# sec-bit/ckb-zkp

Measured on AMD Instinct MI355X. Metric: Groth16 proofs/sec (2^20 constraints, BN256), higher is better.
Workload: dtype u32 limbs (256-bit Montgomery integers); 1 GPU; Groth16 prove, MiMC-chain R1CS, 1048570 constraints (domain 2^20), 1258284 aux, bn254, G1 x4 + G2 x1 MSM + 4 NTT (7 in the reference: evaluation-form key); curve=bn254, log_domain=20, parallelism=independent proofs x1

## Files before the change

ckb_zkp_amd/_lib.py:

```python
from __future__ import annotations

import ctypes as C
import os
from pathlib import Path

LIB_PATH = Path(os.environ.get("ZKP_ACCEL_LIB") or Path(__file__).resolve().parent / "lib" / "libzkp_accel.so")

u64p = C.POINTER(C.c_uint64)
u32p = C.POINTER(C.c_uint32)
u8p = C.POINTER(C.c_uint8)
vp = C.c_void_p


class ZkpError(RuntimeError):
    def __init__(self, status: int, where: str, text: str):
        super().__init__(f"{where}: status {status} ({text})")
        self.status = status


class Csr(C.Structure):
    _fields_ = [("row_ptr", vp), ("col", vp), ("coeff", vp)]


class Groth16PkDesc(C.Structure):
# ... 35 lines not shown

class CtxConfig(C.Structure):
    _fields_ = [("struct_size", C.c_uint32), ("lanes", C.c_int32), ("msm_batch_lanes", C.c_int32),
                ("msm_window_bits", C.c_int32), ("msm_window_bits_g2", C.c_int32), ("msm_chunk_points", C.c_int64),
                ("table_budget_gb", C.c_double), ("h_evaluation_form", C.c_int32), ("c_fold", C.c_int32),
                ("host_affine", C.c_int32), ("c_fold_heavy_cost", C.c_int64), ("multi_exchange", C.c_int32),
                ("multi_exchange_timeout_ms", C.c_int32), ("multi_witness_split", C.c_int32)]


ZKP_ON, ZKP_OFF = 1, 2
ZKP_EXCHANGE_AUTO, ZKP_EXCHANGE_RCCL, ZKP_EXCHANGE_PEER = 0, 1, 2


def make_config(config) -> "CtxConfig | None":
    if config is None:
        return None
    if isinstance(config, CtxConfig):
        cfg = config
    else:
        cfg = CtxConfig()
        names = {f[0] for f in CtxConfig._fields_} - {"struct_size"}
        for k, v in dict(config).items():
            if k not in names:
                raise KeyError(f"zkp_ctx_config has no field {k!r} (fields: {sorted(names)})")
            if isinstance(v, bool):
                v = ZKP_ON if v else ZKP_OFF
            if k == "multi_exchange" and isinstance(v, str):
                v = {"auto": ZKP_EXCHANGE_AUTO, "rccl": ZKP_EXCHANGE_RCCL, "peer": ZKP_EXCHANGE_PEER}[v]
            setattr(cfg, k, v)
    cfg.struct_size = C.sizeof(CtxConfig)
    return cfg


MARLIN_NUM_EVALS = 21


class MarlinProof(C.Structure):
    _fields_ = [("comm", C.c_uint64 * (9 * 12)), ("comm_inf", C.c_uint8 * 9),
                ("shifted", C.c_uint64 * (2 * 12)), ("shifted_inf", C.c_uint8 * 2),
                ("evaluations", C.c_uint64 * (MARLIN_NUM_EVALS * 4)), ("num_opening_proofs", C.c_uint32),
                ("opening_w", C.c_uint64 * (2 * 12)), ("opening_w_inf", C.c_uint8 * 2), ("opening_has_rand", C.c_uint8 * 2),
                ("opening_rand_v", C.c_uint64 * (2 * 4)), ("challenges", C.c_uint64 * (7 * 4))]


SIGNATURES = {
    "zkp_status_string": (C.c_char_p, [C.c_int32]),
    "zkp_version": (C.c_char_p, []),
    "zkp_ctx_create": (C.c_int32, [C.POINTER(vp), C.c_int]),
    "zkp_ctx_create_ex": (C.c_int32, [C.POINTER(vp), C.c_int, C.POINTER(CtxConfig)]),
    "zkp_ctx_get_config": (C.c_int32, [vp, C.POINTER(CtxConfig)]),
    "zkp_ctx_destroy": (C.c_int32, [vp]),
    "zkp_ctx_create_multi": (C.c_int32, [C.POINTER(vp), C.POINTER(C.c_int), C.c_int]),
    "zkp_ctx_create_multi_ex": (C.c_int32, [C.POINTER(vp), C.POINTER(C.c_int), C.c_int, C.POINTER(CtxConfig)]),
    "zkp_ctx_num_devices": (C.c_int32, [vp, C.POINTER(C.c_int32)]),
    "zkp_ctx_device": (C.c_int32, [vp, C.c_int32, C.POINTER(vp)]),
    "zkp_groth16_pk_upload_multi": (C.c_int32, [vp, C.POINTER(Groth16PkDesc), C.c_int32, C.POINTER(vp)]),
    "zkp_groth16_pk_multi_free": (C.c_int32, [vp, vp]),
    "zkp_groth16_multi_info": (C.c_int32, [vp, vp, u64p]),
    "zkp_groth16_prove_multi": (C.c_int32, [vp, vp, vp, C.c_int32, vp, vp, vp, vp]),
    "zkp_groth16_prove_batch_multi": (C.c_int32, [vp, vp, C.c_size_t, vp, C.c_int32, vp, vp, vp, vp]),
    "zkp_ctx_set_stream": (C.c_int32, [vp, vp]),
    "zkp_ctx_sync": (C.c_int32, [vp]),
    "zkp_dev_alloc": (C.c_int32, [vp, C.c_size_t, C.POINTER(vp)]),
    "zkp_dev_free": (C.c_int32, [vp, vp]),
    "zkp_h2d": (C.c_int32, [vp, vp, vp, C.c_size_t]),
    "zkp_d2h": (C.c_int32, [vp, vp, vp, C.c_size_t]),
    "zkp_timer_start": (C.c_int32, [vp]),
    "zkp_timer_stop_ms": (C.c_int32, [vp, C.POINTER(C.c_float)]),
    "zkp_ntt": (C.c_int32, [vp, C.c_int, vp, C.c_uint32, C.c_int32]),
    "zkp_ntt_dev": (C.c_int32, [vp, C.c_int, vp, C.c_uint32, C.c_int32]),
    "zkp_bases_upload_g1": (C.c_int32, [vp, C.c_int, vp, vp, C.c_size_t, C.POINTER(C.c_uint64)]),
    "zkp_bases_upload_g2": (C.c_int32, [vp, C.c_int, vp, vp, C.c_size_t, C.POINTER(C.c_uint64)]),
    "zkp_bases_share": (C.c_int32, [vp, vp, C.c_uint64, u64p]),
    "zkp_bases_free": (C.c_int32, [vp, C.c_uint64]),
    "zkp_bases_len": (C.c_int32, [vp, C.c_uint64, C.POINTER(C.c_size_t)]),
    "zkp_msm_g1": (C.c_int32, [vp, C.c_uint64, C.c_size_t, vp, C.c_size_t, vp]),
    "zkp_msm_g2": (C.c_int32, [vp, C.c_uint64, C.c_size_t, vp, C.c_size_t, vp]),
    "zkp_msm_g1_dev": (C.c_int32, [vp, C.c_uint64, C.c_size_t, vp, C.c_size_t, vp]),
    "zkp_msm_g2_dev": (C.c_int32, [vp, C.c_uint64, C.c_size_t, vp, C.c_size_t, vp]),
    "zkp_vartime_multiscalar_mul_g1": (C.c_int32, [vp, C.c_uint64, vp, C.c_size_t, vp]),
    "zkp_vartime_multiscalar_mul_g2": (C.c_int32, [vp, C.c_uint64, vp, C.c_size_t, vp]),
    "zkp_msm_g1_var": (C.c_int32, [vp, C.c_int, vp, vp, vp, C.c_size_t, C.c_int32, vp]),
    "zkp_msm_g2_var": (C.c_int32, [vp, C.c_int, vp, vp, vp, C.c_size_t, C.c_int32, vp]),
    "zkp_msm_g1_var_batch_dev": (C.c_int32, [vp, C.c_int, C.c_size_t, vp, vp, vp, vp, C.c_int32, vp]),
    "zkp_msm_g2_var_batch_dev": (C.c_int32, [vp, C.c_int, C.c_size_t, vp, vp, vp, vp, C.c_int32, vp]),
    "zkp_g1_ipa_fold_dev": (C.c_int32, [vp, C.c_int, vp, vp, vp, vp, C.c_size_t, vp, vp, vp, vp]),
    "zkp_fr_dot_batch_dev": (C.c_int32, [vp, C.c_int, C.c_size_t, vp, vp, vp, vp]),
    "zkp_fr_sumcheck_round_dev": (C.c_int32, [vp, C.c_int, C.c_int32, C.c_size_t, vp, C.c_size_t, vp, vp]),
    "zkp_fr_eq_evals_dev": (C.c_int32, [vp, C.c_int, vp, C.c_size_t, vp]),
    "zkp_fr_product_circuit_dev": (C.c_int32, [vp, C.c_int, C.c_size_t, vp, C.c_size_t, vp]),
    "zkp_fr_memcheck_circuits_dev": (C.c_int32, [vp, C.c_int, C.c_size_t, vp, vp, vp, vp, vp, C.c_size_t, vp, vp, vp]),
    "zkp_msm_g1_mont_dev": (C.c_int32, [vp, C.c_uint64, C.c_size_t, vp, C.c_size_t, vp]),
    "zkp_msm_g2_mont_dev": (C.c_int32, [vp, C.c_uint64, C.c_size_t, vp, C.c_size_t, vp]),
    "zkp_msm_g1_mont_batch_dev": (C.c_int32, [vp, C.c_uint64, C.c_size_t, vp, vp, vp, vp]),
    "zkp_msm_mont_multi_dev": (C.c_int32, [vp, C.c_size_t, vp, vp, vp, vp, vp, C.c_size_t]),
    "zkp_fr_vec_op_dev": (C.c_int32, [vp, C.c_int, C.c_int32, vp, vp, vp, vp, C.c_size_t]),
    "zkp_fr_spmv_dev": (C.c_int32, [vp, C.c_int, vp, vp, vp, C.c_size_t, vp, vp]),
    "zkp_fr_gather_dev": (C.c_int32, [vp, vp, vp, C.c_size_t, vp]),
    "zkp_poly_divide_by_vanishing_dev": (C.c_int32, [vp, C.c_int, vp, C.c_size_t, C.c_size_t, vp, vp]),
    "zkp_d2d": (C.c_int32, [vp, vp, vp, C.c_size_t]),
    "zkp_dev_zero": (C.c_int32, [vp, vp, C.c_size_t]),
    "zkp_fr_batch_inverse_dev": (C.c_int32, [vp, C.c_int, vp, C.c_size_t]),
    "zkp_poly_evaluate_dev": (C.c_int32, [vp, C.c_int, vp, C.c_size_t, vp, vp]),
    "zkp_poly_div_linear_dev": (C.c_int32, [vp, C.c_int, vp, C.c_size_t, vp, vp, vp]),
    "zkp_g1_fold": (C.c_int32, [vp, C.c_int, vp, C.c_size_t, vp]),
    "zkp_g2_fold": (C.c_int32, [vp, C.c_int, vp, C.c_size_t, vp]),
    "zkp_g1_into_affine": (C.c_int32, [vp, C.c_int, vp, vp, vp]),
    "zkp_g1_decompress": (C.c_int32, [vp, C.c_int, vp, C.c_size_t, vp, vp, C.POINTER(C.c_size_t)]),
    "zkp_g2_decompress": (C.c_int32, [vp, C.c_int, vp, C.c_size_t, vp, vp, C.POINTER(C.c_size_t)]),
    "zkp_g1_compress": (C.c_int32, [vp, C.c_int, vp, vp, C.c_size_t, vp]),
    "zkp_g2_compress": (C.c_int32, [vp, C.c_int, vp, vp, C.c_size_t, vp]),
    "zkp_g1_subgroup_check": (C.c_int32, [vp, C.c_int, vp, vp, C.c_size_t, C.POINTER(C.c_size_t)]),
    "zkp_g2_subgroup_check": (C.c_int32, [vp, C.c_int, vp, vp, C.c_size_t, C.POINTER(C.c_size_t)]),
    "zkp_g2_into_affine": (C.c_int32, [vp, C.c_int, vp, vp, vp]),
    "zkp_groth16_points_into_affine": (C.c_int32, [C.c_int, vp, vp, vp, vp, vp]),
    "zkp_fixed_base_mul_g1": (C.c_int32, [vp, C.c_int, vp, vp, C.c_size_t, vp, vp]),
    "zkp_fixed_base_mul_g2": (C.c_int32, [vp, C.c_int, vp, vp, C.c_size_t, vp, vp]),
    "zkp_groth16_pk_upload": (C.c_int32, [vp, C.POINTER(Groth16PkDesc), C.POINTER(vp)]),
    "zkp_groth16_pk_upload_ex": (C.c_int32, [vp, C.POINTER(Groth16PkDesc), C.c_uint32, C.POINTER(vp)]),
    "zkp_groth16_pk_upload_shard": (C.c_int32, [vp, C.POINTER(Groth16PkDesc), C.c_int32, C.c_int32, C.POINTER(vp)]),
    "zkp_groth16_partials_bytes": (C.c_int32, [C.c_int, C.POINTER(C.c_size_t)]),
    "zkp_groth16_prove_partials_dev": (C.c_int32, [vp, vp, vp, vp, vp, vp]),
    "zkp_groth16_fold_assemble_dev": (C.c_int32, [vp, C.c_int, vp, C.c_int32, vp, vp, vp, vp]),
    "zkp_groth16_pk_free": (C.c_int32, [vp, vp]),
    "zkp_groth16_witness_map": (C.c_int32, [vp, vp, vp, vp]),
    "zkp_groth16_witness_map_dev": (C.c_int32, [vp, vp, vp, vp]),
    "zkp_groth16_domain_size": (C.c_int32, [vp, C.POINTER(C.c_uint64)]),
    "zkp_groth16_pk_info": (C.c_int32, [vp, vp, C.POINTER(C.c_uint64)]),
    "zkp_groth16_prove": (C.c_int32, [vp, vp, vp, vp, vp, vp, vp]),
    "zkp_groth16_prove_dev": (C.c_int32, [vp, vp, vp, vp, vp, vp, vp]),
    "zkp_groth16_prove_batch_dev": (C.c_int32, [vp, vp, C.c_size_t, vp, vp, vp, vp, vp]),
    "zkp_groth16_prove_batch": (C.c_int32, [vp, vp, C.c_size_t, vp, vp, vp, vp, vp]),
    "zkp_groth16_assemble": (C.c_int32, [vp, C.c_int, vp, vp, vp, vp, vp]),
    "zkp_groth16_last_timing": (C.c_int32, [vp, C.POINTER(Groth16Timing)]),
    "zkp_marlin_last_timing": (C.c_int32, [vp, C.POINTER(MarlinTiming)]),
    "zkp_set_profiling": (C.c_int32, [vp, C.c_int32]),
    "zkp_marlin_index_upload": (C.c_int32, [vp, C.POINTER(MarlinIndexDesc), C.POINTER(vp)]),
    "zkp_marlin_index_free": (C.c_int32, [vp, vp]),
    "zkp_marlin_index_info": (C.c_int32, [vp, u64p]),
    "zkp_marlin_index_commit": (C.c_int32, [vp, vp, C.c_uint64, vp, vp]),
    "zkp_marlin_prove": (C.c_int32, [vp, vp, C.c_uint64, C.c_uint64, vp, C.c_size_t, vp, vp, C.c_size_t,
                                     C.POINTER(MarlinRand), vp, C.POINTER(MarlinProof)]),
    "zkp_fs_rng_new": (C.c_int32, [vp, C.c_size_t, C.POINTER(vp)]),
    "zkp_fs_rng_free": (C.c_int32, [vp]),
    "zkp_fs_rng_absorb": (C.c_int32, [vp, vp, C.c_size_t]),
    "zkp_fs_rng_seed": (C.c_int32, [vp, vp]),
    "zkp_fs_rng_next_u64": (C.c_int32, [vp, u64p]),
    "zkp_fs_rng_rand_u128": (C.c_int32, [vp, vp]),
    "zkp_fs_rng_rand_fr": (C.c_int32, [vp, C.c_int, vp]),
    "zkp_fs_rng_sample_outside_domain": (C.c_int32, [vp, C.c_int, C.c_uint32, vp]),
    "zkp_merlin_oneshot": (C.c_int32, [vp, C.c_size_t, vp, C.c_size_t, vp, C.c_size_t, vp, C.c_size_t, vp, C.c_size_t]),
    "zkp_bench_mulmod": (C.c_int32, [vp, C.c_int, C.c_int32, C.c_int32, C.POINTER(C.c_double)]),
    "zkp_bench_hbm_copy": (C.c_int32, [vp, C.c_size_t, C.POINTER(C.c_double)]),
}

_lib = None


def load(path: os.PathLike | None = None) -> C.CDLL:
    global _lib
    if _lib is not None and path is None:
        return _lib
    p = Path(path) if path else LIB_PATH
    if not p.exists():
        raise ImportError(f"{p} not found — build it with `python -m ckb_zkp_amd.build` "
                          "(hipcc --offload-arch=gfx950); there is no CPU fallback")
    lib = C.CDLL(str(p))
    for name, (res, args) in SIGNATURES.items():
        fn = getattr(lib, name)
        fn.restype, fn.argtypes = res, args
    if path is None:
        _lib = lib
    return lib


ZKP_ERR_INVALID_POINT = -7


def check(status: int, where: str) -> None:
    if status != 0:
        raise ZkpError(status, where, load().zkp_status_string(status).decode())
```

ckb_zkp_amd/csrc/capi.hip:

```cpp
#include <cstdint>
#include <cstdlib>
#include <cstring>

#include "ctx.hpp"
#include "host_field.hpp"
#include "internal.hpp"
#include "ipa.hpp"
#include "spark.hpp"
#include "sumcheck.hpp"

using namespace zkp;

namespace {

template <class Fn>
int32_t guarded(zkp_ctx* ctx, Fn&& fn) {
  if (!ctx) return ZKP_ERR_BAD_ARG;
  std::lock_guard<std::recursive_mutex> lk(ctx->mu);
  try {
    ZKP_HIP(hipSetDevice(ctx->device));
    fn();
    return ZKP_OK;
  } catch (const StatusError& e) {
    return e.status;
// ... 572 lines not shown
  return subgroup_any(ctx, curve, 1, xy, inf, n, bad);
}
int32_t zkp_g2_subgroup_check(zkp_ctx* ctx, zkp_curve_t curve, const uint64_t* xy, const uint8_t* inf, size_t n, size_t* bad) {
  return subgroup_any(ctx, curve, 2, xy, inf, n, bad);
}
int32_t zkp_fixed_base_mul_g1(zkp_ctx* ctx, zkp_curve_t curve, const uint64_t* base, const uint64_t* scalars, size_t n,
                              uint64_t* out_xy, uint8_t* out_inf) {
  if (!base || (n && (!scalars || !out_xy || !out_inf))) return ZKP_ERR_BAD_ARG;
  return guarded(ctx, [&] { fixed_base_mul(ctx, curve, 1, base, scalars, n, out_xy, out_inf); });
}
int32_t zkp_fixed_base_mul_g2(zkp_ctx* ctx, zkp_curve_t curve, const uint64_t* base, const uint64_t* scalars, size_t n,
                              uint64_t* out_xy, uint8_t* out_inf) {
  if (!base || (n && (!scalars || !out_xy || !out_inf))) return ZKP_ERR_BAD_ARG;
  return guarded(ctx, [&] { fixed_base_mul(ctx, curve, 2, base, scalars, n, out_xy, out_inf); });
}

int32_t zkp_groth16_pk_upload(zkp_ctx* ctx, const zkp_groth16_pk_desc* desc, zkp_groth16_pk** out) {
  if (!desc || !out) return ZKP_ERR_BAD_ARG;
  return guarded(ctx, [&] { *out = groth16_pk_upload(ctx, desc); });
}
int32_t zkp_groth16_pk_upload_ex(zkp_ctx* ctx, const zkp_groth16_pk_desc* desc, uint32_t flags, zkp_groth16_pk** out) {
  if (!desc || !out || (flags & ~(uint32_t)ZKP_PK_KEEP_FORM)) return ZKP_ERR_BAD_ARG;
  return guarded(ctx, [&] { *out = groth16_pk_upload(ctx, desc, 0, 0, (int)flags); });
}
int32_t zkp_groth16_pk_upload_shard(zkp_ctx* ctx, const zkp_groth16_pk_desc* desc, int32_t rank, int32_t world,
                                    zkp_groth16_pk** out) {
  if (!desc || !out || world < 1 || rank < 0 || rank >= world) return ZKP_ERR_BAD_ARG;
  return guarded(ctx, [&] { *out = groth16_pk_upload(ctx, desc, rank, world); });
}
int32_t zkp_groth16_partials_bytes(zkp_curve_t curve, size_t* bytes) {
  if (!bytes || (curve != ZKP_BN254 && curve != ZKP_BLS12_381)) return ZKP_ERR_BAD_ARG;
  *bytes = groth16_partials_bytes(curve);
  return ZKP_OK;
}
int32_t zkp_groth16_prove_partials_dev(zkp_ctx* ctx, zkp_groth16_pk* pk, const uint64_t* z_dev, const uint64_t* r,
                                       const uint64_t* s, void* partials_dev) {
  if (!pk || !z_dev || !r || !s || !partials_dev) return ZKP_ERR_BAD_ARG;
  return guarded(ctx, [&] { groth16_prove_partials(ctx, pk, z_dev, r, s, partials_dev); });
}
int32_t zkp_groth16_fold_assemble_dev(zkp_ctx* ctx, zkp_curve_t curve, const void* gathered_dev, int32_t world,
                                      const uint64_t* r, const uint64_t* s, uint64_t* proof, uint8_t* inf) {
  if (!gathered_dev || world < 1 || !r || !s || !proof || !inf) return ZKP_ERR_BAD_ARG;
  return guarded(ctx, [&] { groth16_fold_assemble(ctx, curve, gathered_dev, world, r, s, proof, inf); });
}
int32_t zkp_groth16_pk_upload_multi(zkp_ctx* ctx, const zkp_groth16_pk_desc* desc, int32_t mode, zkp_groth16_pk_multi** out) {
  if (!ctx || !desc || !out || ctx->devs.empty() || (mode != ZKP_MULTI_SHARD && mode != ZKP_MULTI_REPLICATE)) return ZKP_ERR_BAD_ARG;
  return guarded_multi(ctx, [&] { *out = groth16_pk_upload_multi(ctx, desc, mode); });
}
int32_t zkp_groth16_pk_multi_free(zkp_ctx* ctx, zkp_groth16_pk_multi* pk) {
  if (!ctx || !pk || ctx->devs.empty()) return ZKP_ERR_BAD_ARG;
  return guarded_multi(ctx, [&] { groth16_pk_multi_free(ctx, pk); });
}
int32_t zkp_groth16_multi_info(zkp_ctx* ctx, zkp_groth16_pk_multi* pk, uint64_t info[6]) {
  if (!ctx || !pk || !info || ctx->devs.empty()) return ZKP_ERR_BAD_ARG;
  return guarded(ctx, [&] { groth16_multi_info(ctx, pk, info); });
}
int32_t zkp_groth16_prove_multi(zkp_ctx* ctx, zkp_groth16_pk_multi* pk, const uint64_t* const* z, int32_t z_on_device,
                                const uint64_t* r, const uint64_t* s, uint64_t* proof, uint8_t* inf) {
  if (!ctx || !pk || !z || !z[0] || !r || !s || !proof || !inf || ctx->devs.empty()) return ZKP_ERR_BAD_ARG;
  if (z_on_device)
    for (size_t k = 0; k < ctx->devs.size(); k++)
      if (!z[k]) return ZKP_ERR_BAD_ARG;
  return guarded_multi(ctx, [&] { groth16_prove_multi(ctx, pk, z, z_on_device != 0, r, s, proof, inf); });
}
int32_t zkp_groth16_prove_batch_multi(zkp_ctx* ctx, zkp_groth16_pk_multi* pk, size_t count, const uint64_t* const* z,
                                      int32_t z_on_device, const uint64_t* r, const uint64_t* s, uint64_t* proofs,
                                      uint8_t* inf) {
  if (!ctx || !pk || ctx->devs.empty() || (count && (!z || !r || !s || !proofs || !inf))) return ZKP_ERR_BAD_ARG;
  return guarded_multi(ctx, [&] { groth16_prove_batch_multi(ctx, pk, count, z, z_on_device != 0, r, s, proofs, inf); });
}
int32_t zkp_groth16_pk_free(zkp_ctx* ctx, zkp_groth16_pk* pk) {
  if (!pk) return ZKP_ERR_BAD_ARG;
  return guarded(ctx, [&] { groth16_pk_free(ctx, pk); });
}
int32_t zkp_groth16_pk_info(zkp_ctx* ctx, zkp_groth16_pk* pk, uint64_t info[8]) {
  if (!ctx || !pk || !info) return ZKP_ERR_BAD_ARG;
  return guarded(ctx, [&] { groth16_pk_info(ctx, pk, info); });
}
int32_t zkp_groth16_domain_size(zkp_groth16_pk* pk, uint64_t* n) {
  if (!pk || !n) return ZKP_ERR_BAD_ARG;
  *n = groth16_domain_size(pk);
  return ZKP_OK;
}
int32_t zkp_groth16_witness_map(zkp_ctx* ctx, zkp_groth16_pk* pk, const uint64_t* z, uint64_t* h) {
  if (!pk || !z || !h) return ZKP_ERR_BAD_ARG;
  return guarded(ctx, [&] { groth16_witness_map(ctx, pk, z, h, false); });
}
int32_t zkp_groth16_witness_map_dev(zkp_ctx* ctx, zkp_groth16_pk* pk, const uint64_t* z, uint64_t* h) {
  if (!pk || !z || !h) return ZKP_ERR_BAD_ARG;
  return guarded(ctx, [&] { groth16_witness_map(ctx, pk, z, h, true); });
}
int32_t zkp_groth16_prove(zkp_ctx* ctx, zkp_groth16_pk* pk, const uint64_t* z, const uint64_t* r, const uint64_t* s,
                          uint64_t* proof, uint8_t* inf) {
  if (!pk || !z || !r || !s || !proof || !inf) return ZKP_ERR_BAD_ARG;
  return guarded(ctx, [&] { groth16_prove(ctx, pk, z, false, r, s, proof, inf); });
}
int32_t zkp_groth16_prove_dev(zkp_ctx* ctx, zkp_groth16_pk* pk, const uint64_t* z, const uint64_t* r,
                              const uint64_t* s, uint64_t* proof, uint8_t* inf) {
  if (!pk || !z || !r || !s || !proof || !inf) return ZKP_ERR_BAD_ARG;
  return guarded(ctx, [&] { groth16_prove(ctx, pk, z, true, r, s, proof, inf); });
}
int32_t zkp_groth16_prove_batch_dev(zkp_ctx* ctx, zkp_groth16_pk* pk, size_t n, const uint64_t* const* z_dev,
                                    const uint64_t* r, const uint64_t* s, uint64_t* proofs, uint8_t* inf) {
  if (!pk || (n && (!z_dev || !r || !s || !proofs || !inf))) return ZKP_ERR_BAD_ARG;
  return guarded(ctx, [&] { groth16_prove_batch(ctx, pk, n, z_dev, r, s, proofs, inf); });
}
int32_t zkp_groth16_prove_batch(zkp_ctx* ctx, zkp_groth16_pk* pk, size_t n, const uint64_t* const* z_host,
                                const uint64_t* r, const uint64_t* s, uint64_t* proofs, uint8_t* inf) {
  if (!pk || (n && (!z_host || !r || !s || !proofs || !inf))) return ZKP_ERR_BAD_ARG;
  return guarded(ctx, [&] { groth16_prove_batch(ctx, pk, n, z_host, r, s, proofs, inf, false); });
}
int32_t zkp_groth16_assemble(zkp_ctx* ctx, zkp_curve_t curve, const uint64_t* sums, const uint64_t* r,
                             const uint64_t* s, uint64_t* proof, uint8_t* inf) {
  if (!sums || !r || !s || !proof || !inf) return ZKP_ERR_BAD_ARG;
  return guarded(ctx, [&] { groth16_assemble(ctx, curve, sums, r, s, proof, inf); });
}
int32_t zkp_marlin_index_upload(zkp_ctx* ctx, const zkp_marlin_index_desc* desc, zkp_marlin_index** out) {
  if (!desc || !out) return ZKP_ERR_BAD_ARG;
  return guarded(ctx, [&] { *out = marlin_index_upload(ctx, desc); });
}
int32_t zkp_marlin_index_free(zkp_ctx* ctx, zkp_marlin_index* index) {
  if (!index) return ZKP_ERR_BAD_ARG;
  return guarded(ctx, [&] { marlin_index_free(ctx, index); });
}
int32_t zkp_marlin_index_info(const zkp_marlin_index* index, uint64_t info[6]) {
  if (!index || !info) return ZKP_ERR_BAD_ARG;
  marlin_index_info(index, info);
  return ZKP_OK;
}
int32_t zkp_marlin_index_commit(zkp_ctx* ctx, zkp_marlin_index* index, uint64_t powers_of_g, uint64_t* comms_xy,
                                uint8_t* inf) {
  if (!index || !comms_xy || !inf) return ZKP_ERR_BAD_ARG;
  return guarded(ctx, [&] { marlin_index_commit(ctx, index, powers_of_g, comms_xy, inf); });
}
int32_t zkp_marlin_prove(zkp_ctx* ctx, zkp_marlin_index* index, uint64_t powers_of_g, uint64_t powers_of_gamma_g,
                         const uint8_t* ivk_bytes, size_t ivk_len, const uint64_t* x, const uint64_t* w, size_t n_w,
                         const zkp_marlin_rand* rnd, const uint64_t* fixed_challenges, zkp_marlin_proof* out) {
  if (!index || !x || (n_w && !w) || !rnd || !out || (!fixed_challenges && !ivk_bytes)) return ZKP_ERR_BAD_ARG;
  if (!rnd->w || !rnd->z_a || !rnd->z_b || !rnd->mask || !rnd->blind_w || !rnd->blind_z_a || !rnd->blind_z_b ||
      !rnd->blind_g_1 || !rnd->blind_shifted_g_1)
    return ZKP_ERR_BAD_ARG;
  return guarded(ctx, [&] {
    marlin_prove(ctx, index, powers_of_g, powers_of_gamma_g, ivk_bytes, ivk_len, x, w, n_w, rnd, fixed_challenges, out);
  });
}
int32_t zkp_bench_mulmod(zkp_ctx* ctx, zkp_curve_t curve, int32_t field, int32_t unsaturated, double* out) {
  if (!out || (curve != ZKP_BN254 && curve != ZKP_BLS12_381) || field < 0 || field > 1) return ZKP_ERR_BAD_ARG;
  return guarded(ctx, [&] { *out = bench_mulmod(ctx, curve, field, unsaturated != 0); });
}
int32_t zkp_bench_hbm_copy(zkp_ctx* ctx, size_t bytes, double* out) {
  if (!out) return ZKP_ERR_BAD_ARG;
  return guarded(ctx, [&] { *out = bench_hbm_copy(ctx, bytes); });
}
int32_t zkp_marlin_last_timing(zkp_ctx* ctx, zkp_marlin_timing* out) {
  if (!ctx || !out) return ZKP_ERR_BAD_ARG;
  return guarded(ctx, [&] { *out = ctx->last_marlin_timing; });
}
int32_t zkp_groth16_last_timing(zkp_ctx* ctx, zkp_groth16_timing* out) {
  if (!ctx || !out) return ZKP_ERR_BAD_ARG;
  return guarded(ctx, [&] { *out = ctx->last_timing; });
}

}
```

ckb_zkp_amd/csrc/internal.hpp:

```cpp
#pragma once
#include "ctx.hpp"

namespace zkp {

void ntt_run(zkp_ctx* ctx, int curve, uint32_t* data_dev, int log_n, int op);
void ntt_run_batch(zkp_ctx* ctx, int curve, uint32_t* const* data_dev, int count, int log_n, int op);
bool ntt_ifft_coset_fft(zkp_ctx* ctx, int curve, uint32_t* data, int log_n);
uint32_t* ntt_qap_coset_ifft(zkp_ctx* ctx, int curve, uint32_t* a, uint32_t* b, uint32_t* c, const uint32_t* zinv, int log_n);
void ntt_free_tables(zkp_ctx* ctx);

void fr_vec_op(zkp_ctx* ctx, int curve, int op, const uint64_t* a, const uint64_t* b, const uint64_t* k_host,
               uint64_t* out, size_t n);
void fr_batch_inverse(zkp_ctx* ctx, int curve, uint64_t* v, size_t n);
void fr_dot_batch(zkp_ctx* ctx, int curve, size_t count, const uint64_t* const* a, const uint64_t* const* b, const size_t* ns,
                  uint64_t* out_host);
void fr_spmv(zkp_ctx* ctx, int curve, const uint32_t* row_ptr, const uint32_t* col, const uint64_t* coeff, size_t nrows,
             const uint64_t* x, uint64_t* out);
void fr_gather(zkp_ctx* ctx, const uint64_t* in, const int32_t* idx, size_t n, uint64_t* out);
void poly_vanishing_fold(zkp_ctx* ctx, int curve, const uint64_t* p, size_t len, size_t n, uint64_t* q, uint64_t* rem);
void poly_div_linear(zkp_ctx* ctx, int curve, const uint64_t* p, size_t n, const uint64_t* z_host, uint64_t* q,
                     uint64_t* eval_out_host);
void marlin_round2_prod(zkp_ctx* ctx, int curve, const uint64_t* ra, const uint64_t* za, const uint64_t* zb, const uint64_t* t,
                        const uint64_t* z, const uint64_t* k_host, uint64_t* out, size_t n);
void marlin_t3_evals(zkp_ctx* ctx, int curve, const uint64_t* const* on_k, const uint64_t* k_host, uint64_t* out, size_t n);
void marlin_h2_numerator(zkp_ctx* ctx, int curve, const uint64_t* const* on_b, const uint64_t* t, const uint64_t* k_host, uint64_t* out,
                         size_t n);
void poly_evaluate_batch(zkp_ctx* ctx, int curve, size_t count, const uint64_t* const* p, const size_t* n, const uint64_t* z_host,
                         uint64_t* out_host);

uint64_t bases_upload(zkp_ctx* ctx, int curve, int group, const uint64_t* xy_host, const uint8_t* inf_host, size_t n,
                      int c_hint = 0, int cap_hint = 0, int lgk_hint = -1);
size_t bases_table_bytes(zkp_ctx* ctx, int curve, int group, size_t n, int lgk);
int bases_plan_lgk(zkp_ctx* ctx, int curve, const int* groups, const size_t* ns, int count);
void bases_free(zkp_ctx* ctx, uint64_t handle);
uint64_t bases_share(zkp_ctx* dst, zkp_ctx* src, uint64_t handle);
size_t bases_len(zkp_ctx* ctx, uint64_t handle);
int bases_group(zkp_ctx* ctx, uint64_t handle);
void msm_run(zkp_ctx* ctx, uint64_t handle, size_t offset, const uint64_t* scalars_dev, size_t n, bool montgomery,
             uint64_t* out_xyz_host, void* out_dev_xyzz = nullptr, float* ms_accumulate = nullptr,
             uint64_t* n_entries = nullptr, int ws = 0, int sort_src = -1, float* ms_scan = nullptr, int l1_src = -1);
double bench_mulmod(zkp_ctx* ctx, int curve, int field, bool unsaturated);
double bench_hbm_copy(zkp_ctx* ctx, size_t bytes);
bool bases_same_shape(zkp_ctx* ctx, uint64_t h1, uint64_t h2);
void bases_set_sort_flags(zkp_ctx* ctx, uint64_t handle, const uint8_t* flags_host, size_t n);
void bases_set_group(zkp_ctx* ctx, uint64_t owner, const uint8_t* member_flags_host, size_t n);
void bases_set_filter_bit(zkp_ctx* ctx, uint64_t handle, int bit);
void msm_run_batch(zkp_ctx* ctx, uint64_t handle, size_t count, const size_t* offsets, const uint64_t* const* scalars_dev,
                   const size_t* ns, bool montgomery, uint64_t* out_xyz_host);
void msm_run_multi(zkp_ctx* ctx, size_t count, const uint64_t* handles, const size_t* offsets,
                   const uint64_t* const* scalars_dev, const size_t* ns, bool montgomery, uint64_t* out_xyz_host,
                   size_t slot_words);
void msm_var_run(zkp_ctx* ctx, int curve, int group, const uint64_t* xy_host, const uint8_t* inf_host,
                 const uint64_t* scalars_host, size_t n, bool montgomery, uint64_t* out_xyz_host);
void msm_var_batch_run(zkp_ctx* ctx, int curve, int group, size_t count, const uint64_t* const* xy_dev,
                       const uint8_t* const* inf_dev, const uint64_t* const* scalars_dev, const size_t* ns, bool montgomery,
                       uint64_t* out_xyz_host);
void msm_free_all(zkp_ctx* ctx);
void bases_drop(zkp_ctx* ctx, uint64_t handle);
void point_fold(zkp_ctx* ctx, int curve, int group, const uint64_t* xyz_host, size_t k, uint64_t* out_xyz_host);
void point_into_affine(zkp_ctx* ctx, int curve, int group, const uint64_t* xyz_host, uint64_t* xy_out, uint8_t* inf_out);
size_t points_decompress(zkp_ctx* ctx, int curve, int group, const uint8_t* bytes, size_t n, uint64_t* xy_out, uint8_t* inf_out);
void points_compress(zkp_ctx* ctx, int curve, int group, const uint64_t* xy, const uint8_t* inf, size_t n, uint8_t* bytes_out);
size_t points_subgroup_check(zkp_ctx* ctx, int curve, int group, const uint64_t* xy, const uint8_t* inf, size_t n);
void points_fold_into_affine(zkp_ctx* ctx, int curve, int group, const uint64_t* a_xyz_host, const uint64_t* b_xyz_host,
                             const uint8_t* has_b, size_t k, uint64_t* xy_out, uint8_t* inf_out);
void fixed_base_mul(zkp_ctx* ctx, int curve, int group, const uint64_t* base_xy, const uint64_t* scalars_host, size_t n,
                    uint64_t* out_xy, uint8_t* out_inf);

zkp_groth16_pk* groth16_pk_upload(zkp_ctx* ctx, const zkp_groth16_pk_desc* d, int rank = 0, int world = 0, int flags = 0);
size_t groth16_partials_bytes(int curve);
void groth16_prove_partials(zkp_ctx* ctx, zkp_groth16_pk* pk, const uint64_t* z_dev, const uint64_t* r, const uint64_t* s,
                            void* out_dev);
void groth16_fold_assemble(zkp_ctx* ctx, int curve, const void* gathered_dev, int world, const uint64_t* r,
                           const uint64_t* s, uint64_t* proof_out, uint8_t* inf_out);
void groth16_pk_free(zkp_ctx* ctx, zkp_groth16_pk* pk);
uint64_t groth16_domain_size(zkp_groth16_pk* pk);
void groth16_pk_info(zkp_ctx* ctx, zkp_groth16_pk* pk, uint64_t info[8]);
void bases_info(zkp_ctx* ctx, uint64_t handle, uint64_t info[5]);
void groth16_witness_map(zkp_ctx* ctx, zkp_groth16_pk* pk, const uint64_t* z, uint64_t* h, bool on_device);
void groth16_prove(zkp_ctx* ctx, zkp_groth16_pk* pk, const uint64_t* z, bool z_on_device, const uint64_t* r,
                   const uint64_t* s, uint64_t* proof_out, uint8_t* inf_out);

void groth16_prove_batch(zkp_ctx* ctx, zkp_groth16_pk* pk, size_t n, const uint64_t* const* z_dev, const uint64_t* r,
                         const uint64_t* s, uint64_t* proofs_out, uint8_t* inf_out, bool z_on_device = true);
void groth16_assemble(zkp_ctx* ctx, int curve, const uint64_t* sums_xyz, const uint64_t* r, const uint64_t* s,
                      uint64_t* proof_out, uint8_t* inf_out);

zkp_groth16_pk_multi* groth16_pk_upload_multi(zkp_ctx* root, const zkp_groth16_pk_desc* d, int mode);
void groth16_pk_multi_free(zkp_ctx* root, zkp_groth16_pk_multi* pk);
void groth16_multi_info(zkp_ctx* root, zkp_groth16_pk_multi* pk, uint64_t info[6]);
void groth16_prove_multi(zkp_ctx* root, zkp_groth16_pk_multi* pk, const uint64_t* const* z, bool z_on_device, const uint64_t* r,
                         const uint64_t* s, uint64_t* proof_out, uint8_t* inf_out);
void groth16_prove_batch_multi(zkp_ctx* root, zkp_groth16_pk_multi* pk, size_t n, const uint64_t* const* z, bool z_on_device,
                               const uint64_t* r, const uint64_t* s, uint64_t* proofs_out, uint8_t* inf_out);

zkp_marlin_index* marlin_index_upload(zkp_ctx* ctx, const zkp_marlin_index_desc* d);
void marlin_index_free(zkp_ctx* ctx, zkp_marlin_index* ix);
void marlin_index_commit(zkp_ctx* ctx, zkp_marlin_index* ix, uint64_t powers_g, uint64_t* comms_xy, uint8_t* inf);
void marlin_index_info(const zkp_marlin_index* ix, uint64_t info[6]);
void marlin_prove(zkp_ctx* ctx, zkp_marlin_index* ix, uint64_t powers_g, uint64_t powers_gamma_g, const uint8_t* ivk_bytes,
                  size_t ivk_len, const uint64_t* x_mont, const uint64_t* w_mont, size_t n_w, const zkp_marlin_rand* rnd,
                  const uint64_t* fixed_challenges, zkp_marlin_proof* out);

}
```

ckb_zkp_amd/csrc/msm.hip:

```cpp
#include <algorithm>
#include <cstdlib>
#include <cstring>
#include <map>
#include <type_traits>
#include <memory>
#include <mutex>
#include <vector>

#include "field_dev.hpp"
#include "internal.hpp"
#include "msm_digits.hpp"
#include "msm_small.hpp"
#include "msm_vtbl.hpp"

namespace zkp {

#if defined(ZKP_NO_SORT_PRIO)
#define ZKP_SORT_PRIO() do { } while (0)
#else
#define ZKP_SORT_PRIO() __builtin_amdgcn_s_setprio(3)
#endif

const MsmVtbl* msm_vtbl_c01();
const MsmVtbl* msm_vtbl_c02();
// ... 65 lines not shown
  if ((1 << lgk) >= p.W) {
    p.lgk = 0;
    while ((1 << p.lgk) < p.W) p.lgk++;
  }
  p.J = (p.W + (1 << p.lgk) - 1) >> p.lgk;
  return p;
}
size_t bases_table_bytes(zkp_ctx* ctx, int curve, int group, size_t n, int lgk) {
  const MsmVtbl* vt = msm_vtbl(curve, group);
  return std::max<size_t>(1, n) * (size_t)window_plan(ctx->cfg, vt->scalar_bits, n, group, 0, lgk).J * vt->aff_bytes;
}
static double table_budget_left(zkp_ctx* ctx) {
  size_t free_b = 0, total_b = 0;
  if (hipMemGetInfo(&free_b, &total_b) != hipSuccess) return 1e30;
  double left = (double)free_b - 0.25 * (double)total_b;
  if (ctx->cfg.table_budget_gb > 0.0) {
    const double b = ctx->cfg.table_budget_gb * 1073741824.0 - (double)ctx->table_bytes;
    left = std::min(left + 0.25 * (double)total_b - 1073741824.0, b);
  }
  return left;
}
int bases_plan_lgk(zkp_ctx* ctx, int curve, const int* groups, const size_t* ns, int count) {
  if (const char* e = getenv("ZKP_TABLE_K")) {
    int k = atoi(e), lg = 0;
    while ((1 << lg) < k) lg++;
    return std::min(lg, 6);
  }
  const double left = table_budget_left(ctx);
  for (int lgk = 0; lgk <= 6; lgk++) {
    double need = 0;
    for (int q = 0; q < count; q++) need += (double)bases_table_bytes(ctx, curve, groups[q], ns[q], lgk);
    if (need <= left) return lgk;
  }
  return 6;
}

uint64_t bases_upload(zkp_ctx* ctx, int curve, int group, const uint64_t* xy, const uint8_t* inf, size_t n, int c_hint,
                      int cap_hint, int lgk_hint) {
  auto e = std::make_shared<BasesEntry>();
  e->curve = curve;
  e->group = group;
  e->vt = msm_vtbl(curve, group);
  e->n = n;
  int lgk = lgk_hint;
  if (lgk < 0) lgk = c_hint > 0 ? 0 : bases_plan_lgk(ctx, curve, &group, &n, 1);
  const WindowPlan wp = window_plan(ctx->cfg, e->vt->scalar_bits, n, group, c_hint, lgk);
  e->c = wp.c;
  e->W = wp.W;
  e->wide = wp.wide;
  e->lgk = wp.lgk;
  e->var = wp.lgk > 0;
  {
    const char* env = group == 2 ? getenv("ZKP_TASK_CAP_G2") : nullptr;
    if (!env) env = getenv("ZKP_TASK_CAP");
    if (cap_hint >= 4) e->cap = std::min<uint32_t>(MSM_TASK_CAP, (uint32_t)cap_hint);
    if (env && atoi(env) >= 4) e->cap = std::min<uint32_t>(MSM_TASK_CAP, (uint32_t)atoi(env));
  }
  ZKP_REQUIRE((double)n * e->W < 2147483000.0, ZKP_ERR_BAD_ARG);
  const size_t ab = e->vt->aff_bytes;
  size_t bytes = std::max<size_t>(1, n) * wp.J * ab;
  if (hipMalloc(&e->table, bytes) != hipSuccess) throw StatusError{ZKP_ERR_OOM};
  e->table_bytes = bytes;
  ctx->table_bytes += bytes;
  if (n) {
    ZKP_HIP(hipMemcpyAsync(e->table, xy, n * ab, hipMemcpyHostToDevice, ctx->cur->stream));
    if (inf) {
      if (hipMalloc(&e->inf, n) != hipSuccess) throw StatusError{ZKP_ERR_OOM};
      ZKP_HIP(hipMemcpyAsync(e->inf, inf, n, hipMemcpyHostToDevice, ctx->cur->stream));
      e->vt->ingest(ctx->cur->stream, e->table, e->inf, n);
    }
    if (wp.lgk > 0) e->vt->precompute(ctx->cur->stream, e->table, n, e->c << wp.lgk, wp.J, wp.J);
    else e->vt->precompute(ctx->cur->stream, e->table, n, e->c, e->W, e->wide);
    ZKP_HIP(hipGetLastError());
    ZKP_HIP(hipStreamSynchronize(ctx->cur->stream));
  }
  if (getenv("ZKP_DEBUG_MSM"))
    fprintf(stderr, "[msm] bases group=%d n=%zu: c=%d W=%d wide=%d k=%d copies=%d (%.2f GiB)\n", group, n, e->c, e->W, e->wide,
            1 << e->lgk, wp.J, (double)bytes / 1073741824.0);
  uint64_t h = ctx->next_handle++;
  ctx->bases[h] = e;
  return h;
}

static std::shared_ptr<BasesEntry> get_bases(zkp_ctx* ctx, uint64_t handle) {
  auto it = ctx->bases.find(handle);
  if (it == ctx->bases.end()) throw StatusError{ZKP_ERR_BAD_HANDLE};
  return it->second;
}
void bases_free(zkp_ctx* ctx, uint64_t handle) {
  ZKP_HIP(hipStreamSynchronize(ctx->cur->stream));
  auto it = ctx->bases.find(handle);
  if (it == ctx->bases.end()) throw StatusError{ZKP_ERR_BAD_HANDLE};
  if (it->second.use_count() == 1) ctx->table_bytes -= std::min(ctx->table_bytes, it->second->table_bytes);
  ctx->bases.erase(it);
}
size_t bases_len(zkp_ctx* ctx, uint64_t handle) { return get_bases(ctx, handle)->n; }
int bases_group(zkp_ctx* ctx, uint64_t handle) { return get_bases(ctx, handle)->group; }
void bases_info(zkp_ctx* ctx, uint64_t handle, uint64_t info[5]) {
  auto e = get_bases(ctx, handle);
  info[0] = (uint64_t)e->c;
  info[1] = (uint64_t)e->W;
  info[2] = (uint64_t)1 << e->lgk;
  info[3] = e->lgk ? (uint64_t)((e->W + (1 << e->lgk) - 1) >> e->lgk) : (uint64_t)e->W;
  info[4] = e->table_bytes;
}
void bases_drop(zkp_ctx* ctx, uint64_t handle) {
  auto it = ctx->bases.find(handle);
  if (it == ctx->bases.end()) return;
  if (it->second.use_count() == 1) ctx->table_bytes -= std::min(ctx->table_bytes, it->second->table_bytes);
  ctx->bases.erase(it);
}
void msm_free_all(zkp_ctx* ctx) {
  ctx->bases.clear();
  ctx->table_bytes = 0;
  ctx->var_plans.clear();
}
uint64_t bases_share(zkp_ctx* dst, zkp_ctx* src, uint64_t handle) {
  auto e = get_bases(src, handle);
  ZKP_REQUIRE(dst->device == src->device, ZKP_ERR_BAD_ARG);
  uint64_t h = dst->next_handle++;
  dst->bases[h] = e;
  return h;
}
void bases_set_sort_flags(zkp_ctx* ctx, uint64_t handle, const uint8_t* flags_host, size_t n) {
  auto e = get_bases(ctx, handle);
  ZKP_REQUIRE(n == e->n, ZKP_ERR_BAD_ARG);
  if (e->sort_inf) (void)hipFree(e->sort_inf);
  e->sort_inf = nullptr;
  if (!flags_host || n == 0) return;
  if (hipMalloc(&e->sort_inf, n) != hipSuccess) throw StatusError{ZKP_ERR_OOM};
  ZKP_HIP(hipMemcpyAsync(e->sort_inf, flags_host, n, hipMemcpyHostToDevice, ctx->cur->stream));
  ZKP_HIP(hipStreamSynchronize(ctx->cur->stream));
}
void bases_set_group(zkp_ctx* ctx, uint64_t owner, const uint8_t* member_flags_host, size_t n) {
  auto e = get_bases(ctx, owner);
  ZKP_REQUIRE(n == e->n, ZKP_ERR_BAD_ARG);
  if (e->group_flags) (void)hipFree(e->group_flags);
  e->group_flags = nullptr;
  if (!member_flags_host || n == 0) return;
  if (hipMalloc(&e->group_flags, n) != hipSuccess) throw StatusError{ZKP_ERR_OOM};
  ZKP_HIP(hipMemcpyAsync(e->group_flags, member_flags_host, n, hipMemcpyHostToDevice, ctx->cur->stream));
  ZKP_HIP(hipStreamSynchronize(ctx->cur->stream));
}
void bases_set_filter_bit(zkp_ctx* ctx, uint64_t handle, int bit) {
  ZKP_REQUIRE(bit >= -1 && bit < 3, ZKP_ERR_BAD_ARG);
  get_bases(ctx, handle)->filter_bit = bit;
}
bool bases_same_shape(zkp_ctx* ctx, uint64_t h1, uint64_t h2) {
  auto a = get_bases(ctx, h1), b = get_bases(ctx, h2);
  return a->curve == b->curve && a->n == b->n && a->c == b->c && a->W == b->W && a->wide == b->wide && a->cap == b->cap && a->lgk == b->lgk;
}


constexpr int SCAN_CHUNK = 2048;
__global__ __launch_bounds__(256) void scan_reduce_kernel(const uint32_t* __restrict__ in, size_t n,
                                                          uint32_t* __restrict__ sums) {
  ZKP_SORT_PRIO();
  __shared__ uint32_t red[256];
  size_t base = (size_t)blockIdx.x * SCAN_CHUNK;
  uint32_t acc = 0;
  for (int k = 0; k < SCAN_CHUNK / 256; k++) {
    size_t i = base + (size_t)k * 256 + threadIdx.x;
    if (i < n) acc += in[i];
  }
  red[threadIdx.x] = acc;
  __syncthreads();
  for (int s = 128; s > 0; s >>= 1) {
    if ((int)threadIdx.x < s) red[threadIdx.x] += red[threadIdx.x + s];
    __syncthreads();
  }
  if (threadIdx.x == 0) sums[blockIdx.x] = red[0];
}
__global__ __launch_bounds__(1024) void scan_sums_kernel(uint32_t* __restrict__ sums, size_t m) {
  ZKP_SORT_PRIO();
  __shared__ uint32_t buf[1024];
  uint32_t carry = 0;
  for (size_t t0 = 0; t0 < m; t0 += 1024) {
    size_t i = t0 + threadIdx.x;
    uint32_t v = i < m ? sums[i] : 0;
    buf[threadIdx.x] = v;
    __syncthreads();
    for (int d = 1; d < 1024; d <<= 1) {
      uint32_t add = (int)threadIdx.x >= d ? buf[threadIdx.x - d] : 0;
      __syncthreads();
      buf[threadIdx.x] += add;
      __syncthreads();
    }
    if (i < m) sums[i] = carry + buf[threadIdx.x] - v;
    uint32_t total = buf[1023];
    __syncthreads();
    carry += total;
  }
}
__global__ __launch_bounds__(256) void scan_apply_kernel(const uint32_t* __restrict__ in, size_t n,
                                                         const uint32_t* __restrict__ sums,
                                                         uint32_t* __restrict__ out) {
  ZKP_SORT_PRIO();
  __shared__ uint32_t part[256];
  size_t base = (size_t)blockIdx.x * SCAN_CHUNK;
  constexpr int PER = SCAN_CHUNK / 256;
  uint32_t v[PER];
  uint32_t acc = 0;
  for (int k = 0; k < PER; k++) {
    size_t i = base + (size_t)threadIdx.x * PER + k;
    v[k] = i < n ? in[i] : 0;
    acc += v[k];
  }
  part[threadIdx.x] = acc;
  __syncthreads();
  for (int d = 1; d < 256; d <<= 1) {
    uint32_t add = (int)threadIdx.x >= d ? part[threadIdx.x - d] : 0;
    __syncthreads();
    part[threadIdx.x] += add;
    __syncthreads();
  }
  uint32_t run = sums[blockIdx.x] + part[threadIdx.x] - acc;
  for (int k = 0; k < PER; k++) {
    size_t i = base + (size_t)threadIdx.x * PER + k;
    if (i < n) out[i] = run;
    run += v[k];
  }
}
static void exclusive_scan_u32(hipStream_t st, const uint32_t* in, uint32_t* out, size_t n, DevBuf& tmp) {
  if (n == 0) return;
  size_t chunks = (n + SCAN_CHUNK - 1) / SCAN_CHUNK;
  uint32_t* sums = tmp.as<uint32_t>(chunks + 1);
  hipLaunchKernelGGL(scan_reduce_kernel, dim3(chunks), dim3(256), 0, st, in, n, sums);
  hipLaunchKernelGGL(scan_sums_kernel, dim3(1), dim3(1024), 0, st, sums, chunks);
  hipLaunchKernelGGL(scan_apply_kernel, dim3(chunks), dim3(256), 0, st, in, n, sums, out);
}

constexpr int SORT_H1_MAX = 13;
constexpr uint32_t SORT_BIN_TARGET = 16384;
constexpr int SORT_L_MAX = 13;
constexpr int SORT_SCALARS = 2048;
constexpr int SORT_SCALARS_UNUSED_ = 0;
template <class FrP, int NT>
__global__ __launch_bounds__(NT) void sort_hist_kernel(const uint32_t* __restrict__ scalars, size_t n, size_t offset,
                                                        const uint8_t* __restrict__ inf, int montgomery, int c, int W, int wide,
                                                        uint32_t nb, int L, uint32_t nbins1,
                                                        uint32_t* __restrict__ hist, uint32_t nblocks, uint32_t tile,
                                                        int lgk) {
  ZKP_SORT_PRIO();
  const uint32_t gmask = (1u << lgk) - 1;
  __shared__ uint32_t cnt[(1 << SORT_H1_MAX) + 1];
  for (uint32_t i = threadIdx.x; i <= nbins1; i += NT) cnt[i] = 0;
  __syncthreads();
  for (uint32_t j = threadIdx.x; j < tile; j += NT) {
    size_t i = (size_t)blockIdx.x * tile + j;
    if (i < n && !(inf && inf[offset + i])) {
      DigitIter it = load_scalar<FrP>(scalars, i, montgomery);
      for (int w = 0; w < W; w++) {
        uint32_t key, neg;
        it.next(w, c, wide, nb, key, neg);
        if (key < nb) atomicAdd(&cnt[((((uint32_t)w & gmask) << (c - 1)) | key) >> L], 1u);
      }
    }
  }
  __syncthreads();
  for (uint32_t i = threadIdx.x; i < nbins1; i += NT) hist[(size_t)i * nblocks + blockIdx.x] = cnt[i];
}
template <class FrP>
__global__ __launch_bounds__(256) void sort_scatter_kernel(const uint32_t* __restrict__ scalars, size_t n,
                                                           size_t offset, const uint8_t* __restrict__ inf,
                                                           int montgomery, size_t ntab, int c, int W, int wide, uint32_t nb,
                                                           int L, uint32_t nbins1, const uint32_t* __restrict__ offs,
                                                           uint32_t nblocks, uint32_t tile,
                                                           uint64_t* __restrict__ kv, int lgk,
                                                           const uint8_t* __restrict__ group_flags) {
  ZKP_SORT_PRIO();
  const uint32_t gmask = (1u << lgk) - 1;
  __shared__ uint32_t cur[(1 << SORT_H1_MAX) + 1];
  for (uint32_t i = threadIdx.x; i < nbins1; i += 256) cur[i] = offs[(size_t)i * nblocks + blockIdx.x];
  __syncthreads();
  const uint32_t lmask = (1u << L) - 1;
  for (uint32_t rep = 0; rep < tile / 256; rep++) {
    size_t i = (size_t)blockIdx.x * tile + rep * 256 + threadIdx.x;
    if (i < n && !(inf && inf[offset + i])) {
      DigitIter it = load_scalar<FrP>(scalars, i, montgomery);
      const uint64_t gbits = group_flags ? (uint64_t)(group_flags[offset + i] & 7u) << 61 : 0;
      for (int w = 0; w < W; w++) {
        uint32_t key, neg;
        it.next(w, c, wide, nb, key, neg);
        if (key < nb) {
          const uint32_t fk = (((uint32_t)w & gmask) << (c - 1)) | key;
          uint32_t pos = atomicAdd(&cur[fk >> L], 1u);
          uint32_t val = (uint32_t)((size_t)(w >> lgk) * ntab + offset + i) | (neg << 31);
          kv[pos] = gbits | ((uint64_t)(fk & lmask) << 32) | val;
        }
      }
    }
  }
}
template <int NT>
__device__ __forceinline__ uint32_t block_excl_scan(uint32_t v, uint32_t* tmp, uint32_t* total) {
  const uint32_t t = threadIdx.x, lane = t & 63u, wave = t >> 6;
  uint32_t incl = v;
#pragma unroll
  for (int d = 1; d < 64; d <<= 1) {
    const uint32_t up = (uint32_t)__shfl_up((int)incl, d, 64);
    if (lane >= (uint32_t)d) incl += up;
  }
  if (lane == 63u) tmp[wave] = incl;
  __syncthreads();
  if (t == 0) {
    uint32_t run = 0;
    for (int w = 0; w < NT / 64; w++) {
      const uint32_t x = tmp[w];
      tmp[w] = run;
      run += x;
    }
    tmp[NT / 64] = run;
  }
  __syncthreads();
  const uint32_t res = tmp[wave] + incl - v;
  *total = tmp[NT / 64];
  __syncthreads();
  return res;
}

__device__ __forceinline__ uint32_t wave_agg_inc(uint32_t* cnt, uint32_t idx, bool active) {
  const uint64_t act = __ballot(active);
  uint32_t res = 0;
  if (act == 0) return 0;
  const int leader = __ffsll((unsigned long long)act) - 1;
  const uint32_t lidx = (uint32_t)__builtin_amdgcn_readlane((int)idx, leader);
  const bool same = active && idx == lidx;
  const uint64_t m = __ballot(same);
  const uint32_t pc = (uint32_t)__popcll(m);
  if (pc >= 8) {
    const uint32_t lane = __builtin_amdgcn_mbcnt_hi(~0u, __builtin_amdgcn_mbcnt_lo(~0u, 0u));
    uint32_t base = 0;
    if ((int)lane == leader) base = atomicAdd(&cnt[lidx], pc);
    base = (uint32_t)__builtin_amdgcn_readlane((int)base, leader);
    if (same) res = base + __builtin_amdgcn_mbcnt_hi((uint32_t)(m >> 32), __builtin_amdgcn_mbcnt_lo((uint32_t)m, 0u));
    else if (active) res = atomicAdd(&cnt[idx], 1u);
  } else if (active) {
    res = atomicAdd(&cnt[idx], 1u);
  }
  return res;
}

#ifndef ZKP_SORT_STAGE_BYTES
#define ZKP_SORT_STAGE_BYTES (56 * 1024)
#endif
constexpr uint32_t SORT_STAGE_BYTES = ZKP_SORT_STAGE_BYTES;
template <class FrP, int NT>
__global__ __launch_bounds__(NT) void sort_scatter_staged_kernel(const uint32_t* __restrict__ scalars, size_t n,
                                                                  size_t offset, const uint8_t* __restrict__ inf,
                                                                  int montgomery, size_t ntab, int c, int W, int wide, uint32_t nb,
                                                                  int L, uint32_t nbins1, const uint32_t* __restrict__ offs,
                                                                  uint32_t nblocks, uint32_t tile, uint64_t* __restrict__ kv,
                                                                  int lgk, const uint8_t* __restrict__ group_flags, uint32_t sub) {
  ZKP_SORT_PRIO();
  const uint32_t gmask = (1u << lgk) - 1;
  extern __shared__ __attribute__((aligned(16))) uint32_t sm[];
  __shared__ uint32_t pre[NT];
  uint32_t* cur = sm;
  uint32_t* cnt = cur + nbins1;
  uint64_t* stage = reinterpret_cast<uint64_t*>(cnt + ((nbins1 + 3) & ~3u));
  const uint32_t tid = threadIdx.x;
  for (uint32_t i = tid; i < nbins1; i += NT) cur[i] = offs[(size_t)i * nblocks + blockIdx.x];
  const uint32_t lmask = (1u << L) - 1;
  const uint32_t per = (nbins1 + NT - 1) / NT;
  for (uint32_t s0 = 0; s0 < tile; s0 += sub) {
    for (uint32_t i = tid; i < nbins1; i += NT) cnt[i] = 0;
    __syncthreads();
    for (uint32_t rep = 0; rep * NT < sub; rep++) {
      const uint32_t j = rep * NT + tid;
      const size_t i = (size_t)blockIdx.x * tile + s0 + j;
      const bool live = j < sub && s0 + j < tile && i < n && !(inf && inf[offset + i]);
      DigitIter it = load_scalar<FrP>(scalars, live ? i : 0, montgomery);
      for (int w = 0; w < W; w++) {
        uint32_t key, neg;
        it.next(w, c, wide, nb, key, neg);
        const uint32_t fk = (((uint32_t)w & gmask) << (c - 1)) | key;
        (void)wave_agg_inc(cnt, fk >> L, live && key < nb);
      }
    }
    __syncthreads();
    uint32_t total;
    {
      uint32_t acc = 0;
      for (uint32_t k = 0; k < per; k++) {
        const uint32_t idx = tid * per + k;
        if (idx < nbins1) acc += cnt[idx];
      }
      uint32_t run = block_excl_scan<NT>(acc, pre, &total);
      for (uint32_t k = 0; k < per; k++) {
        const uint32_t idx = tid * per + k;
        if (idx < nbins1) {
          const uint32_t v = cnt[idx];
          cnt[idx] = run;
          run += v;
        }
      }
    }
    __syncthreads();
    for (uint32_t rep = 0; rep * NT < sub; rep++) {
      const uint32_t j = rep * NT + tid;
      const size_t i = (size_t)blockIdx.x * tile + s0 + j;
      const bool live = j < sub && s0 + j < tile && i < n && !(inf && inf[offset + i]);
      DigitIter it = load_scalar<FrP>(scalars, live ? i : 0, montgomery);
      const uint64_t gbits = live && group_flags ? (uint64_t)(group_flags[offset + i] & 7u) << 61 : 0;
      for (int w = 0; w < W; w++) {
        uint32_t key, neg;
        it.next(w, c, wide, nb, key, neg);
        const uint32_t fk = (((uint32_t)w & gmask) << (c - 1)) | key;
        const bool act = live && key < nb;
        const uint32_t pos = wave_agg_inc(cnt, fk >> L, act);
        if (act) {
          const uint32_t val = (uint32_t)((size_t)(w >> lgk) * ntab + offset + i) | (neg << 31);
          stage[pos] = gbits | ((uint64_t)(fk >> L) << 45) | ((uint64_t)(fk & lmask) << 32) | val;
        }
      }
    }
    __syncthreads();
    for (uint32_t j = tid; j < total; j += NT) {
      const uint64_t e = stage[j];
      const uint32_t b = (uint32_t)(e >> 45) & 0x1fffu;
      const uint32_t lo = b ? cnt[b - 1] : 0;
      kv[cur[b] + (j - lo)] = e;
    }
    __syncthreads();
    for (uint32_t b = tid; b < nbins1; b += NT) cur[b] += cnt[b] - (b ? cnt[b - 1] : 0);
    __syncthreads();
  }
}
constexpr uint32_t SORT_BIN_THREADS = 1024;
#ifndef ZKP_SORT_BIN_STAGE
#define ZKP_SORT_BIN_STAGE 20480
#endif
constexpr uint32_t SORT_BIN_STAGE = ZKP_SORT_BIN_STAGE;
__global__ __launch_bounds__(SORT_BIN_THREADS) void sort_bin_kernel(const uint64_t* __restrict__ kv,
                                                                    const uint32_t* __restrict__ offs,
                                                                    uint32_t nblocks, int L,
                                                                    uint32_t* __restrict__ vout,
                                                                    uint32_t* __restrict__ start,
                                                                    uint32_t* __restrict__ end, int drop_bit) {
  ZKP_SORT_PRIO();
  extern __shared__ uint32_t sm[];
  __shared__ uint32_t pre[SORT_BIN_THREADS];
  const uint32_t nk = 1u << L;
  uint32_t* cnt = sm;
  uint32_t* stage = sm + nk;
  const uint32_t b = blockIdx.x, T = SORT_BIN_THREADS, t = threadIdx.x;
  const uint32_t lo = offs[(size_t)b * nblocks], hi = offs[(size_t)(b + 1) * nblocks];
  const bool staged = hi - lo <= SORT_BIN_STAGE;
  for (uint32_t i = t; i < nk; i += T) cnt[i] = 0;
  __syncthreads();
  const uint64_t dmask = drop_bit >= 0 ? (uint64_t)1 << (61 + drop_bit) : 0;
  const uint32_t kmask = nk - 1;
  for (uint32_t i = lo + t; i < hi; i += T) {
    const uint64_t x = kv[i];
    if (!(x & dmask)) atomicAdd(&cnt[(uint32_t)(x >> 32) & kmask], 1u);
  }
  __syncthreads();
  {
    const uint32_t per = (nk + T - 1) / T;
    uint32_t acc = 0;
    for (uint32_t k = 0; k < per; k++) {
      uint32_t idx = t * per + k;
      if (idx < nk) acc += cnt[idx];
    }
    uint32_t total_unused;
    uint32_t run = block_excl_scan<(int)SORT_BIN_THREADS>(acc, pre, &total_unused);
    for (uint32_t k = 0; k < per; k++) {
      uint32_t idx = t * per + k;
      if (idx < nk) {
        uint32_t v = cnt[idx];
        start[((size_t)b << L) + idx] = lo + run;
        end[((size_t)b << L) + idx] = lo + run + v;
        cnt[idx] = run;
        run += v;
      }
    }
  }
  __syncthreads();
  for (uint32_t i = lo + t; i < hi; i += T) {
    const uint64_t x = kv[i];
    if (x & dmask) continue;
    uint32_t pos = atomicAdd(&cnt[(uint32_t)(x >> 32) & kmask], 1u);
    if (staged) stage[pos] = (uint32_t)x;
    else vout[lo + pos] = (uint32_t)x;
  }
  if (staged) {
    __syncthreads();
    for (uint32_t i = t; i < hi - lo; i += T) vout[lo + i] = stage[i];
  }
}

constexpr int TM_NLONG = 0, TM_HIST = 1, TM_CUR = 256, TM_WORDS = 512;

__global__ void task_count_kernel(const uint32_t* __restrict__ start, const uint32_t* __restrict__ end, uint32_t nb,
                                  uint32_t* __restrict__ tcount, uint32_t cap) {
  ZKP_SORT_PRIO();
  uint32_t b = blockIdx.x * blockDim.x + threadIdx.x;
  if (b > nb) return;
  tcount[b] = b < nb ? (end[b] - start[b] + cap - 1) / cap : 0;
}

__global__ __launch_bounds__(256) void zero_empty_buckets_kernel(const uint32_t* __restrict__ start,
                                                                 const uint32_t* __restrict__ end, uint32_t nb,
                                                                 char* __restrict__ buckets, uint32_t xb) {
  ZKP_SORT_PRIO();
  const uint32_t b = blockIdx.x * blockDim.x + threadIdx.x;
  if (b >= nb || end[b] != start[b]) return;
  uint4* p = reinterpret_cast<uint4*>(buckets + (size_t)b * xb);
  for (uint32_t k = 0; k < xb / 16; k++) p[k] = make_uint4(0, 0, 0, 0);
}

__global__ __launch_bounds__(1024) void task_fill_kernel(const uint32_t* __restrict__ start,
                                                        const uint32_t* __restrict__ end,
                                                        const uint32_t* __restrict__ toff, uint32_t nb,
                                                        uint32_t* __restrict__ task_start,
                                                        uint32_t* __restrict__ task_len,
                                                        uint32_t* __restrict__ task_dst,
                                                        uint32_t* __restrict__ long_list,
                                                        uint32_t* __restrict__ tmeta, uint32_t cap) {
  ZKP_SORT_PRIO();
  __shared__ uint32_t hist[MSM_TASK_CAP + 1];
  for (int i = threadIdx.x; i <= (int)MSM_TASK_CAP; i += blockDim.x) hist[i] = 0;
  __syncthreads();
  uint32_t b = blockIdx.x * blockDim.x + threadIdx.x;
  if (b < nb) {
    const uint32_t s = start[b], len = end[b] - s;
    const uint32_t t0 = toff[b], nt = toff[b + 1] - t0;
    if (nt > 1) long_list[atomicAdd(&tmeta[TM_NLONG], 1u)] = b;
    for (uint32_t j = 0; j < nt; j++) {
      uint32_t l = min(cap, len - j * cap);
      task_start[t0 + j] = s + j * cap;
      task_len[t0 + j] = l;
      task_dst[t0 + j] = nt == 1 ? b : (0x80000000u | (t0 + j));
      atomicAdd(&hist[l], 1u);
    }
  }
  __syncthreads();
  for (int i = threadIdx.x; i <= (int)MSM_TASK_CAP; i += blockDim.x)
    if (hist[i]) atomicAdd(&tmeta[TM_HIST + i], hist[i]);
}

__global__ void task_cursor_kernel(uint32_t* tmeta) {
  ZKP_SORT_PRIO();
  if (threadIdx.x || blockIdx.x) return;
  uint32_t acc = 0;
  for (int l = MSM_TASK_CAP; l >= 0; l--) {
    tmeta[TM_CUR + l] = acc;
    acc += tmeta[TM_HIST + l];
  }
}

__global__ __launch_bounds__(1024) void task_order_kernel(const uint32_t* __restrict__ task_start,
                                                         const uint32_t* __restrict__ task_len,
                                                         const uint32_t* __restrict__ task_dst,
                                                         const uint32_t* __restrict__ n_tasks_dev,
                                                         uint32_t* __restrict__ tmeta, uint4* __restrict__ desc) {
  ZKP_SORT_PRIO();
  __shared__ uint32_t cnt[MSM_TASK_CAP + 1];
  __shared__ uint32_t base[MSM_TASK_CAP + 1];
  for (int i = threadIdx.x; i <= (int)MSM_TASK_CAP; i += blockDim.x) cnt[i] = 0;
  __syncthreads();
  uint32_t t = blockIdx.x * blockDim.x + threadIdx.x;
  const bool live = t < *n_tasks_dev;
  uint32_t l = 0, rank = 0;
  if (live) {
    l = task_len[t];
    rank = atomicAdd(&cnt[l], 1u);
  }
  __syncthreads();
  for (int i = threadIdx.x; i <= (int)MSM_TASK_CAP; i += blockDim.x)
    if (cnt[i]) base[i] = atomicAdd(&tmeta[TM_CUR + i], cnt[i]);
  __syncthreads();
  if (live) desc[base[l] + rank] = make_uint4(task_start[t], l, task_dst[t], t);
}

__global__ void sched_check_kernel(const uint32_t* toff, const uint32_t* long_list, const uint32_t* tmeta, uint32_t nb,
                                   uint32_t max_tasks, uint32_t* rep) {
  const uint32_t n_long = tmeta[TM_NLONG], n_tasks = toff[nb];
  for (uint32_t b = blockIdx.x * blockDim.x + threadIdx.x; b < nb; b += gridDim.x * blockDim.x) {
    if (toff[b + 1] < toff[b]) atomicAdd(&rep[0], 1u);
    atomicMax(&rep[1], toff[b + 1] - toff[b]);
  }
  for (uint32_t w = blockIdx.x * blockDim.x + threadIdx.x; w < n_long; w += gridDim.x * blockDim.x)
    if (long_list[w] >= nb) atomicAdd(&rep[2], 1u);
  if (blockIdx.x == 0 && threadIdx.x == 0) {
    rep[3] = n_long;
    rep[4] = n_tasks;
    rep[5] = n_tasks > max_tasks;
  }
}

static void msm_run_entry(zkp_ctx* ctx, const BasesEntry* be, size_t offset, const uint64_t* scalars_dev, size_t n,
                          bool montgomery, uint64_t* out_xyz_host, void* out_dev_xyzz, float* ms_accumulate,
                          uint64_t* n_entries, int ws_idx, int sort_src, float* ms_scan, int l1_src = -1);
void msm_run(zkp_ctx* ctx, uint64_t handle, size_t offset, const uint64_t* scalars_dev, size_t n, bool montgomery,
             uint64_t* out_xyz_host, void* out_dev_xyzz, float* ms_accumulate, uint64_t* n_entries, int ws_idx,
             int sort_src, float* ms_scan, int l1_src) {
  struct ChainReset {
    zkp_ctx* c;
    ~ChainReset() {
      c->msm_defer_reduce = false;
      c->msm_acc_into = -1;
    }
  } chain_reset{ctx};
  auto be = get_bases(ctx, handle);
  const size_t chunk_pts = (size_t)std::max<long long>(0, ctx->cfg.msm_chunk);
  const bool chunkable = chunk_pts >= 1024 && n >= 2 * chunk_pts && be->group == 1 && !be->var && sort_src < 0 && l1_src < 0 &&
                         !be->group_flags && !ctx->profiling && !ms_accumulate && !ms_scan && !n_entries &&
                         !ctx->msm_defer_reduce && ctx->msm_acc_into < 0 && ctx->msm_bucket_ws < 0 && !ctx->batch_mode;
  if (!chunkable) {
    msm_run_entry(ctx, be.get(), offset, scalars_dev, n, montgomery, out_xyz_host, out_dev_xyzz, ms_accumulate, n_entries,
                  ws_idx, sort_src, ms_scan, l1_src);
    return;
  }
  const size_t nch0 = (n + chunk_pts - 1) / chunk_pts, per = ((n + nch0 - 1) / nch0 + 255) & ~(size_t)255;
  static const size_t first_div = [] { const char* e = getenv("ZKP_MSM_CHUNK_FIRST"); long v = e ? atol(e) : 2; return (size_t)(v < 1 ? 1 : v); }();
  const size_t first = first_div > 1 ? std::max<size_t>(((per / first_div) + 255) & ~(size_t)255, 1024) : 0;
  const size_t rest = first && first < n ? n - first : n;
  const size_t nrest = (rest + per - 1) / per, per_rest = ((rest + nrest - 1) / nrest + 255) & ~(size_t)255;
  const size_t nch = (first && first < n ? 1 : 0) + (rest + per_rest - 1) / per_rest;
  const int wa = ws_idx, wb = ws_idx ^ 2;
  hipStream_t sa = wa == 0 ? ctx->cur->stream : ctx->cur->ws[wa].stream, sb = wb == 0 ? ctx->cur->stream : ctx->cur->ws[wb].stream;
  ZKP_HIP(hipEventRecord(ctx->cur->ws[wa].l1_done, sa));
  ZKP_HIP(hipStreamWaitEvent(sb, ctx->cur->ws[wa].l1_done, 0));
  size_t done = 0;
  for (size_t k = 0; k < nch; k++) {
    const size_t len = std::min((k == 0 && first && first < n) ? first : per_rest, n - done);
    const bool last = k + 1 == nch;
    const int w = ((nch - 1 - k) & 1) ? wb : wa;
    ctx->msm_defer_reduce = !last;
    ctx->msm_acc_into = k > 0 ? wa : -1;
    ctx->msm_bucket_ws = wa;
    msm_run_entry(ctx, be.get(), offset + done, scalars_dev + 4 * done, len, montgomery, last ? out_xyz_host : nullptr,
                  last ? out_dev_xyzz : nullptr, nullptr, nullptr, w, -1, nullptr, -1);
    done += len;
  }
}

struct VarPlan {
  DevBuf d1, d2;
  uint32_t n1 = 0, n2 = 0;
};
static VarPlan& var_plan(zkp_ctx* ctx, int c, int W, hipStream_t st) {
  auto key = std::make_pair(c, W);
  auto it = ctx->var_plans.find(key);
  if (it != ctx->var_plans.end()) return *static_cast<VarPlan*>(it->second.get());
  const uint32_t nb_w = 1u << (c - 1);
  std::vector<SegDesc> s1, s2(256);
  uint32_t lvl_off = 0, cnt = (uint32_t)W * nb_w;
  for (auto& d : s2) d = SegDesc{0, 1, 0, 0};
  for (int l = 0; l < c - 1; l++) {
    const uint32_t pw = nb_w >> (l + 1);
    const uint32_t ch = std::min<uint32_t>((uint32_t)SEG_CHUNK, pw);
    for (int w = 0; w < W; w++) {
      const uint32_t first = (uint32_t)s1.size();
      for (uint32_t j = 0; j < pw / ch; j++)
        s1.push_back(SegDesc{lvl_off + (uint32_t)w * (nb_w >> l) + 1 + 2 * j * ch, 2, ch, (uint32_t)s1.size()});
      const int t = c * w + l;
      if (t < 256) s2[t] = SegDesc{first, 1, (uint32_t)s1.size() - first, (uint32_t)t};
    }
    lvl_off += cnt;
    cnt >>= 1;
  }
  for (int t = 0; t < 256; t++) s2[t].out = (uint32_t)t;
  auto vp = std::make_shared<VarPlan>();
  vp->n1 = (uint32_t)s1.size();
  vp->n2 = 256;
  ZKP_HIP(hipMemcpyAsync(vp->d1.as<SegDesc>(s1.size()), s1.data(), s1.size() * sizeof(SegDesc), hipMemcpyHostToDevice, st));
  ZKP_HIP(hipMemcpyAsync(vp->d2.as<SegDesc>(256), s2.data(), 256 * sizeof(SegDesc), hipMemcpyHostToDevice, st));
  ZKP_HIP(hipStreamSynchronize(st));
  ctx->var_plans[key] = vp;
  return *vp;
}

static void msm_run_entry(zkp_ctx* ctx, const BasesEntry* be, size_t offset, const uint64_t* scalars_dev, size_t n,
                          bool montgomery, uint64_t* out_xyz_host, void* out_dev_xyzz, float* ms_accumulate,
                          uint64_t* n_entries, int ws_idx, int sort_src, float* ms_scan, int l1_src) {
  const MsmVtbl* vt = be->vt;
  MsmWorkspace& ws = ctx->cur->ws[ws_idx];
  const bool defer = ctx->msm_defer_reduce;
  const int into = ctx->msm_acc_into;
  const int bucket_ws = into >= 0 ? into : ctx->msm_bucket_ws;
  ctx->msm_defer_reduce = false;
  ctx->msm_acc_into = -1;
  ctx->msm_bucket_ws = -1;
  ZKP_REQUIRE(!(defer || into >= 0) || (n > 0 && !be->var && be->group == 1), ZKP_ERR_BAD_ARG);
  const bool reuse = sort_src >= 0;
  MsmWorkspace& sw = reuse ? ctx->cur->ws[sort_src] : ws;
  hipStream_t st = ws_idx == 0 ? ctx->cur->stream : ws.stream;
  const size_t XB = vt->bucket_bytes;
  const size_t jac_words = 3 * (size_t)vt->fN;
  uint32_t* out_jac = ws.out.as<uint32_t>(64 * 4);
  if (ms_accumulate) *ms_accumulate = 0.f;
  if (ms_scan) *ms_scan = 0.f;
  if (n_entries) *n_entries = 0;
  if (n == 0) {
    vt->write_identity(st, (char*)out_dev_xyzz, out_jac);
  } else {
    const int c = be->c, W = be->W, wide = be->wide;
    const int var = be->var ? 1 : 0;
    const int lgk = be->lgk, K = 1 << lgk;
    ZKP_REQUIRE(var == (lgk > 0), ZKP_ERR_BAD_ARG);
    const uint32_t nb_w = 1u << (c - 1);
    const int kbits = (c - 1) + lgk;
    const uint32_t nb = 1u << kbits;
    const size_t E = n * (size_t)W;
    ZKP_REQUIRE(E < 2147483000ull, ZKP_ERR_BAD_ARG);
    const bool l1_reuse = !reuse && l1_src >= 0;
    MsmWorkspace& lw = l1_reuse ? ctx->cur->ws[l1_src] : sw;
    uint32_t* vals = sw.vals.as<uint32_t>(E + 8);
    uint64_t* kv = lw.keys2.as<uint64_t>(E);
    const uint32_t* sc = reinterpret_cast<const uint32_t*>(scalars_dev);
    const int mont = montgomery ? 1 : 0;
    static const int h1_env = [] { const char* e = getenv("ZKP_SORT_H1"); return e ? atoi(e) : 0; }();
    int H1 = 10;
    while (H1 < SORT_H1_MAX && (E >> H1) > SORT_BIN_TARGET) H1++;
    if (h1_env > 0) H1 = std::min(SORT_H1_MAX, h1_env);
    H1 = std::min(H1, kbits);
    if (kbits - H1 > SORT_L_MAX) H1 = kbits - SORT_L_MAX;
    const int LB = kbits - H1;
    const uint32_t nbins1 = 1u << H1;
    uint32_t tile = SORT_SCALARS;
    while ((n + tile - 1) / tile > 1536) tile += 256;
    const uint32_t nblocks = (uint32_t)((n + tile - 1) / tile);
    const size_t hist_n = (size_t)nbins1 * nblocks + 1;
    uint32_t* hist = lw.sort_tmp.as<uint32_t>(2 * hist_n);
    uint32_t* offs = hist + hist_n;
    uint32_t* start = sw.offsets.as<uint32_t>(2 * (size_t)nb);
    uint32_t* end = start + nb;
    const uint8_t* scan_inf = be->sort_inf && !ctx->profiling ? be->sort_inf : be->inf;
    if (reuse) {
      if (sort_src != ws_idx) ZKP_HIP(hipStreamWaitEvent(st, sw.sorted, 0));
    } else if (l1_reuse) {
      if (l1_src != ws_idx) ZKP_HIP(hipStreamWaitEvent(st, lw.l1_done, 0));
    } else {
      ZKP_HIP(hipMemsetAsync(hist + hist_n - 1, 0, 4, st));
    }
    const uint8_t* grp = scan_inf == be->sort_inf ? be->group_flags : nullptr;
    static const bool staged_on = !(getenv("ZKP_SORT_STAGED") && atoi(getenv("ZKP_SORT_STAGED")) == 0);
    uint32_t staged_sub = 0;
    size_t staged_lds = 0;
    if (staged_on && nbins1 <= 2048 && (size_t)256 * W * 8 <= SORT_STAGE_BYTES) {
      staged_sub = (uint32_t)(SORT_STAGE_BYTES / ((size_t)W * 8)) / 256 * 256;
      staged_sub = std::min<uint32_t>(staged_sub, tile);
      staged_lds = ((size_t)nbins1 + ((nbins1 + 3) & ~3u)) * 4 + (size_t)staged_sub * W * 8;
    }
    const bool timed_scan = ms_scan && ctx->profiling && !reuse && !l1_reuse;
    if (timed_scan) ZKP_HIP(hipEventRecord(ctx->ev2, st));
    if (reuse || l1_reuse) {
    } else {
      static const int nt_hist = [] { const char* e = getenv("ZKP_SORT_NT_HIST"); return e ? atoi(e) : 1024; }();
      static const int nt_scat = [] { const char* e = getenv("ZKP_SORT_NT_SCATTER"); return e ? atoi(e) : 512; }();
      auto level1 = [&](auto tag) {
        using FrP = decltype(tag);
        auto hist_l = [&](auto nt) {
          constexpr int NT = decltype(nt)::value;
          hipLaunchKernelGGL((sort_hist_kernel<FrP, NT>), dim3(nblocks), dim3(NT), 0, st, sc, n, offset, scan_inf, mont, c, W, wide, nb_w,
                             LB, nbins1, hist, nblocks, tile, lgk);
        };
        if (nt_hist >= 1024) hist_l(std::integral_constant<int, 1024>{});
        else if (nt_hist >= 512) hist_l(std::integral_constant<int, 512>{});
        else hist_l(std::integral_constant<int, 256>{});
        exclusive_scan_u32(st, hist, offs, hist_n, ws.scan_tmp);
        if (staged_sub) {
          auto scat_l = [&](auto nt) {
            constexpr int NT = decltype(nt)::value;
            hipLaunchKernelGGL((sort_scatter_staged_kernel<FrP, NT>), dim3(nblocks), dim3(NT), staged_lds, st, sc, n, offset,
                               scan_inf, mont, be->n, c, W, wide, nb_w, LB, nbins1, offs, nblocks, tile, kv, lgk, grp, staged_sub);
          };
          if (nt_scat >= 1024) scat_l(std::integral_constant<int, 1024>{});
          else if (nt_scat >= 512) scat_l(std::integral_constant<int, 512>{});
          else scat_l(std::integral_constant<int, 256>{});
        } else {
          hipLaunchKernelGGL(sort_scatter_kernel<FrP>, dim3(nblocks), dim3(256), 0, st, sc, n, offset, scan_inf, mont, be->n, c, W, wide,
                             nb_w, LB, nbins1, offs, nblocks, tile, kv, lgk, grp);
        }
      };
      if (be->curve == ZKP_BN254) level1(Bn254Fr{});
      else level1(Bls381Fr{});
    }
    if (timed_scan) {
      ZKP_HIP(hipEventRecord(ctx->ev3, st));
      ZKP_HIP(hipEventSynchronize(ctx->ev3));
      ZKP_HIP(hipEventElapsedTime(ms_scan, ctx->ev2, ctx->ev3));
    }
    if (!reuse && !l1_reuse) ZKP_HIP(hipEventRecord(ws.l1_done, st));
    if (!reuse && !l1_reuse) ctx->mark(st, ":l1");
    if (!reuse)
      hipLaunchKernelGGL(sort_bin_kernel, dim3(nbins1), dim3(SORT_BIN_THREADS), ((size_t)4 << LB) + 4 * (size_t)SORT_BIN_STAGE, st,
                         kv, offs, nblocks, LB, vals, start, end, (l1_reuse || grp) ? be->filter_bit : -1);
    uint32_t* const sorted_vals = vals;
    const uint32_t max_tasks = nb + (uint32_t)(E / be->cap) + 1;
    uint32_t* sched = sw.sched.as<uint32_t>((size_t)2 * (nb + 2) + (size_t)8 * max_tasks + TM_WORDS + 8);
    uint32_t* tcount = sched;
    uint32_t* toff = tcount + (nb + 2);
    uint32_t* task_start = toff + (nb + 2);
    uint32_t* task_len = task_start + max_tasks;
    uint32_t* task_dst = task_len + max_tasks;
    uint32_t* long_list = task_dst + max_tasks;
    uint32_t* tmeta = long_list + max_tasks;
    uint4* desc = reinterpret_cast<uint4*>((reinterpret_cast<uintptr_t>(tmeta + TM_WORDS) + 15) & ~(uintptr_t)15);
    if (!reuse) {
      ZKP_HIP(hipMemsetAsync(tmeta, 0, TM_WORDS * 4, st));
      hipLaunchKernelGGL(task_count_kernel, dim3((nb + 256) / 256), dim3(256), 0, st, start, end, nb, tcount, be->cap);
      exclusive_scan_u32(st, tcount, toff, (size_t)nb + 1, ws.scan_tmp2);
      static const uint32_t tnt = [] { const char* e = getenv("ZKP_TASK_NT"); const int v = e ? atoi(e) : 1024; return (uint32_t)(v >= 1024 ? 1024 : v >= 512 ? 512 : 256); }();
      hipLaunchKernelGGL(task_fill_kernel, dim3((nb + tnt - 1) / tnt), dim3(tnt), 0, st, start, end, toff, nb, task_start,
                         task_len, task_dst, long_list, tmeta, be->cap);
      hipLaunchKernelGGL(task_cursor_kernel, dim3(1), dim3(64), 0, st, tmeta);
      hipLaunchKernelGGL(task_order_kernel, dim3((max_tasks + tnt - 1) / tnt), dim3(tnt), 0, st, task_start, task_len, task_dst,
                         toff + nb, tmeta, desc);
      ZKP_HIP(hipEventRecord(ws.sorted, st));
      ctx->mark(st, ":sorted");
    }
    MsmWorkspace& bws = bucket_ws >= 0 ? ctx->cur->ws[bucket_ws] : ws;
    char* buckets = reinterpret_cast<char*>(bws.buckets.get((size_t)2 * nb * XB + XB));
    char* task_partial = reinterpret_cast<char*>(ws.partial.get((size_t)max_tasks * XB));
    static const bool zero_all = getenv("ZKP_MEMSET_BUCKETS") && atoi(getenv("ZKP_MEMSET_BUCKETS")) != 0;
    const uint32_t init = into >= 0 ? 1u : 0u;
    if (init) {
      ZKP_REQUIRE(bws.chain_nb == nb && bws.chain_xb == XB, ZKP_ERR_BAD_ARG);
      ZKP_HIP(hipStreamWaitEvent(st, bws.acc_done, 0));
    } else if (zero_all) ZKP_HIP(hipMemsetAsync(buckets, 0, (size_t)nb * XB, st));
    else hipLaunchKernelGGL(zero_empty_buckets_kernel, dim3((nb + 255) / 256), dim3(256), 0, st, start, end, nb, buckets, (uint32_t)XB);
    bws.chain_nb = 0;
    const bool timed = ms_accumulate && ctx->profiling;
    if (timed) ZKP_HIP(hipEventRecord(ctx->ev2, st));
    static const uint32_t force_redo = getenv("ZKP_DEBUG_FORCE_REDO") && atoi(getenv("ZKP_DEBUG_FORCE_REDO")) != 0 ? 2u : 0u;
    ctx->mark(st, ":acc0");
    vt->accumulate(st, be->table, sorted_vals, desc, toff + nb, max_tasks, buckets, task_partial,
                   ws.redo.as<uint32_t>((size_t)max_tasks + 1), init | force_redo);
    ctx->mark(st, ":acc1");
    if (timed) {
      ZKP_HIP(hipEventRecord(ctx->ev3, st));
      ZKP_HIP(hipEventSynchronize(ctx->ev3));
      ZKP_HIP(hipEventElapsedTime(ms_accumulate, ctx->ev2, ctx->ev3));
    }
    static const int dbg = [] { const char* e = getenv("ZKP_DEBUG_MSM"); return e ? atoi(e) : 0; }();
    if (dbg) {
      uint32_t* rep = ws.redo.as<uint32_t>((size_t)max_tasks + 1);
      ZKP_HIP(hipStreamSynchronize(st));
      ZKP_HIP(hipMemsetAsync(rep, 0, 32, st));
      hipLaunchKernelGGL(sched_check_kernel, dim3(256), dim3(256), 0, st, toff, long_list, tmeta, nb, max_tasks, rep);
      uint32_t h[8];
      ZKP_HIP(hipMemcpyAsync(h, rep, 32, hipMemcpyDeviceToHost, st));
      ZKP_HIP(hipStreamSynchronize(st));
      printf("[msm] group=%d n=%zu nb=%u max_tasks=%u: toff inversions=%u max tasks/bucket=%u bad long_list=%u n_long=%u n_tasks=%u overflow=%u\n",
             be->group, n, nb, max_tasks, h[0], h[1], h[2], h[3], h[4], h[5]);
      fflush(stdout);
    }
#ifdef ZKP_ABLATION
    if (dbg != 2)
#endif
      vt->combine(st, long_list, tmeta + TM_NLONG, toff, task_partial, buckets, init);
    if (dbg) {
      hipError_t e = hipStreamSynchronize(st);
      printf("[msm] combine: %s\n", hipGetErrorString(e));
      fflush(stdout);
    }
    if (n_entries) {
      *n_entries = E;
      if (ctx->profiling) {
        uint32_t emitted = 0;
        ZKP_HIP(hipMemcpyAsync(&emitted, offs + hist_n - 1, 4, hipMemcpyDeviceToHost, st));
        ZKP_HIP(hipStreamSynchronize(st));
        *n_entries = emitted;
      }
    }
    if (var) {
      VarPlan& vp = var_plan(ctx, c, K, st);
      uint32_t lvl_off = 0, cnt = nb;
      for (int l = 0; l < c - 1; l++) {
        vt->pair(st, buckets + (size_t)lvl_off * XB, buckets + (size_t)(lvl_off + cnt) * XB, cnt / 2);
        lvl_off += cnt;
        cnt /= 2;
      }
      const char* roots = buckets + (size_t)lvl_off * XB;
      char* partial = reinterpret_cast<char*>(ws.tmp.get(((size_t)vp.n1 + 256 + 8) * XB));
      char* R = partial + (size_t)vp.n1 * XB;
      vt->segsum_desc(st, buckets, vp.d1.as<SegDesc>(vp.n1), vp.n1, partial);
      vt->segsum_desc(st, partial, vp.d2.as<SegDesc>(256), 256, R);
      vt->final_var(st, R, roots, c, K, (char*)out_dev_xyzz, out_jac);
      ZKP_HIP(hipGetLastError());
      if (out_xyz_host) {
        ZKP_HIP(hipMemcpyAsync(out_xyz_host, out_jac, jac_words * 4, hipMemcpyDeviceToHost, st));
        ZKP_HIP(hipStreamSynchronize(st));
      }
      return;
    }
    if (defer) {
      bws.chain_nb = nb;
      bws.chain_xb = XB;
      ZKP_HIP(hipEventRecord(bws.acc_done, st));
      vt->write_identity(st, (char*)out_dev_xyzz, out_jac);
      ZKP_HIP(hipGetLastError());
      ZKP_REQUIRE(!out_xyz_host, ZKP_ERR_BAD_ARG);
      return;
    }
#ifdef ZKP_ABLATION
    if (ctx->dbg_skip_k8) return;
#endif
    const int L = c - 1;
    SegPlan plan{};
    plan.L = L;
    const uint32_t chunk = ctx->batch_mode ? SEG_CHUNK_BATCH : SEG_CHUNK;
    plan.chunk = chunk;
    uint32_t lvl_off = 0, cnt = nb, blocks = 0;
    static const bool fuse_seg = !(getenv("ZKP_PAIR_TOP_FUSE_SEG") && atoi(getenv("ZKP_PAIR_TOP_FUSE_SEG")) == 0);
    int l_top = -1;
    char* top_base = nullptr;
    uint32_t top_cnt = 0;
    for (int l = 0; l < L; l++) {
      uint32_t next_off = lvl_off + cnt;
      static const bool top_fused = !(getenv("ZKP_PAIR_TOP") && atoi(getenv("ZKP_PAIR_TOP")) == 0);
      static const uint32_t top_max = [] {
        const char* e = getenv("ZKP_PAIR_TOP_MAX");
        uint32_t v = e ? (uint32_t)atoi(e) : PAIR_TOP_MAX;
        if (v < 2) v = PAIR_TOP_MAX;
        while (v & (v - 1)) v &= v - 1;
        return v;
      }();
      if (!top_fused || cnt > top_max) vt->pair(st, buckets + (size_t)lvl_off * XB, buckets + (size_t)next_off * XB, cnt / 2);
      else if (cnt == top_max || l == 0) {
        if (fuse_seg && cnt / 2 <= chunk) {
          l_top = l;
          top_base = buckets + (size_t)lvl_off * XB;
          top_cnt = cnt;
        } else {
          vt->pair_top(st, buckets + (size_t)lvl_off * XB, cnt);
        }
      }
      plan.first_block[l] = blocks;
      plan.off[l] = lvl_off + 1;
      plan.stride[l] = 2;
      plan.count[l] = cnt / 2;
      blocks += (cnt / 2 + chunk - 1) / chunk;
      lvl_off = next_off;
      cnt /= 2;
    }
    plan.first_block[L] = blocks;
    const char* root = buckets + (size_t)lvl_off * XB;
    char* partial = reinterpret_cast<char*>(ws.tmp.get(((size_t)blocks + 64) * XB));
    char* Obuf = partial + (size_t)blocks * XB;
    if (L > 0 && l_top >= 0) {
      SegPlan low = plan;
      low.L = l_top;
      const uint32_t blocks_low = plan.first_block[l_top];
      vt->pair_top_segsum(st, top_base, top_cnt, buckets, &low, partial, blocks_low);
      SegPlan p2{};
      p2.L = L;
      p2.chunk = chunk;
      for (int l = 0; l < L; l++) {
        p2.first_block[l] = l;
        if (l < l_top) {
          p2.off[l] = plan.first_block[l];
          p2.stride[l] = 1;
          p2.count[l] = plan.first_block[l + 1] - plan.first_block[l];
        } else {
          p2.off[l] = plan.off[l];
          p2.stride[l] = plan.stride[l];
          p2.count[l] = plan.count[l];
        }
        ZKP_REQUIRE(p2.count[l] <= chunk, ZKP_ERR_BAD_ARG);
      }
      p2.first_block[L] = L;
      vt->segsum(st, partial, &p2, Obuf, L, buckets, l_top);
    } else if (L > 0) {
      vt->segsum(st, buckets, &plan, partial, blocks, nullptr, 1 << 30);
      SegPlan p2{};
      p2.L = L;
      p2.chunk = chunk;
      for (int l = 0; l < L; l++) {
        p2.first_block[l] = l;
        p2.off[l] = plan.first_block[l];
        p2.stride[l] = 1;
        p2.count[l] = plan.first_block[l + 1] - plan.first_block[l];
        ZKP_REQUIRE(p2.count[l] <= chunk, ZKP_ERR_BAD_ARG);
      }
      p2.first_block[L] = L;
      vt->segsum(st, partial, &p2, Obuf, L, nullptr, 1 << 30);
    }
    vt->final(st, Obuf, L, root, (char*)out_dev_xyzz, out_jac);
    ctx->mark(st, ":reduced");
  }
  ZKP_HIP(hipGetLastError());
  if (out_xyz_host) {
    ZKP_HIP(hipMemcpyAsync(out_xyz_host, out_jac, jac_words * 4, hipMemcpyDeviceToHost, st));
    ZKP_HIP(hipStreamSynchronize(st));
  }
}

void msm_run_multi(zkp_ctx* ctx, size_t count, const uint64_t* handles, const size_t* offsets,
                   const uint64_t* const* scalars_dev, const size_t* ns, bool montgomery, uint64_t* out_xyz_host,
                   size_t slot_words) {
  if (count == 0) return;
  const size_t jw = slot_words;
  zkp_lane* L = ctx->cur;
  if (ctx->pinned_cap < count * jw * 4) {
    if (ctx->pinned) (void)hipHostFree(ctx->pinned);
    ctx->pinned = nullptr;
    ctx->pinned_cap = 0;
    ZKP_HIP(hipHostMalloc(reinterpret_cast<void**>(&ctx->pinned), count * jw * 4 + 4096));
    ctx->pinned_cap = count * jw * 4 + 4096;
  }
  constexpr int NW = zkp_lane::N_WS_MSM;
  const int NL = std::max(1, std::min(ctx->cfg.msm_batch_lanes, (int)zkp_ctx::N_LANES));
  auto stream_of = [&](int li, int w) { return w == 0 ? ctx->lanes[li].stream : ctx->lanes[li].ws[w].stream; };
  struct Restore {
    zkp_ctx* c;
    zkp_lane* cur;
    int idx;
    ~Restore() {
      c->cur = cur;
      c->cur_idx = idx;
    }
  } restore{ctx, ctx->cur, ctx->cur_idx};
  ZKP_HIP(hipEventRecord(L->ev_fork, L->stream));
  for (int li = 0; li < NL; li++)
    for (int w = 0; w < NW; w++)
      if (stream_of(li, w) != L->stream) ZKP_HIP(hipStreamWaitEvent(stream_of(li, w), L->ev_fork, 0));
  for (size_t k = 0; k < count; k++) {
    const int li = (int)((k / NW) % NL), w = (int)(k % NW);
    auto be = get_bases(ctx, handles[k]);
    const size_t words = 3 * (size_t)be->vt->fN;
    ZKP_REQUIRE(words <= jw, ZKP_ERR_BAD_ARG);
    ZKP_REQUIRE(offsets[k] <= be->n, ZKP_ERR_BAD_ARG);
    const size_t n = std::min(ns[k], be->n - offsets[k]);
    ctx->cur = &ctx->lanes[li];
    ctx->cur_idx = li;
    msm_run(ctx, handles[k], offsets[k], scalars_dev[k], n, montgomery, nullptr, nullptr, nullptr, nullptr, w);
    ZKP_HIP(hipMemcpyAsync(ctx->pinned + k * jw, ctx->lanes[li].ws[w].out.p, words * 4, hipMemcpyDeviceToHost, stream_of(li, w)));
  }
  ctx->cur = restore.cur;
  ctx->cur_idx = restore.idx;
  for (int li = 0; li < NL; li++)
    for (int w = 0; w < NW; w++) {
      if (stream_of(li, w) == L->stream) continue;
      ZKP_HIP(hipEventRecord(ctx->lanes[li].ws[w].done, stream_of(li, w)));
      ZKP_HIP(hipStreamWaitEvent(L->stream, ctx->lanes[li].ws[w].done, 0));
    }
  ZKP_HIP(hipStreamSynchronize(L->stream));
  memcpy(out_xyz_host, ctx->pinned, count * jw * 4);
}

void msm_run_batch(zkp_ctx* ctx, uint64_t handle, size_t count, const size_t* offsets, const uint64_t* const* scalars_dev,
                   const size_t* ns, bool montgomery, uint64_t* out_xyz_host) {
  if (count == 0) return;
  std::vector<uint64_t> handles(count, handle);
  msm_run_multi(ctx, count, handles.data(), offsets, scalars_dev, ns, montgomery, out_xyz_host,
                3 * (size_t)get_bases(ctx, handle)->vt->fN);
}

void msm_var_run(zkp_ctx* ctx, int curve, int group, const uint64_t* xy_host, const uint8_t* inf_host,
                 const uint64_t* scalars_host, size_t n, bool montgomery, uint64_t* out_xyz_host) {
  BasesEntry e;
  e.curve = curve;
  e.group = group;
  e.vt = msm_vtbl(curve, group);
  e.n = n;
  e.var = true;
  e.owns = false;
  e.c = n >= 4096 ? 16 : 8;
  if (const char* env = getenv("ZKP_MSM_VAR_C")) {
    int c = atoi(env);
    if (c == 4 || c == 8 || c == 16) e.c = c;
  }
  e.W = 256 / e.c;
  e.wide = e.W;
  while ((1 << e.lgk) < e.W) e.lgk++;
  ZKP_REQUIRE((double)n * e.W < 2147483000.0, ZKP_ERR_BAD_ARG);
  hipStream_t st = ctx->cur->stream;
  const size_t ab = e.vt->aff_bytes;
  uint64_t* sdev = nullptr;
  if (n) {
    char* buf = reinterpret_cast<char*>(ctx->var_bases.get(n * ab + n + 64));
    e.table = buf;
    ZKP_HIP(hipMemcpyAsync(e.table, xy_host, n * ab, hipMemcpyHostToDevice, st));
    if (inf_host) {
      e.inf = reinterpret_cast<uint8_t*>(buf + n * ab);
      ZKP_HIP(hipMemcpyAsync(e.inf, inf_host, n, hipMemcpyHostToDevice, st));
    }
    sdev = ctx->msm_scalars.as<uint64_t>(n * 4);
    ZKP_HIP(hipMemcpyAsync(sdev, scalars_host, n * 32, hipMemcpyHostToDevice, st));
  }
  msm_run_entry(ctx, &e, 0, sdev, n, montgomery, out_xyz_host, nullptr, nullptr, nullptr, 0, -1, nullptr);
}

const MsmSmallVtbl* msm_small_vtbl_c01();
const MsmSmallVtbl* msm_small_vtbl_c02();
const MsmSmallVtbl* msm_small_vtbl_c11();
const MsmSmallVtbl* msm_small_vtbl_c12();
const MsmSmallVtbl* msm_small_vtbl(int curve, int group) {
  if (curve == ZKP_BN254 && group == 1) return msm_small_vtbl_c01();
  if (curve == ZKP_BN254 && group == 2) return msm_small_vtbl_c02();
  if (curve == ZKP_BLS12_381 && group == 1) return msm_small_vtbl_c11();
  if (curve == ZKP_BLS12_381 && group == 2) return msm_small_vtbl_c12();
  throw StatusError{ZKP_ERR_UNSUPPORTED_CURVE};
}

void msm_var_batch_run(zkp_ctx* ctx, int curve, int group, size_t count, const uint64_t* const* xy_dev,
                       const uint8_t* const* inf_dev, const uint64_t* const* scalars_dev, const size_t* ns, bool montgomery,
                       uint64_t* out_xyz_host) {
  const MsmSmallVtbl* vt = msm_small_vtbl(curve, group);
  const size_t cap = group == 1 ? ZKP_MSM_SMALL_MAX_G1 : ZKP_MSM_SMALL_MAX_G2;
  for (size_t k = 0; k < count; k++) {
    ZKP_REQUIRE(ns[k] <= cap, ZKP_ERR_BAD_ARG);
    if (ns[k] == 0) continue;
    ZKP_REQUIRE(xy_dev[k] && scalars_dev[k], ZKP_ERR_BAD_ARG);
    ZKP_REQUIRE(((uintptr_t)xy_dev[k] | (uintptr_t)scalars_dev[k]) % 16 == 0, ZKP_ERR_BAD_ARG);
  }
  if (count == 0) return;
  ZKP_REQUIRE(count <= ((size_t)1 << 24), ZKP_ERR_BAD_ARG);
  const bool c9_ok = !(curve == ZKP_BLS12_381 && group == 2);
  std::vector<SmallDesc> d(count);
  int c_max = 8;
  for (size_t k = 0; k < count; k++) {
    d[k].c = (c9_ok && ns[k] >= 8192) ? 9 : 8;
    c_max = std::max(c_max, (int)d[k].c);
  }
  uint32_t slice = 4096;
  while (small_lds_bytes(vt->bk_bytes, c_max, slice) > SMALL_LDS_MAX) slice >>= 1;
  auto grid = [&](uint32_t sl) {
    uint64_t total = 0;
    for (size_t k = 0; k < count; k++)
      if (ns[k]) total += (uint64_t)((256 + d[k].c) / d[k].c) * ((ns[k] + sl - 1) / sl);
    return total;
  };
  while (slice > 256 && grid(slice) < 2048) slice >>= 1;
  const uint64_t total_wg = grid(slice);
  ZKP_REQUIRE(total_wg < ((uint64_t)1 << 31), ZKP_ERR_BAD_ARG);
  uint32_t first = 0;
  for (size_t k = 0; k < count; k++) {
    SmallDesc& e = d[k];
// ... 162 lines not shown
```

ckb_zkp_amd/csrc/msm_group.hip:

```cpp
#include "bucket_dev.hpp"
#include "coop_dev.hpp"
#include "ec_dev.hpp"
#include "glv.hpp"
#include "msm_vtbl.hpp"

#ifndef ZKP_CFG_CURVE
#error "compile with -DZKP_CFG_CURVE=0|1 -DZKP_CFG_GROUP=1|2"
#endif

namespace zkp {

#if ZKP_CFG_CURVE == 0
using CfgFq = Bn254Fq;
using CfgFr = Bn254Fr;
constexpr int CFG_BITS = 254;
#else
using CfgFq = Bls381Fq;
using CfgFr = Bls381Fr;
constexpr int CFG_BITS = 255;
#endif
#if ZKP_CFG_GROUP == 1
using CfgF = Fp<CfgFq>;
#else
using CfgF = Fp2<CfgFq>;
#endif
#define ZKP_CAT3(a, b, c) a##b##c
#define ZKP_SYM(name, cu, gr) ZKP_CAT3(name, cu, gr)
#define ZKP_CFG_SYM(name) ZKP_SYM(name##_c, ZKP_CFG_CURVE, ZKP_CFG_GROUP)

namespace ZKP_CFG_SYM(cfg) {}
using namespace ZKP_CFG_SYM(cfg);

template <class F>
__global__ void ingest_kernel(char* table, const uint8_t* inf, size_t n) {
  size_t i = (size_t)blockIdx.x * blockDim.x + threadIdx.x;
  if (i >= n) return;
  if (inf && inf[i]) Affine<F>::inf().store(table + i * Affine<F>::BYTES);
}

template <class F>
__global__ __launch_bounds__(128) void precompute_kernel(char* table, size_t n, int c, int W, int wide) {
  size_t i = (size_t)blockIdx.x * blockDim.x + threadIdx.x;
  if (i >= n) return;
  Affine<F> p = Affine<F>::load(table + i * Affine<F>::BYTES);
  XYZZ<F> acc = XYZZ<F>::from_affine(p);
  for (int w = 1; w < W; w++) {
    const int cw = w - 1 < wide ? c : c - 1;
    for (int k = 0; k < cw; k++) acc = acc.dbl();
    Affine<F> a = acc.to_affine();
    a.store(table + ((size_t)w * n + i) * Affine<F>::BYTES);
    acc = XYZZ<F>::from_affine(a);
  }
}

template <class F>
__global__ __launch_bounds__(256) void pair_kernel(const char* __restrict__ in, char* __restrict__ out,
                                                   uint32_t count) {
  __builtin_amdgcn_s_setprio(3);
  uint32_t k = blockIdx.x * blockDim.x + threadIdx.x;
  if (k >= count) return;
  BkPoint<F>::add_mem(in + (size_t)(2 * k) * BkPoint<F>::BYTES, in + (size_t)(2 * k + 1) * BkPoint<F>::BYTES,
                      out + (size_t)k * BkPoint<F>::BYTES);
}

constexpr int PAIR_TOP_THREADS = 512;
template <class F>
__device__ __forceinline__ void pair_top_body(char* __restrict__ base, uint32_t cnt) {
  char* in = base;
  for (; cnt > 1; cnt >>= 1) {
    char* out = in + (size_t)cnt * BkPoint<F>::BYTES;
    bool coop = false;
    if constexpr (QuadCoop<F>::ON) coop = cnt / 2 <= PAIR_TOP_THREADS / 4;
    if constexpr (QuadCoop<F>::ON) {
      if (coop) {
        const uint32_t k = threadIdx.x >> 2;
        if (k < cnt / 2)
          quad_add_any<F>(in + (size_t)(2 * k) * BkPoint<F>::BYTES, in + (size_t)(2 * k + 1) * BkPoint<F>::BYTES,
                          out + (size_t)k * BkPoint<F>::BYTES, threadIdx.x & 3);
      }
    }
    if (!coop)
      for (uint32_t k = threadIdx.x; k < cnt / 2; k += PAIR_TOP_THREADS)
        BkPoint<F>::add_mem(in + (size_t)(2 * k) * BkPoint<F>::BYTES, in + (size_t)(2 * k + 1) * BkPoint<F>::BYTES,
                            out + (size_t)k * BkPoint<F>::BYTES);
    __threadfence_block();
    __syncthreads();
    in = out;
  }
}
template <class F>
__global__ __launch_bounds__(PAIR_TOP_THREADS) void pair_top_kernel(char* __restrict__ base, uint32_t cnt) {
  __builtin_amdgcn_s_setprio(3);
  pair_top_body<F>(base, cnt);
}

template <class F>
__device__ __forceinline__ void segsum_body(const char* __restrict__ base, const SegPlan& plan, char* __restrict__ partial, uint32_t block,
                                            const char* __restrict__ base_hi, int l_hi) {
  extern __shared__ __attribute__((aligned(16))) char smem[];
  const uint32_t t = threadIdx.x;
  const bool act = t < 256;
  int l = 0;
  while (l + 1 < plan.L && block >= plan.first_block[l + 1]) l++;
  if (l >= l_hi) base = base_hi;
  uint32_t chunk = block - plan.first_block[l];
  uint32_t lo = chunk * plan.chunk;
  uint32_t hi = min(plan.count[l], lo + plan.chunk);
  if constexpr (BkPoint<F>::MEM_ADD) {
    char* my = smem + (act ? t : 0) * BkPoint<F>::BYTES;
    if (act) {
      BkPoint<F>::inf().store(my);
      for (uint32_t i = lo + t; i < hi; i += 256)
        BkPoint<F>::add_mem(my, base + ((size_t)plan.off[l] + (size_t)i * plan.stride[l]) * BkPoint<F>::BYTES, my);
    }
    __syncthreads();
    for (int s = 128; s > 0; s >>= 1) {
      bool coop = false;
      if constexpr (QuadCoop<F>::ON) {
        coop = s <= 64;
        if (coop && (int)(t >> 2) < s) {
          char* mine = smem + (t >> 2) * BkPoint<F>::BYTES;
          quad_add_any<F>(mine, smem + ((t >> 2) + s) * BkPoint<F>::BYTES, mine, t & 3);
        }
      }
      if (!coop && (int)t < s) BkPoint<F>::add_mem(my, smem + (t + s) * BkPoint<F>::BYTES, my);
      __syncthreads();
    }
    if (t == 0) BkPoint<F>::copy_point(partial + (size_t)block * BkPoint<F>::BYTES, my);
    return;
  }
  BkPoint<F> acc = BkPoint<F>::inf();
  if (act) {
    for (uint32_t i = lo + t; i < hi; i += 256)
      acc.add(BkPoint<F>::load(base + ((size_t)plan.off[l] + (size_t)i * plan.stride[l]) * BkPoint<F>::BYTES));
    acc.store(smem + t * BkPoint<F>::BYTES);
  }
  __syncthreads();
  for (int s = 128; s > 0; s >>= 1) {
    if ((int)t < s) {
      BkPoint<F> o = BkPoint<F>::load(smem + (t + s) * BkPoint<F>::BYTES);
      if (!o.is_inf() || !acc.is_inf()) {
        acc.add(o);
        acc.store(smem + t * BkPoint<F>::BYTES);
      }
    }
    __syncthreads();
  }
  if (t == 0) acc.store(partial + (size_t)block * BkPoint<F>::BYTES);
}
template <class F>
__global__ __launch_bounds__(256) void segsum_kernel(const char* __restrict__ base, SegPlan plan, char* __restrict__ partial,
                                                     const char* __restrict__ base_hi, int l_hi) {
  __builtin_amdgcn_s_setprio(3);
  segsum_body<F>(base, plan, partial, blockIdx.x, base_hi, l_hi);
}
template <class F>
__global__ __launch_bounds__(PAIR_TOP_THREADS) void pair_top_segsum_kernel(char* __restrict__ top_base, uint32_t top_cnt,
                                                                           const char* __restrict__ base, SegPlan plan,
                                                                           char* __restrict__ partial) {
  __builtin_amdgcn_s_setprio(3);
  if (blockIdx.x == 0) {
    pair_top_body<F>(top_base, top_cnt);
    return;
  }
  segsum_body<F>(base, plan, partial, blockIdx.x - 1, nullptr, 1 << 30);
}

constexpr uint32_t COMBINE_SMALL = 32;
template <class F>
__global__ __launch_bounds__(256) void combine_small_kernel(const uint32_t* __restrict__ long_list,
                                                            const uint32_t* __restrict__ n_long_dev,
                                                            const uint32_t* __restrict__ toff,
                                                            const char* __restrict__ partial,
                                                            char* __restrict__ buckets, uint32_t init) {
  __builtin_amdgcn_s_setprio(3);
  const uint32_t n_long = *n_long_dev;
  for (uint32_t w = blockIdx.x * blockDim.x + threadIdx.x; w < n_long; w += gridDim.x * blockDim.x) {
    const uint32_t b = long_list[w];
    const uint32_t p0 = toff[b], p1 = toff[b + 1];
    if (p1 - p0 > COMBINE_SMALL) continue;
    BkPoint<F> acc = BkPoint<F>::load(partial + (size_t)p0 * BkPoint<F>::BYTES);
    for (uint32_t i = p0 + 1; i < p1; i++) acc.add(BkPoint<F>::load(partial + (size_t)i * BkPoint<F>::BYTES));
    if (init) acc.add(BkPoint<F>::load(buckets + (size_t)b * BkPoint<F>::BYTES));
    acc.store(buckets + (size_t)b * BkPoint<F>::BYTES);
  }
}

template <class F>
__global__ __launch_bounds__(256) void combine_kernel(const uint32_t* __restrict__ long_list,
                                                      const uint32_t* __restrict__ n_long_dev,
                                                      const uint32_t* __restrict__ toff,
                                                      const char* __restrict__ partial, char* __restrict__ buckets, uint32_t init) {
  extern __shared__ __attribute__((aligned(16))) char smem[];
  const int lane = threadIdx.x & 63;
  const uint32_t wv = __builtin_amdgcn_readfirstlane(threadIdx.x >> 6), nw = blockDim.x >> 6;
  char* my = smem + (size_t)wv * 64 * BkPoint<F>::BYTES;
  const uint32_t n_long = *n_long_dev;
  for (uint32_t w = blockIdx.x * nw + wv; w < n_long; w += gridDim.x * nw) {
    const uint32_t b = __builtin_amdgcn_readfirstlane(long_list[w]);
    const uint32_t p0 = __builtin_amdgcn_readfirstlane(toff[b]), p1 = __builtin_amdgcn_readfirstlane(toff[b + 1]);
    if (p1 - p0 <= COMBINE_SMALL) continue;
    BkPoint<F> acc = BkPoint<F>::inf();
    for (uint32_t i = p0 + lane; i < p1; i += 64) acc.add(BkPoint<F>::load(partial + (size_t)i * BkPoint<F>::BYTES));
    acc.store(my + lane * BkPoint<F>::BYTES);
    __builtin_amdgcn_fence(__ATOMIC_RELEASE, "wavefront");
    for (int s = 32; s > 0; s >>= 1) {
      __builtin_amdgcn_wave_barrier();
      if (lane < s) {
        BkPoint<F> o = BkPoint<F>::load(my + (lane + s) * BkPoint<F>::BYTES);
        if (!o.is_inf()) {
          acc.add(o);
          acc.store(my + lane * BkPoint<F>::BYTES);
        }
      }
      __builtin_amdgcn_fence(__ATOMIC_ACQ_REL, "wavefront");
    }
    if (lane == 0) {
      if (init) acc.add(BkPoint<F>::load(buckets + (size_t)b * BkPoint<F>::BYTES));
      acc.store(buckets + (size_t)b * BkPoint<F>::BYTES);
    }
    __builtin_amdgcn_fence(__ATOMIC_ACQ_REL, "wavefront");
    __builtin_amdgcn_wave_barrier();
  }
}

template <class F>
__global__ __launch_bounds__(128) void final_kernel(const char* __restrict__ O, int L, const char* __restrict__ root,
                                                   char* __restrict__ out_xyzz, uint32_t* __restrict__ out_jac) {
  __builtin_amdgcn_s_setprio(3);
  extern __shared__ __attribute__((aligned(16))) char smem[];
  int t = threadIdx.x;
  if constexpr (QuadCoop<F>::ON && QuadCoop<F>::GROUP == 1) {
    const int q = t >> 2, role = t & 3;
    char* my = smem + q * BkPoint<F>::BYTES;
    if (role == 0) {
      if (q < L) BkPoint<F>::copy_point(my, O + (size_t)q * BkPoint<F>::BYTES);
      else if (q == L) BkPoint<F>::copy_point(my, root);
      else BkPoint<F>::inf().store(my);
    }
    __syncthreads();
    if (q < L)
      for (int k = 0; k < q; k++) quad_dbl_mem<typename QuadCoop<F>::P>(my, my, role);
    __syncthreads();
    for (int s = 16; s > 0; s >>= 1) {
      if (q < s) quad_add_mem<typename QuadCoop<F>::P>(my, smem + (q + s) * BkPoint<F>::BYTES, my, role);
      __syncthreads();
    }
    if (t == 0) {
      const XYZZ<F> res = BkPoint<F>::load(my).to_sat();
      if (out_xyzz) res.store(out_xyzz);
      if (out_jac) res.store_jacobian(out_jac);
    }
    return;
  }
  if constexpr (BkPoint<F>::MEM_ADD) {
    char* my = smem + t * BkPoint<F>::BYTES;
    if (t < L) BkPoint<F>::copy_point(my, O + (size_t)t * BkPoint<F>::BYTES);
    else if (t == L) BkPoint<F>::copy_point(my, root);
    else BkPoint<F>::inf().store(my);
    if (t < L && !BkPoint<F>::load(my).is_inf())
      for (int k = 0; k < t; k++) BkPoint<F>::dbl_mem(my, my);
    __syncthreads();
    for (int s = 32; s > 0; s >>= 1) {
      bool coop = false;
      if constexpr (QuadCoop<F>::ON) {
        coop = s <= 16;
        if (coop && (t >> 2) < s) {
          char* mine = smem + (t >> 2) * BkPoint<F>::BYTES;
          quad_add_any<F>(mine, smem + ((t >> 2) + s) * BkPoint<F>::BYTES, mine, t & 3);
        }
      }
      if (!coop && t < s) BkPoint<F>::add_mem(my, smem + (t + s) * BkPoint<F>::BYTES, my);
      __syncthreads();
    }
    if (t == 0) {
      const XYZZ<F> res = BkPoint<F>::load(my).to_sat();
      if (out_xyzz) res.store(out_xyzz);
      if (out_jac) res.store_jacobian(out_jac);
    }
    return;
  }
  BkPoint<F> acc = BkPoint<F>::inf();
  if (t < L) {
    acc = BkPoint<F>::load(O + (size_t)t * BkPoint<F>::BYTES);
    for (int k = 0; k < t; k++) acc = acc.dbl();
  } else if (t == L) {
    acc = BkPoint<F>::load(root);
  }
  acc.store(smem + t * BkPoint<F>::BYTES);
  __syncthreads();
  for (int s = 32; s > 0; s >>= 1) {
    if (t < s) {
      BkPoint<F> o = BkPoint<F>::load(smem + (t + s) * BkPoint<F>::BYTES);
      if (!o.is_inf() || !acc.is_inf()) {
        acc.add(o);
        acc.store(smem + t * BkPoint<F>::BYTES);
      }
    }
    __syncthreads();
  }
  if (t == 0) {
    const XYZZ<F> res = acc.to_sat();
    if (out_xyzz) res.store(out_xyzz);
    if (out_jac) res.store_jacobian(out_jac);
  }
}

template <class F>
__global__ __launch_bounds__(256) void segsum_desc_kernel(const char* __restrict__ base, const SegDesc* __restrict__ descs,
                                                          char* __restrict__ out) {
  __builtin_amdgcn_s_setprio(3);
  extern __shared__ __attribute__((aligned(16))) char smem[];
  const SegDesc d = descs[blockIdx.x];
  BkPoint<F> acc = BkPoint<F>::inf();
  for (uint32_t i = threadIdx.x; i < d.count; i += 256)
    acc.add(BkPoint<F>::load(base + ((size_t)d.off + (size_t)i * d.stride) * BkPoint<F>::BYTES));
  acc.store(smem + threadIdx.x * BkPoint<F>::BYTES);
  __syncthreads();
// ... 413 lines not shown
  }
  XYZZ<F> r = L_inf[m] ? XYZZ<F>::inf() : XYZZ<F>::from_affine(Affine<F>::load(L_xy + m * Affine<F>::BYTES));
  r.add(acc.neg());
  r.to_affine().store(out_xy + m * Affine<F>::BYTES);
  out_inf[m] = r.is_inf() ? 1 : 0;
}
#endif

namespace ZKP_CFG_SYM(cfg) {
#if ZKP_CFG_GROUP == 1
template <class F>
__device__ __forceinline__ void jac_dbl(F& X, F& Y, F& Z) {
  F A = X.sqr(), B = Y.sqr();
  F C = B.sqr();
  F D = ((X + B).sqr() - A - C).dbl();
  F E = A.dbl() + A;
  F Fq = E.sqr();
  F Z3 = (Y * Z).dbl();
  X = Fq - D.dbl();
  Y = E * (D - X) - C.dbl().dbl().dbl();
  Z = Z3;
}
__global__ __launch_bounds__(128) void assemble_g1_part1_kernel(char* __restrict__ res, size_t slot,
                                                                const uint32_t* __restrict__ rs,
                                                                uint32_t* __restrict__ out,
                                                                uint32_t* __restrict__ flags) {
  using F = CfgF;
  using G = GlvConst<CfgFq>;
  __builtin_amdgcn_s_setprio(3);
  extern __shared__ __attribute__((aligned(16))) char smem[];
  constexpr int NB = G::BITS;
  constexpr size_t JB = 3 * 4 * F::N;
  const int t = threadIdx.x, chain = t >> 6, lane = t & 63;
  char* D = smem + (size_t)chain * NB * JB;
  char* red = smem + 2 * NB * JB + (size_t)chain * 64 * XYZZ<F>::BYTES;
  Fp<CfgFr> k = Fp<CfgFr>::load(rs + (chain == 0 ? 8 : 0)).from_mont();
  uint32_t k1[5], k2[5];
  int neg1, neg2;
  glv_decompose<G>(k.v, k1, &neg1, k2, &neg2);
  if (lane == 0) {
    XYZZ<F> p = XYZZ<F>::load(res + (size_t)chain * slot);
    F X, Y, Z;
    if (out) {
      Affine<F> a = p.to_affine();
      if (chain == 0) {
        a.store(out);
        flags[0] = p.is_inf() ? 1 : 0;
      }
      X = a.x, Y = a.y, Z = p.is_inf() ? F::zero() : F::one();
    } else {
      X = p.x * p.zz.sqr();
      Y = p.y * p.zzz.sqr();
      Z = p.is_inf() ? F::zero() : p.zzz;
    }
    for (int b = 0; b < NB; b++) {
      X.store(D + (size_t)b * JB);
      Y.store(D + (size_t)b * JB + 4 * F::N);
      Z.store(D + (size_t)b * JB + 8 * F::N);
      if (b + 1 < NB) jac_dbl(X, Y, Z);
    }
  }
  __syncthreads();
  F beta;
#pragma unroll
  for (int i = 0; i < F::N; i++) beta.v[i] = G::BETA_MONT[i];
  XYZZ<F> acc = XYZZ<F>::inf();
  for (int b = lane; b < NB; b += 64) {
    const bool t1 = (k1[b >> 5] >> (b & 31)) & 1, t2 = (k2[b >> 5] >> (b & 31)) & 1;
    if (!(t1 || t2)) continue;
    const F X = F::load(D + (size_t)b * JB), Y = F::load(D + (size_t)b * JB + 4 * F::N), Z = F::load(D + (size_t)b * JB + 8 * F::N);
    if (Z.is_zero()) continue;
    const F zz = Z.sqr();
    const F zzz = zz * Z;
    if (t1) acc.add(XYZZ<F>{X, neg1 ? Y.neg() : Y, zz, zzz});
    if (t2) acc.add(XYZZ<F>{beta * X, neg2 ? Y.neg() : Y, zz, zzz});
  }
  acc.store(red + (size_t)lane * XYZZ<F>::BYTES);
  __syncthreads();
  for (int s2 = 32; s2 > 0; s2 >>= 1) {
    if (lane < s2) {
      XYZZ<F> o = XYZZ<F>::load(red + (size_t)(lane + s2) * XYZZ<F>::BYTES);
      if (!o.is_inf() || !acc.is_inf()) {
        acc.add(o);
        acc.store(red + (size_t)lane * XYZZ<F>::BYTES);
      }
    }
    __syncthreads();
  }
  if (t == 0) {
    acc.add(XYZZ<F>::load(smem + 2 * NB * JB + 64 * XYZZ<F>::BYTES));
    acc.store(res + 5 * slot);
  }
}
__global__ __launch_bounds__(64) void assemble_g1_part2_kernel(char* __restrict__ res, size_t slot,
                                                               uint32_t* __restrict__ out,
                                                               uint32_t* __restrict__ flags, int c_off_words) {
  using F = CfgF;
  if (threadIdx.x || blockIdx.x) return;
  XYZZ<F> acc = XYZZ<F>::load(res + 5 * slot);
  acc.add(XYZZ<F>::load(res + 3 * slot));
  acc.add(XYZZ<F>::load(res + 4 * slot));
  if (!out) {
    acc.store(res + 5 * slot);
    return;
  }
  Affine<F> c = acc.to_affine();
  c.store(out + c_off_words);
  flags[2] = acc.is_inf() ? 1 : 0;
}
#else
__global__ __launch_bounds__(64) void assemble_g2_kernel(const char* __restrict__ res, size_t slot,
                                                         uint32_t* __restrict__ out, uint32_t* __restrict__ flags,
                                                         int out_off_words) {
  if (threadIdx.x || blockIdx.x) return;
  XYZZ<CfgF> p = XYZZ<CfgF>::load(res + 2 * slot);
  p.to_affine().store(out + out_off_words);
  flags[1] = p.is_inf() ? 1 : 0;
}
#endif
}

void ZKP_CFG_SYM(msm_accumulate_launch)(hipStream_t, const char*, const uint32_t*, const uint4*, const uint32_t*, uint32_t,
                                        char*, char*, uint32_t*, uint32_t);

namespace {
using F = CfgF;
constexpr size_t XB = XYZZ<F>::BYTES;
constexpr size_t BB = BkPoint<F>::BYTES;
void l_ingest(hipStream_t s, char* table, const uint8_t* inf, size_t n) {
  hipLaunchKernelGGL(ingest_kernel<F>, dim3((n + 255) / 256), dim3(256), 0, s, table, inf, n);
}
void l_precompute(hipStream_t s, char* table, size_t n, int c, int W, int wide) {
  hipLaunchKernelGGL(precompute_kernel<F>, dim3((n + 127) / 128), dim3(128), 0, s, table, n, c, W, wide);
}
void l_combine(hipStream_t s, const uint32_t* long_list, const uint32_t* n_long_dev, const uint32_t* toff,
               const char* partial, char* buckets, uint32_t init) {
  hipLaunchKernelGGL(combine_small_kernel<F>, dim3(256), dim3(256), 0, s, long_list, n_long_dev, toff, partial, buckets, init);
  hipLaunchKernelGGL(combine_kernel<F>, dim3(512), dim3(256), 256 * BB, s, long_list, n_long_dev, toff, partial, buckets, init);
}
void l_pair(hipStream_t s, const char* in, char* out, uint32_t count) {
  hipLaunchKernelGGL(pair_kernel<F>, dim3((count + 255) / 256), dim3(256), 0, s, in, out, count);
}
void l_pair_top(hipStream_t s, char* base, uint32_t count) {
  hipLaunchKernelGGL(pair_top_kernel<F>, dim3(1), dim3(PAIR_TOP_THREADS), 0, s, base, count);
}
void l_segsum(hipStream_t s, const char* base, const SegPlan* plan, char* partial, uint32_t blocks, const char* base_hi, int l_hi) {
  hipLaunchKernelGGL(segsum_kernel<F>, dim3(blocks), dim3(256), 256 * BB, s, base, *plan, partial, base_hi, l_hi);
}
void l_pair_top_segsum(hipStream_t s, char* top_base, uint32_t top_cnt, const char* base, const SegPlan* plan, char* partial,
                       uint32_t blocks) {
  hipLaunchKernelGGL(pair_top_segsum_kernel<F>, dim3(1 + blocks), dim3(PAIR_TOP_THREADS), 256 * BB, s, top_base, top_cnt, base, *plan,
                     partial);
}
void l_final(hipStream_t s, const char* O, int L, const char* root, char* out_xyzz, uint32_t* out_jac) {
  constexpr int threads = (QuadCoop<F>::ON && QuadCoop<F>::GROUP == 1) ? 128 : 64;
  hipLaunchKernelGGL(final_kernel<F>, dim3(1), dim3(threads), 64 * BB, s, O, L, root, out_xyzz, out_jac);
}
void l_identity(hipStream_t s, char* out_xyzz, uint32_t* out_jac) {
  hipLaunchKernelGGL(write_identity_kernel<F>, dim3(1), dim3(64), 0, s, out_xyzz, out_jac);
}
void l_fold(hipStream_t s, const uint32_t* pts, int k, uint32_t* out_jac) {
  hipLaunchKernelGGL(fold_kernel<F>, dim3(1), dim3(64), 0, s, pts, k, out_jac);
}
void l_segsum_desc(hipStream_t s, const char* base, const SegDesc* descs, uint32_t n_desc, char* out) {
  if (n_desc) hipLaunchKernelGGL(segsum_desc_kernel<F>, dim3(n_desc), dim3(256), 256 * BB, s, base, descs, out);
}
void l_final_var(hipStream_t s, const char* R, const char* roots, int c, int W, char* out_xyzz, uint32_t* out_jac) {
  hipLaunchKernelGGL(final_var_kernel<F>, dim3(1), dim3(256), 256 * BB, s, R, roots, c, W, out_xyzz, out_jac);
}
#if ZKP_CFG_GROUP == 1
void l_gfft(hipStream_t s, const char* xy, const uint8_t* inf, size_t n_in, const uint32_t* scal, const uint32_t* tw, uint32_t log_n,
            char* X, char* out_xy, uint8_t* out_inf) {
  const size_t N = (size_t)1 << log_n;
  hipLaunchKernelGGL((gfft_scale_kernel<F, CFG_BITS>), dim3((N + 127) / 128), dim3(128), 0, s, xy, inf, n_in, scal, log_n, X);
  for (uint32_t st = 1; st <= log_n; st++)
    hipLaunchKernelGGL((gfft_stage_kernel<F, CFG_BITS>), dim3((N / 2 + 127) / 128), dim3(128), 0, s, X, tw, log_n, st);
  hipLaunchKernelGGL(gfft_affine_kernel<F>, dim3((N + 127) / 128), dim3(128), 0, s, X, N, out_xy, out_inf);
}
void l_lfold(hipStream_t s, const char* L_xy, const uint8_t* L_inf, size_t n_vars, const uint32_t* col_ptr, const uint32_t* rows,
             const uint8_t* kind, const uint32_t* coeff, const char* G_xy, const uint8_t* G_inf, char* out_xy, uint8_t* out_inf) {
  if (n_vars)
    hipLaunchKernelGGL((lfold_kernel<F, CFG_BITS>), dim3((n_vars + 127) / 128), dim3(128), 0, s, L_xy, L_inf, n_vars, col_ptr, rows,
                       kind, coeff, G_xy, G_inf, out_xy, out_inf);
}
#endif
void l_fold_slots(hipStream_t s, const char* gathered, size_t rank_stride, int world, size_t slot, uint32_t mask,
                  char* res) {
  hipLaunchKernelGGL(fold_slots_kernel<F>, dim3(1), dim3(64), 0, s, gathered, rank_stride, world, slot, mask, res);
}
void l_into_affine(hipStream_t s, const uint32_t* jac, uint32_t* xy, uint32_t* inf) {
  hipLaunchKernelGGL(into_affine_kernel<F>, dim3(1), dim3(64), 0, s, jac, xy, inf);
}
void l_fold_affine_batch(hipStream_t s, const uint32_t* ja, const uint32_t* jb, const uint32_t* has_b, int k, uint32_t* xy,
                         uint32_t* inf) {
  if (k > 0) hipLaunchKernelGGL(fold_affine_batch_kernel<F>, dim3((k + 63) / 64), dim3(64), 0, s, ja, jb, has_b, k, xy, inf);
}
void l_decompress(hipStream_t s, const uint32_t* bytes, size_t n, const uint32_t* bcoef, char* xy, uint8_t* inf, uint32_t* status) {
  hipLaunchKernelGGL(curve_b_kernel<F>, dim3(1), dim3(64), 0, s, const_cast<uint32_t*>(bcoef));
  if (n) hipLaunchKernelGGL(decompress_kernel<F>, dim3((n + 63) / 64), dim3(64), 0, s, bytes, n, bcoef, xy, inf, status);
}
void l_compress(hipStream_t s, const char* xy, const uint8_t* inf, size_t n, uint32_t* bytes) {
  if (n) hipLaunchKernelGGL(compress_kernel<F>, dim3((n + 63) / 64), dim3(64), 0, s, xy, inf, n, bytes);
}
void l_subgroup_check(hipStream_t s, const char* xy, const uint8_t* inf, size_t n, const uint32_t* bcoef, uint32_t* status) {
  hipLaunchKernelGGL(curve_b_kernel<F>, dim3(1), dim3(64), 0, s, const_cast<uint32_t*>(bcoef));
  if (n) hipLaunchKernelGGL(subgroup_check_kernel<F>, dim3((n + 63) / 64), dim3(64), 0, s, xy, inf, n, bcoef, status);
}
void l_from_jacobian(hipStream_t s, const uint32_t* jac, char* out) {
  hipLaunchKernelGGL(from_jacobian_kernel<F>, dim3(1), dim3(64), 0, s, jac, out);
}
void l_fixed_base(hipStream_t s, const uint32_t* base, const uint32_t* scalars, size_t n, char* out_xy,
                  uint8_t* out_inf) {
  hipLaunchKernelGGL((fixed_base_kernel<F, CFG_BITS>), dim3((n + 127) / 128), dim3(128), 0, s, base, scalars, n,
                     out_xy, out_inf);
}
#if ZKP_CFG_GROUP == 1
void l_assemble_g1_p1(hipStream_t s, char* res, size_t slot, const uint32_t* rs, uint32_t* out, uint32_t* flags) {
  const size_t lds = 2 * (size_t)GlvConst<CfgFq>::BITS * 3 * 4 * F::N + 2 * 64 * XB;
  hipLaunchKernelGGL(assemble_g1_part1_kernel, dim3(1), dim3(128), lds, s, res, slot, rs, out, flags);
}
void l_assemble_g1_p2(hipStream_t s, char* res, size_t slot, uint32_t* out, uint32_t* flags, int c_off_words) {
  hipLaunchKernelGGL(assemble_g1_part2_kernel, dim3(1), dim3(64), 0, s, res, slot, out, flags, c_off_words);
}
#else
void l_assemble_g2(hipStream_t s, const char* res, size_t slot, uint32_t* out, uint32_t* flags, int off) {
  hipLaunchKernelGGL(assemble_g2_kernel, dim3(1), dim3(64), 0, s, res, slot, out, flags, off);
}
#endif
}

const MsmVtbl* ZKP_CFG_SYM(msm_vtbl)() {
  static const MsmVtbl v = {
      F::N, Affine<F>::BYTES, XYZZ<F>::BYTES, BkPoint<F>::BYTES, CFG_BITS,
      l_ingest, l_precompute, ZKP_CFG_SYM(msm_accumulate_launch), l_combine, l_pair, l_segsum, l_final, l_identity, l_fold,
      l_into_affine, l_fold_affine_batch, l_decompress, l_compress, l_subgroup_check, l_from_jacobian, l_fixed_base, l_segsum_desc, l_final_var, l_fold_slots,
#if ZKP_CFG_GROUP == 1
      l_assemble_g1_p1, l_assemble_g1_p2, nullptr,
#else
      nullptr, nullptr, l_assemble_g2,
#endif
      l_pair_top,
#if ZKP_CFG_GROUP == 1
      l_gfft, l_lfold,
#else
      nullptr, nullptr,
#endif
      l_pair_top_segsum,
  };
  return &v;
}

}
```

ckb_zkp_amd/csrc/msm_vtbl.hpp:

```cpp
#pragma once
#include <hip/hip_runtime.h>
#include <stddef.h>
#include <stdint.h>

namespace zkp {

constexpr int SEG_CHUNK = 1024;
constexpr int SEG_CHUNK_BATCH = 4096;
constexpr uint32_t MSM_TASK_CAP = 128;
struct SegPlan {
  int L;
  uint32_t chunk;
  uint32_t first_block[26];
  uint32_t off[25];
  uint32_t stride[25];
  uint32_t count[25];
};

struct SegDesc {
  uint32_t off, stride, count, out;
};

struct MsmVtbl {
  int fN;
  size_t aff_bytes, xyzz_bytes;
  size_t bucket_bytes;
  int scalar_bits;
  void (*ingest)(hipStream_t, char* table, const uint8_t* inf, size_t n);
  void (*precompute)(hipStream_t, char* table, size_t n, int c, int W, int wide);
  void (*accumulate)(hipStream_t, const char* table, const uint32_t* vals, const uint4* desc,
                     const uint32_t* n_tasks_dev, uint32_t max_tasks, char* buckets, char* partial, uint32_t* redo, uint32_t init);
  void (*combine)(hipStream_t, const uint32_t* long_list, const uint32_t* n_long_dev, const uint32_t* toff,
                  const char* partial, char* buckets, uint32_t init);
  void (*pair)(hipStream_t, const char* in, char* out, uint32_t count);
  void (*segsum)(hipStream_t, const char* base, const SegPlan* plan, char* partial, uint32_t blocks, const char* base_hi, int l_hi);
  void (*final)(hipStream_t, const char* O, int L, const char* root, char* out_xyzz, uint32_t* out_jac);
  void (*write_identity)(hipStream_t, char* out_xyzz, uint32_t* out_jac);
  void (*fold)(hipStream_t, const uint32_t* pts, int k, uint32_t* out_jac);
  void (*into_affine)(hipStream_t, const uint32_t* jac, uint32_t* xy, uint32_t* inf);
  void (*fold_affine_batch)(hipStream_t, const uint32_t* jac_a, const uint32_t* jac_b, const uint32_t* has_b, int k,
                            uint32_t* xy, uint32_t* inf);
  void (*decompress)(hipStream_t, const uint32_t* bytes, size_t n, const uint32_t* bcoef, char* xy, uint8_t* inf, uint32_t* status);
  void (*compress)(hipStream_t, const char* xy, const uint8_t* inf, size_t n, uint32_t* bytes);
  void (*subgroup_check)(hipStream_t, const char* xy, const uint8_t* inf, size_t n, const uint32_t* bcoef, uint32_t* status);
  void (*from_jacobian)(hipStream_t, const uint32_t* jac, char* out_xyzz);
  void (*fixed_base)(hipStream_t, const uint32_t* base, const uint32_t* scalars, size_t n, char* out_xy,
                     uint8_t* out_inf);
  void (*segsum_desc)(hipStream_t, const char* base, const SegDesc* descs, uint32_t n_desc, char* out);
  void (*final_var)(hipStream_t, const char* R, const char* roots, int c, int W, char* out_xyzz, uint32_t* out_jac);
  void (*fold_slots)(hipStream_t, const char* gathered, size_t rank_stride, int world, size_t slot, uint32_t mask,
                     char* res);
  void (*assemble_g1_part1)(hipStream_t, char* res, size_t slot, const uint32_t* rs, uint32_t* out, uint32_t* flags);
  void (*assemble_g1_part2)(hipStream_t, char* res, size_t slot, uint32_t* out, uint32_t* flags, int c_off_words);
  void (*assemble_g2)(hipStream_t, const char* res, size_t slot, uint32_t* out, uint32_t* flags, int out_off_words);
  void (*pair_top)(hipStream_t, char* base, uint32_t count);
  void (*gfft)(hipStream_t, const char* xy, const uint8_t* inf, size_t n_in, const uint32_t* scal, const uint32_t* tw, uint32_t log_n,
               char* X, char* out_xy, uint8_t* out_inf);
  void (*lfold)(hipStream_t, const char* L_xy, const uint8_t* L_inf, size_t n_vars, const uint32_t* col_ptr, const uint32_t* rows,
                const uint8_t* kind, const uint32_t* coeff, const char* G_xy, const uint8_t* G_inf, char* out_xy, uint8_t* out_inf);
  void (*pair_top_segsum)(hipStream_t, char* top_base, uint32_t top_cnt, const char* base, const SegPlan* plan, char* partial,
                          uint32_t blocks);
};
constexpr uint32_t PAIR_TOP_MAX = 2048;

const MsmVtbl* msm_vtbl(int curve, int group);

}
```

include/zkp_accel.h:

```cpp
#ifndef ZKP_ACCEL_H
#define ZKP_ACCEL_H
#include <stddef.h>
#include <stdint.h>
#ifdef __cplusplus
extern "C" {
#endif

typedef enum { ZKP_BN254 = 0, ZKP_BLS12_381 = 1 } zkp_curve_t;

typedef enum {
  ZKP_OK = 0,
  ZKP_ERR_BAD_ARG = -1,
  ZKP_ERR_UNSUPPORTED_CURVE = -2,
  ZKP_ERR_DOMAIN_TOO_LARGE = -3,
  ZKP_ERR_OOM = -4,
  ZKP_ERR_DEVICE = -5,
  ZKP_ERR_BAD_HANDLE = -6,
  ZKP_ERR_INVALID_POINT = -7
} zkp_status;

typedef enum { ZKP_NTT_FFT = 0, ZKP_NTT_IFFT = 1, ZKP_NTT_COSET_FFT = 2, ZKP_NTT_COSET_IFFT = 3 } zkp_ntt_op;

typedef struct zkp_ctx zkp_ctx;

// ... 136 lines not shown
} zkp_csr;

typedef struct {
  zkp_curve_t curve;
  uint32_t num_inputs;
  uint32_t num_aux;
  uint32_t num_constraints;
  zkp_csr at, bt, ct;
  const uint64_t* alpha_g1; const uint64_t* beta_g1; const uint64_t* delta_g1;
  const uint64_t* beta_g2; const uint64_t* delta_g2;
  const uint64_t* a_query; const uint8_t* a_inf; size_t a_len;
  const uint64_t* b_g1_query; const uint8_t* b_g1_inf; size_t b_g1_len;
  const uint64_t* b_g2_query; const uint8_t* b_g2_inf; size_t b_g2_len;
  const uint64_t* h_query; const uint8_t* h_inf; size_t h_len;
  const uint64_t* l_query; const uint8_t* l_inf; size_t l_len;
} zkp_groth16_pk_desc;

typedef struct zkp_groth16_pk zkp_groth16_pk;

int32_t zkp_groth16_pk_upload(zkp_ctx* ctx, const zkp_groth16_pk_desc* desc, zkp_groth16_pk** out);
#define ZKP_PK_KEEP_FORM 1u
int32_t zkp_groth16_pk_upload_ex(zkp_ctx* ctx, const zkp_groth16_pk_desc* desc, uint32_t flags, zkp_groth16_pk** out);
int32_t zkp_groth16_pk_free(zkp_ctx* ctx, zkp_groth16_pk* pk);

int32_t zkp_groth16_witness_map(zkp_ctx* ctx, zkp_groth16_pk* pk, const uint64_t* z_host, uint64_t* h_host);
int32_t zkp_groth16_witness_map_dev(zkp_ctx* ctx, zkp_groth16_pk* pk, const uint64_t* z_dev, uint64_t* h_dev);
int32_t zkp_groth16_domain_size(zkp_groth16_pk* pk, uint64_t* n);
int32_t zkp_groth16_pk_info(zkp_ctx* ctx, zkp_groth16_pk* pk, uint64_t info[8]);

int32_t zkp_groth16_prove(zkp_ctx* ctx, zkp_groth16_pk* pk, const uint64_t* z_host, const uint64_t* r,
                          const uint64_t* s, uint64_t* proof_out, uint8_t* inf_out);
int32_t zkp_groth16_prove_dev(zkp_ctx* ctx, zkp_groth16_pk* pk, const uint64_t* z_dev, const uint64_t* r,
                              const uint64_t* s, uint64_t* proof_out, uint8_t* inf_out);

int32_t zkp_groth16_prove_batch_dev(zkp_ctx* ctx, zkp_groth16_pk* pk, size_t n, const uint64_t* const* z_dev,
                                    const uint64_t* r, const uint64_t* s, uint64_t* proofs_out, uint8_t* inf_out);

int32_t zkp_groth16_prove_batch(zkp_ctx* ctx, zkp_groth16_pk* pk, size_t n, const uint64_t* const* z_host,
                                const uint64_t* r, const uint64_t* s, uint64_t* proofs_out, uint8_t* inf_out);

int32_t zkp_groth16_assemble(zkp_ctx* ctx, zkp_curve_t curve, const uint64_t* sums_xyz, const uint64_t* r,
                             const uint64_t* s, uint64_t* proof_out, uint8_t* inf_out);

int32_t zkp_groth16_pk_upload_shard(zkp_ctx* ctx, const zkp_groth16_pk_desc* desc, int32_t rank, int32_t world,
                                    zkp_groth16_pk** out);
int32_t zkp_groth16_partials_bytes(zkp_curve_t curve, size_t* bytes);
int32_t zkp_groth16_prove_partials_dev(zkp_ctx* ctx, zkp_groth16_pk* pk, const uint64_t* z_dev, const uint64_t* r,
                                       const uint64_t* s, void* partials_dev);
int32_t zkp_groth16_fold_assemble_dev(zkp_ctx* ctx, zkp_curve_t curve, const void* gathered_dev, int32_t world,
                                      const uint64_t* r, const uint64_t* s, uint64_t* proof_out, uint8_t* inf_out);

typedef struct zkp_groth16_pk_multi zkp_groth16_pk_multi;
typedef enum { ZKP_MULTI_SHARD = 0, ZKP_MULTI_REPLICATE = 1 } zkp_multi_mode;
int32_t zkp_ctx_create_multi(zkp_ctx** out, const int* device_ids, int n_devices);
int32_t zkp_ctx_create_multi_ex(zkp_ctx** out, const int* device_ids, int n_devices, const zkp_ctx_config* cfg);
int32_t zkp_ctx_num_devices(zkp_ctx* ctx, int32_t* n);
int32_t zkp_ctx_device(zkp_ctx* ctx, int32_t rank, zkp_ctx** member);
int32_t zkp_groth16_pk_upload_multi(zkp_ctx* ctx, const zkp_groth16_pk_desc* desc, int32_t mode,
                                    zkp_groth16_pk_multi** out);
int32_t zkp_groth16_pk_multi_free(zkp_ctx* ctx, zkp_groth16_pk_multi* pk);
int32_t zkp_groth16_multi_info(zkp_ctx* ctx, zkp_groth16_pk_multi* pk, uint64_t info[6]);
int32_t zkp_groth16_prove_multi(zkp_ctx* ctx, zkp_groth16_pk_multi* pk, const uint64_t* const* z, int32_t z_on_device,
                                const uint64_t* r, const uint64_t* s, uint64_t* proof_out, uint8_t* inf_out);
int32_t zkp_groth16_prove_batch_multi(zkp_ctx* ctx, zkp_groth16_pk_multi* pk, size_t count, const uint64_t* const* z,
                                      int32_t z_on_device, const uint64_t* r, const uint64_t* s, uint64_t* proofs_out,
                                      uint8_t* inf_out);

typedef struct zkp_fs_rng zkp_fs_rng;
int32_t zkp_fs_rng_new(const uint8_t* seed_material, size_t len, zkp_fs_rng** out);
int32_t zkp_fs_rng_free(zkp_fs_rng* rng);
int32_t zkp_fs_rng_absorb(zkp_fs_rng* rng, const uint8_t* material, size_t len);
int32_t zkp_fs_rng_seed(const zkp_fs_rng* rng, uint8_t out32[32]);
int32_t zkp_fs_rng_next_u64(zkp_fs_rng* rng, uint64_t* out);
int32_t zkp_fs_rng_rand_u128(zkp_fs_rng* rng, uint64_t out[2]);
int32_t zkp_fs_rng_rand_fr(zkp_fs_rng* rng, zkp_curve_t curve, uint64_t* out_mont);
int32_t zkp_fs_rng_sample_outside_domain(zkp_fs_rng* rng, zkp_curve_t curve, uint32_t log_domain, uint64_t* out_mont);
int32_t zkp_merlin_oneshot(const uint8_t* label, size_t label_len, const uint8_t* msg_label, size_t msg_label_len,
                           const uint8_t* msg, size_t msg_len, const uint8_t* chal_label, size_t chal_label_len,
                           uint8_t* out, size_t out_len);

typedef struct zkp_marlin_index zkp_marlin_index;
typedef struct {
  zkp_curve_t curve;
  uint32_t num_inputs;
  uint32_t n;
  uint32_t pad_aux;
  zkp_csr a, b, c;
} zkp_marlin_index_desc;
#define ZKP_MARLIN_NUM_EVALS 21
typedef struct {
  const uint64_t* w;
  const uint64_t* z_a;
  const uint64_t* z_b;
  const uint64_t* mask;
  int32_t mask_on_device;
  const uint64_t* blind_w;
  const uint64_t* blind_z_a;
  const uint64_t* blind_z_b;
  const uint64_t* blind_g_1;
  const uint64_t* blind_shifted_g_1;
} zkp_marlin_rand;
typedef struct {
  uint64_t comm[9 * 12];
  uint8_t comm_inf[9];
  uint64_t shifted[2 * 12];
  uint8_t shifted_inf[2];
  uint64_t evaluations[ZKP_MARLIN_NUM_EVALS * 4];
  uint32_t num_opening_proofs;
  uint64_t opening_w[2 * 12];
  uint8_t opening_w_inf[2];
  uint8_t opening_has_rand[2];
  uint64_t opening_rand_v[2 * 4];
  uint64_t challenges[7 * 4];
} zkp_marlin_proof;
int32_t zkp_marlin_index_upload(zkp_ctx* ctx, const zkp_marlin_index_desc* desc, zkp_marlin_index** out);
int32_t zkp_marlin_index_free(zkp_ctx* ctx, zkp_marlin_index* index);
int32_t zkp_marlin_index_info(const zkp_marlin_index* index, uint64_t info[6]);
int32_t zkp_marlin_index_commit(zkp_ctx* ctx, zkp_marlin_index* index, uint64_t powers_of_g, uint64_t* comms_xy,
                                uint8_t* inf);
int32_t zkp_marlin_prove(zkp_ctx* ctx, zkp_marlin_index* index, uint64_t powers_of_g, uint64_t powers_of_gamma_g,
                         const uint8_t* ivk_bytes, size_t ivk_len, const uint64_t* x, const uint64_t* w, size_t n_w,
                         const zkp_marlin_rand* rnd, const uint64_t* fixed_challenges, zkp_marlin_proof* out);

typedef struct {
  float ms_total;
  float ms_witness_map;
  float ms_msm[5];
  float ms_assemble;
  float ms_msm_accumulate;
  uint64_t msm_accumulate_launches;
  uint64_t msm_points;
  float ms_msm_scan;
  uint64_t msm_scan_launches;
  uint64_t msm_scan_bytes;
  float ms_msm_acc[5];
  uint64_t msm_entries[5];
} zkp_groth16_timing;
int32_t zkp_groth16_last_timing(zkp_ctx* ctx, zkp_groth16_timing* out);
typedef struct {
  double ms_round[3];
  double ms_commit[3];
  double ms_evaluations;
  double ms_open;
  double ms_total;
  uint64_t commit_points;
  uint64_t open_points;
  uint64_t ntt_count;
  uint64_t ntt_elements;
} zkp_marlin_timing;
int32_t zkp_marlin_last_timing(zkp_ctx* ctx, zkp_marlin_timing* out);
int32_t zkp_set_profiling(zkp_ctx* ctx, int32_t enable);
int32_t zkp_bench_mulmod(zkp_ctx* ctx, zkp_curve_t curve, int32_t field, int32_t unsaturated, double* gmulmod_per_s);
int32_t zkp_bench_hbm_copy(zkp_ctx* ctx, size_t bytes, double* gbytes_per_s);

#ifdef __cplusplus
}
#endif
#endif
```

rust/zkp-accel/src/ffi.rs:

```rust
#![allow(non_camel_case_types, clippy::too_many_arguments)]
use std::os::raw::{c_char, c_int, c_void};

#[repr(C)]
pub struct zkp_ctx {
    _p: [u8; 0],
}
#[repr(C)]
pub struct zkp_groth16_pk {
    _p: [u8; 0],
}
#[repr(C)]
pub struct zkp_groth16_pk_multi {
    _p: [u8; 0],
}
#[repr(C)]
pub struct zkp_fs_rng {
    _p: [u8; 0],
}
#[repr(C)]
pub struct zkp_marlin_index {
    _p: [u8; 0],
}

pub const ZKP_BN254: c_int = 0;
// ... 118 lines not shown
#[repr(C)]
pub struct zkp_marlin_proof {
    pub comm: [u64; 108],
    pub comm_inf: [u8; 9],
    pub shifted: [u64; 24],
    pub shifted_inf: [u8; 2],
    pub evaluations: [u64; 84],
    pub num_opening_proofs: u32,
    pub opening_w: [u64; 24],
    pub opening_w_inf: [u8; 2],
    pub opening_has_rand: [u8; 2],
    pub opening_rand_v: [u64; 8],
    pub challenges: [u64; 28],
}

#[repr(C)]
#[derive(Clone, Copy)]
pub struct zkp_groth16_timing {
    pub ms_total: f32,
    pub ms_witness_map: f32,
    pub ms_msm: [f32; 5],
    pub ms_assemble: f32,
    pub ms_msm_accumulate: f32,
    pub msm_accumulate_launches: u64,
    pub msm_points: u64,
    pub ms_msm_scan: f32,
    pub msm_scan_launches: u64,
    pub msm_scan_bytes: u64,
    pub ms_msm_acc: [f32; 5],
    pub msm_entries: [u64; 5],
}

#[repr(C)]
pub struct zkp_marlin_timing {
    pub ms_round: [f64; 3],
    pub ms_commit: [f64; 3],
    pub ms_evaluations: f64,
    pub ms_open: f64,
    pub ms_total: f64,
    pub commit_points: u64,
    pub open_points: u64,
    pub ntt_count: u64,
    pub ntt_elements: u64,
}

extern "C" {
    pub fn zkp_status_string(status: i32) -> *const c_char;
    pub fn zkp_version() -> *const c_char;
    pub fn zkp_ctx_create(out: *mut *mut zkp_ctx, device_id: c_int) -> i32;
    pub fn zkp_ctx_create_ex(out: *mut *mut zkp_ctx, device_id: c_int, cfg: *const zkp_ctx_config) -> i32;
    pub fn zkp_ctx_get_config(ctx: *mut zkp_ctx, out: *mut zkp_ctx_config) -> i32;
    pub fn zkp_ctx_destroy(ctx: *mut zkp_ctx) -> i32;
    pub fn zkp_ctx_set_stream(ctx: *mut zkp_ctx, hip_stream: *mut c_void) -> i32;
    pub fn zkp_ctx_sync(ctx: *mut zkp_ctx) -> i32;
    pub fn zkp_dev_alloc(ctx: *mut zkp_ctx, bytes: usize, dptr: *mut *mut c_void) -> i32;
    pub fn zkp_dev_free(ctx: *mut zkp_ctx, dptr: *mut c_void) -> i32;
    pub fn zkp_h2d(ctx: *mut zkp_ctx, dst_dev: *mut c_void, src_host: *const c_void, bytes: usize) -> i32;
    pub fn zkp_d2h(ctx: *mut zkp_ctx, dst_host: *mut c_void, src_dev: *const c_void, bytes: usize) -> i32;
    pub fn zkp_timer_start(ctx: *mut zkp_ctx) -> i32;
    pub fn zkp_timer_stop_ms(ctx: *mut zkp_ctx, ms: *mut f32) -> i32;
    pub fn zkp_ntt(ctx: *mut zkp_ctx, curve: c_int, data_host: *mut u64, log_n: u32, op: i32) -> i32;
    pub fn zkp_ntt_dev(ctx: *mut zkp_ctx, curve: c_int, data_dev: *mut u64, log_n: u32, op: i32) -> i32;
    pub fn zkp_fr_vec_op_dev(ctx: *mut zkp_ctx, curve: c_int, op: i32, a: *const u64, b: *const u64, k_host: *const u64, out: *mut u64, n: usize) -> i32;
    pub fn zkp_fr_spmv_dev(ctx: *mut zkp_ctx, curve: c_int, row_ptr_dev: *const u32, col_dev: *const u32, coeff_dev: *const u64, nrows: usize, x_dev: *const u64, out_dev: *mut u64) -> i32;
    pub fn zkp_fr_gather_dev(ctx: *mut zkp_ctx, in_dev: *const u64, idx_dev: *const i32, n: usize, out_dev: *mut u64) -> i32;
    pub fn zkp_poly_divide_by_vanishing_dev(ctx: *mut zkp_ctx, curve: c_int, p_dev: *const u64, len: usize, n: usize, q_dev: *mut u64, rem_dev: *mut u64) -> i32;
    pub fn zkp_d2d(ctx: *mut zkp_ctx, dst_dev: *mut c_void, src_dev: *const c_void, bytes: usize) -> i32;
    pub fn zkp_dev_zero(ctx: *mut zkp_ctx, dst_dev: *mut c_void, bytes: usize) -> i32;
    pub fn zkp_fr_batch_inverse_dev(ctx: *mut zkp_ctx, curve: c_int, v: *mut u64, n: usize) -> i32;
    pub fn zkp_poly_evaluate_dev(ctx: *mut zkp_ctx, curve: c_int, p: *const u64, n: usize, z_host: *const u64, eval_out_host: *mut u64) -> i32;
    pub fn zkp_poly_div_linear_dev(ctx: *mut zkp_ctx, curve: c_int, p: *const u64, n: usize, z_host: *const u64, q_dev: *mut u64, eval_out_host: *mut u64) -> i32;
    pub fn zkp_bases_upload_g1(ctx: *mut zkp_ctx, curve: c_int, xy: *const u64, inf: *const u8, n: usize, handle: *mut u64) -> i32;
    pub fn zkp_bases_upload_g2(ctx: *mut zkp_ctx, curve: c_int, xy: *const u64, inf: *const u8, n: usize, handle: *mut u64) -> i32;
    pub fn zkp_bases_free(ctx: *mut zkp_ctx, handle: u64) -> i32;
    pub fn zkp_bases_share(dst: *mut zkp_ctx, src: *mut zkp_ctx, src_handle: u64, dst_handle: *mut u64) -> i32;
    pub fn zkp_bases_len(ctx: *mut zkp_ctx, handle: u64, n: *mut usize) -> i32;
    pub fn zkp_msm_g1(ctx: *mut zkp_ctx, handle: u64, offset: usize, scalars_host: *const u64, n: usize, out_xyz: *mut u64) -> i32;
    pub fn zkp_msm_g2(ctx: *mut zkp_ctx, handle: u64, offset: usize, scalars_host: *const u64, n: usize, out_xyz: *mut u64) -> i32;
    pub fn zkp_msm_g1_dev(ctx: *mut zkp_ctx, handle: u64, offset: usize, scalars_dev: *const u64, n: usize, out_xyz_host: *mut u64) -> i32;
    pub fn zkp_msm_g2_dev(ctx: *mut zkp_ctx, handle: u64, offset: usize, scalars_dev: *const u64, n: usize, out_xyz_host: *mut u64) -> i32;
    pub fn zkp_vartime_multiscalar_mul_g1(ctx: *mut zkp_ctx, handle: u64, fr_scalars_host: *const u64, n: usize, out_xyz: *mut u64) -> i32;
    pub fn zkp_vartime_multiscalar_mul_g2(ctx: *mut zkp_ctx, handle: u64, fr_scalars_host: *const u64, n: usize, out_xyz: *mut u64) -> i32;
    pub fn zkp_msm_g1_var(ctx: *mut zkp_ctx, curve: c_int, xy_host: *const u64, inf_host: *const u8, scalars_host: *const u64, n: usize, montgomery: i32, out_xyz: *mut u64) -> i32;
    pub fn zkp_msm_g2_var(ctx: *mut zkp_ctx, curve: c_int, xy_host: *const u64, inf_host: *const u8, scalars_host: *const u64, n: usize, montgomery: i32, out_xyz: *mut u64) -> i32;
    pub fn zkp_msm_g1_var_batch_dev(ctx: *mut zkp_ctx, curve: c_int, count: usize, xy_dev: *const *const u64, inf_dev: *const *const u8, scalars_dev: *const *const u64, ns: *const usize, montgomery: i32, out_xyz: *mut u64) -> i32;
    pub fn zkp_msm_g2_var_batch_dev(ctx: *mut zkp_ctx, curve: c_int, count: usize, xy_dev: *const *const u64, inf_dev: *const *const u8, scalars_dev: *const *const u64, ns: *const usize, montgomery: i32, out_xyz: *mut u64) -> i32;
    pub fn zkp_g1_ipa_fold_dev(ctx: *mut zkp_ctx, curve: c_int, l_xy: *const u64, l_inf: *const u8, r_xy: *const u64, r_inf: *const u8, n: usize, a_host: *const u64, b_host: *const u64, out_xy: *mut u64, out_inf: *mut u8) -> i32;
    pub fn zkp_fr_dot_batch_dev(ctx: *mut zkp_ctx, curve: c_int, count: usize, a_dev: *const *const u64, b_dev: *const *const u64, ns: *const usize, out_host: *mut u64) -> i32;
    pub fn zkp_fr_sumcheck_round_dev(ctx: *mut zkp_ctx, curve: c_int, kind: i32, count: usize, tables_dev: *mut *mut u64, len: usize, bind_host: *const u64, evals_out_host: *mut u64) -> i32;
    pub fn zkp_fr_eq_evals_dev(ctx: *mut zkp_ctx, curve: c_int, r_host: *const u64, k: usize, out_dev: *mut u64) -> i32;
    pub fn zkp_fr_product_circuit_dev(ctx: *mut zkp_ctx, curve: c_int, count: usize, circuits_dev: *mut *mut u64, n: usize, roots_host: *mut u64) -> i32;
    pub fn zkp_fr_memcheck_circuits_dev(ctx: *mut zkp_ctx, curve: c_int, count: usize, addr_dev: *const *const u32, val_dev: *const *const u64, ts_dev: *const *const u32, ts_add: *const u32, circuits_dev: *mut *mut u64, n: usize, gamma1_host: *const u64, gamma2_host: *const u64, roots_host: *mut u64) -> i32;
    pub fn zkp_msm_g1_mont_dev(ctx: *mut zkp_ctx, handle: u64, offset: usize, fr_scalars_dev: *const u64, n: usize, out_xyz_host: *mut u64) -> i32;
    pub fn zkp_msm_g2_mont_dev(ctx: *mut zkp_ctx, handle: u64, offset: usize, fr_scalars_dev: *const u64, n: usize, out_xyz_host: *mut u64) -> i32;
    pub fn zkp_msm_g1_mont_batch_dev(ctx: *mut zkp_ctx, bases_handle: u64, count: usize, offsets: *const usize, scalars_dev: *const *const u64, ns: *const usize, out_xyz: *mut u64) -> i32;
    pub fn zkp_msm_mont_multi_dev(ctx: *mut zkp_ctx, count: usize, bases_handles: *const u64, offsets: *const usize, scalars_dev: *const *const u64, ns: *const usize, out_xyz: *mut u64, slot_u64: usize) -> i32;
    pub fn zkp_g1_fold(ctx: *mut zkp_ctx, curve: c_int, xyz_host: *const u64, k: usize, out_xyz: *mut u64) -> i32;
    pub fn zkp_g2_fold(ctx: *mut zkp_ctx, curve: c_int, xyz_host: *const u64, k: usize, out_xyz: *mut u64) -> i32;
    pub fn zkp_g1_into_affine(ctx: *mut zkp_ctx, curve: c_int, xyz_host: *const u64, xy_out: *mut u64, inf_out: *mut u8) -> i32;
    pub fn zkp_g2_into_affine(ctx: *mut zkp_ctx, curve: c_int, xyz_host: *const u64, xy_out: *mut u64, inf_out: *mut u8) -> i32;
    pub fn zkp_groth16_points_into_affine(curve: c_int, a_xyzz: *const u64, b_xyzz: *const u64, c_xyzz: *const u64, proof_out: *mut u64, inf_out: *mut u8) -> i32;
    pub fn zkp_g1_decompress(ctx: *mut zkp_ctx, curve: c_int, bytes: *const u8, n: usize, xy_out: *mut u64, inf_out: *mut u8, bad_index: *mut usize) -> i32;
    pub fn zkp_g2_decompress(ctx: *mut zkp_ctx, curve: c_int, bytes: *const u8, n: usize, xy_out: *mut u64, inf_out: *mut u8, bad_index: *mut usize) -> i32;
    pub fn zkp_g1_compress(ctx: *mut zkp_ctx, curve: c_int, xy: *const u64, inf: *const u8, n: usize, bytes_out: *mut u8) -> i32;
    pub fn zkp_g2_compress(ctx: *mut zkp_ctx, curve: c_int, xy: *const u64, inf: *const u8, n: usize, bytes_out: *mut u8) -> i32;
    pub fn zkp_g1_subgroup_check(ctx: *mut zkp_ctx, curve: c_int, xy: *const u64, inf: *const u8, n: usize, bad_index: *mut usize) -> i32;
    pub fn zkp_g2_subgroup_check(ctx: *mut zkp_ctx, curve: c_int, xy: *const u64, inf: *const u8, n: usize, bad_index: *mut usize) -> i32;
    pub fn zkp_fixed_base_mul_g1(ctx: *mut zkp_ctx, curve: c_int, base_xy: *const u64, scalars_host: *const u64, n: usize, out_xy: *mut u64, out_inf: *mut u8) -> i32;
    pub fn zkp_fixed_base_mul_g2(ctx: *mut zkp_ctx, curve: c_int, base_xy: *const u64, scalars_host: *const u64, n: usize, out_xy: *mut u64, out_inf: *mut u8) -> i32;
    pub fn zkp_groth16_pk_upload(ctx: *mut zkp_ctx, desc: *const zkp_groth16_pk_desc, out: *mut *mut zkp_groth16_pk) -> i32;
    pub fn zkp_groth16_pk_upload_ex(ctx: *mut zkp_ctx, desc: *const zkp_groth16_pk_desc, flags: u32, out: *mut *mut zkp_groth16_pk) -> i32;
    pub fn zkp_groth16_pk_free(ctx: *mut zkp_ctx, pk: *mut zkp_groth16_pk) -> i32;
    pub fn zkp_groth16_witness_map(ctx: *mut zkp_ctx, pk: *mut zkp_groth16_pk, z_host: *const u64, h_host: *mut u64) -> i32;
    pub fn zkp_groth16_witness_map_dev(ctx: *mut zkp_ctx, pk: *mut zkp_groth16_pk, z_dev: *const u64, h_dev: *mut u64) -> i32;
    pub fn zkp_groth16_domain_size(pk: *mut zkp_groth16_pk, n: *mut u64) -> i32;
    pub fn zkp_groth16_pk_info(ctx: *mut zkp_ctx, pk: *mut zkp_groth16_pk, info: *mut u64) -> i32;
    pub fn zkp_groth16_prove(ctx: *mut zkp_ctx, pk: *mut zkp_groth16_pk, z_host: *const u64, r: *const u64, s: *const u64, proof_out: *mut u64, inf_out: *mut u8) -> i32;
    pub fn zkp_groth16_prove_dev(ctx: *mut zkp_ctx, pk: *mut zkp_groth16_pk, z_dev: *const u64, r: *const u64, s: *const u64, proof_out: *mut u64, inf_out: *mut u8) -> i32;
    pub fn zkp_groth16_prove_batch_dev(ctx: *mut zkp_ctx, pk: *mut zkp_groth16_pk, n: usize, z_dev: *const *const u64, r: *const u64, s: *const u64, proofs_out: *mut u64, inf_out: *mut u8) -> i32;
    pub fn zkp_groth16_prove_batch(ctx: *mut zkp_ctx, pk: *mut zkp_groth16_pk, n: usize, z_host: *const *const u64, r: *const u64, s: *const u64, proofs_out: *mut u64, inf_out: *mut u8) -> i32;
    pub fn zkp_groth16_assemble(ctx: *mut zkp_ctx, curve: c_int, sums_xyz: *const u64, r: *const u64, s: *const u64, proof_out: *mut u64, inf_out: *mut u8) -> i32;
    pub fn zkp_groth16_pk_upload_shard(ctx: *mut zkp_ctx, desc: *const zkp_groth16_pk_desc, rank: i32, world: i32, out: *mut *mut zkp_groth16_pk) -> i32;
    pub fn zkp_groth16_partials_bytes(curve: c_int, bytes: *mut usize) -> i32;
    pub fn zkp_groth16_prove_partials_dev(ctx: *mut zkp_ctx, pk: *mut zkp_groth16_pk, z_dev: *const u64, r: *const u64, s: *const u64, partials_dev: *mut c_void) -> i32;
    pub fn zkp_groth16_fold_assemble_dev(ctx: *mut zkp_ctx, curve: c_int, gathered_dev: *const c_void, world: i32, r: *const u64, s: *const u64, proof_out: *mut u64, inf_out: *mut u8) -> i32;
    pub fn zkp_ctx_create_multi(out: *mut *mut zkp_ctx, device_ids: *const c_int, n_devices: c_int) -> i32;
    pub fn zkp_ctx_create_multi_ex(out: *mut *mut zkp_ctx, device_ids: *const c_int, n_devices: c_int, cfg: *const zkp_ctx_config) -> i32;
    pub fn zkp_ctx_num_devices(ctx: *mut zkp_ctx, n: *mut i32) -> i32;
    pub fn zkp_ctx_device(ctx: *mut zkp_ctx, rank: i32, member: *mut *mut zkp_ctx) -> i32;
    pub fn zkp_groth16_pk_upload_multi(ctx: *mut zkp_ctx, desc: *const zkp_groth16_pk_desc, mode: i32, out: *mut *mut zkp_groth16_pk_multi) -> i32;
    pub fn zkp_groth16_pk_multi_free(ctx: *mut zkp_ctx, pk: *mut zkp_groth16_pk_multi) -> i32;
    pub fn zkp_groth16_multi_info(ctx: *mut zkp_ctx, pk: *mut zkp_groth16_pk_multi, info: *mut u64) -> i32;
    pub fn zkp_groth16_prove_multi(ctx: *mut zkp_ctx, pk: *mut zkp_groth16_pk_multi, z: *const *const u64, z_on_device: i32, r: *const u64, s: *const u64, proof_out: *mut u64, inf_out: *mut u8) -> i32;
    pub fn zkp_groth16_prove_batch_multi(ctx: *mut zkp_ctx, pk: *mut zkp_groth16_pk_multi, count: usize, z: *const *const u64, z_on_device: i32, r: *const u64, s: *const u64, proofs_out: *mut u64, inf_out: *mut u8) -> i32;
    pub fn zkp_fs_rng_new(seed_material: *const u8, len: usize, out: *mut *mut zkp_fs_rng) -> i32;
    pub fn zkp_fs_rng_free(rng: *mut zkp_fs_rng) -> i32;
    pub fn zkp_fs_rng_absorb(rng: *mut zkp_fs_rng, material: *const u8, len: usize) -> i32;
    pub fn zkp_fs_rng_seed(rng: *const zkp_fs_rng, out32: *mut u8) -> i32;
    pub fn zkp_fs_rng_next_u64(rng: *mut zkp_fs_rng, out: *mut u64) -> i32;
    pub fn zkp_fs_rng_rand_u128(rng: *mut zkp_fs_rng, out: *mut u64) -> i32;
    pub fn zkp_fs_rng_rand_fr(rng: *mut zkp_fs_rng, curve: c_int, out_mont: *mut u64) -> i32;
    pub fn zkp_fs_rng_sample_outside_domain(rng: *mut zkp_fs_rng, curve: c_int, log_domain: u32, out_mont: *mut u64) -> i32;
    pub fn zkp_merlin_oneshot(label: *const u8, label_len: usize, msg_label: *const u8, msg_label_len: usize, msg: *const u8, msg_len: usize, chal_label: *const u8, chal_label_len: usize, out: *mut u8, out_len: usize) -> i32;
    pub fn zkp_marlin_index_upload(ctx: *mut zkp_ctx, desc: *const zkp_marlin_index_desc, out: *mut *mut zkp_marlin_index) -> i32;
    pub fn zkp_marlin_index_free(ctx: *mut zkp_ctx, index: *mut zkp_marlin_index) -> i32;
    pub fn zkp_marlin_index_info(index: *const zkp_marlin_index, info: *mut u64) -> i32;
    pub fn zkp_marlin_index_commit(ctx: *mut zkp_ctx, index: *mut zkp_marlin_index, powers_of_g: u64, comms_xy: *mut u64, inf: *mut u8) -> i32;
    pub fn zkp_marlin_prove(ctx: *mut zkp_ctx, index: *mut zkp_marlin_index, powers_of_g: u64, powers_of_gamma_g: u64, ivk_bytes: *const u8, ivk_len: usize, x: *const u64, w: *const u64, n_w: usize, rnd: *const zkp_marlin_rand, fixed_challenges: *const u64, out: *mut zkp_marlin_proof) -> i32;
    pub fn zkp_groth16_last_timing(ctx: *mut zkp_ctx, out: *mut zkp_groth16_timing) -> i32;
    pub fn zkp_marlin_last_timing(ctx: *mut zkp_ctx, out: *mut zkp_marlin_timing) -> i32;
    pub fn zkp_set_profiling(ctx: *mut zkp_ctx, enable: i32) -> i32;
    pub fn zkp_bench_mulmod(ctx: *mut zkp_ctx, curve: c_int, field: i32, unsaturated: i32, gmulmod_per_s: *mut f64) -> i32;
    pub fn zkp_bench_hbm_copy(ctx: *mut zkp_ctx, bytes: usize, gbytes_per_s: *mut f64) -> i32;
}
```

Baseline: 137.9 proofs/s.

## Use single-pass chained scan, fuse task counting, and fuse bucket pair-reduction levels

Replaces the three-kernel reduce/scan/apply exclusive scan with a single-pass decoupled-lookback chained scan that resets its own state. Task counting and empty-bucket zeroing are folded into the scan's load functor, and the cursor kernel is folded into task_order. The explicit memsets go away and so do several launches. It also adds a pair_fused kernel that collapses three bucket pairing levels into one launch, plus a debug scan entry point. The cost is spin-waiting on global status flags and more complex level planning in the reduction.

```diff
diff --git a/ckb_zkp_amd/_lib.py b/ckb_zkp_amd/_lib.py
--- a/ckb_zkp_amd/_lib.py
+++ b/ckb_zkp_amd/_lib.py
@@ -211,6 +211,7 @@
     "zkp_merlin_oneshot": (C.c_int32, [vp, C.c_size_t, vp, C.c_size_t, vp, C.c_size_t, vp, C.c_size_t, vp, C.c_size_t]),
     "zkp_bench_mulmod": (C.c_int32, [vp, C.c_int, C.c_int32, C.c_int32, C.POINTER(C.c_double)]),
     "zkp_bench_hbm_copy": (C.c_int32, [vp, C.c_size_t, C.POINTER(C.c_double)]),
+    "zkp_debug_exclusive_scan_u32": (C.c_int32, [vp, vp, C.c_size_t, vp]),
 }
 
 _lib = None
diff --git a/ckb_zkp_amd/csrc/capi.hip b/ckb_zkp_amd/csrc/capi.hip
--- a/ckb_zkp_amd/csrc/capi.hip
+++ b/ckb_zkp_amd/csrc/capi.hip
@@ -748,6 +748,10 @@
   if (!out) return ZKP_ERR_BAD_ARG;
   return guarded(ctx, [&] { *out = bench_hbm_copy(ctx, bytes); });
 }
+int32_t zkp_debug_exclusive_scan_u32(zkp_ctx* ctx, const uint32_t* in, size_t n, uint32_t* out) {
+  if (n && (!in || !out)) return ZKP_ERR_BAD_ARG;
+  return guarded(ctx, [&] { debug_exclusive_scan_u32(ctx, in, n, out); });
+}
 int32_t zkp_marlin_last_timing(zkp_ctx* ctx, zkp_marlin_timing* out) {
   if (!ctx || !out) return ZKP_ERR_BAD_ARG;
   return guarded(ctx, [&] { *out = ctx->last_marlin_timing; });
diff --git a/ckb_zkp_amd/csrc/internal.hpp b/ckb_zkp_amd/csrc/internal.hpp
--- a/ckb_zkp_amd/csrc/internal.hpp
+++ b/ckb_zkp_amd/csrc/internal.hpp
@@ -55,6 +55,7 @@
 void msm_var_batch_run(zkp_ctx* ctx, int curve, int group, size_t count, const uint64_t* const* xy_dev,
                        const uint8_t* const* inf_dev, const uint64_t* const* scalars_dev, const size_t* ns, bool montgomery,
                        uint64_t* out_xyz_host);
+void debug_exclusive_scan_u32(zkp_ctx* ctx, const uint32_t* in_host, size_t n, uint32_t* out_host);
 void msm_free_all(zkp_ctx* ctx);
 void bases_drop(zkp_ctx* ctx, uint64_t handle);
 void point_fold(zkp_ctx* ctx, int curve, int group, const uint64_t* xyz_host, size_t k, uint64_t* out_xyz_host);
diff --git a/ckb_zkp_amd/csrc/msm.hip b/ckb_zkp_amd/csrc/msm.hip
--- a/ckb_zkp_amd/csrc/msm.hip
+++ b/ckb_zkp_amd/csrc/msm.hip
@@ -241,84 +241,6 @@
 }
 
 
-constexpr int SCAN_CHUNK = 2048;
-__global__ __launch_bounds__(256) void scan_reduce_kernel(const uint32_t* __restrict__ in, size_t n,
-                                                          uint32_t* __restrict__ sums) {
-  ZKP_SORT_PRIO();
-  __shared__ uint32_t red[256];
-  size_t base = (size_t)blockIdx.x * SCAN_CHUNK;
-  uint32_t acc = 0;
-  for (int k = 0; k < SCAN_CHUNK / 256; k++) {
-    size_t i = base + (size_t)k * 256 + threadIdx.x;
-    if (i < n) acc += in[i];
-  }
-  red[threadIdx.x] = acc;
-  __syncthreads();
-  for (int s = 128; s > 0; s >>= 1) {
-    if ((int)threadIdx.x < s) red[threadIdx.x] += red[threadIdx.x + s];
-    __syncthreads();
-  }
-  if (threadIdx.x == 0) sums[blockIdx.x] = red[0];
-}
-__global__ __launch_bounds__(1024) void scan_sums_kernel(uint32_t* __restrict__ sums, size_t m) {
-  ZKP_SORT_PRIO();
-  __shared__ uint32_t buf[1024];
-  uint32_t carry = 0;
-  for (size_t t0 = 0; t0 < m; t0 += 1024) {
-    size_t i = t0 + threadIdx.x;
-    uint32_t v = i < m ? sums[i] : 0;
-    buf[threadIdx.x] = v;
-    __syncthreads();
-    for (int d = 1; d < 1024; d <<= 1) {
-      uint32_t add = (int)threadIdx.x >= d ? buf[threadIdx.x - d] : 0;
-      __syncthreads();
-      buf[threadIdx.x] += add;
-      __syncthreads();
-    }
-    if (i < m) sums[i] = carry + buf[threadIdx.x] - v;
-    uint32_t total = buf[1023];
-    __syncthreads();
-    carry += total;
-  }
-}
-__global__ __launch_bounds__(256) void scan_apply_kernel(const uint32_t* __restrict__ in, size_t n,
-                                                         const uint32_t* __restrict__ sums,
-                                                         uint32_t* __restrict__ out) {
-  ZKP_SORT_PRIO();
-  __shared__ uint32_t part[256];
-  size_t base = (size_t)blockIdx.x * SCAN_CHUNK;
-  constexpr int PER = SCAN_CHUNK / 256;
-  uint32_t v[PER];
-  uint32_t acc = 0;
-  for (int k = 0; k < PER; k++) {
-    size_t i = base + (size_t)threadIdx.x * PER + k;
-    v[k] = i < n ? in[i] : 0;
-    acc += v[k];
-  }
-  part[threadIdx.x] = acc;
-  __syncthreads();
-  for (int d = 1; d < 256; d <<= 1) {
-    uint32_t add = (int)threadIdx.x >= d ? part[threadIdx.x - d] : 0;
-    __syncthreads();
-    part[threadIdx.x] += add;
-    __syncthreads();
-  }
-  uint32_t run = sums[blockIdx.x] + part[threadIdx.x] - acc;
-  for (int k = 0; k < PER; k++) {
-    size_t i = base + (size_t)threadIdx.x * PER + k;
-    if (i < n) out[i] = run;
-    run += v[k];
-  }
-}
-static void exclusive_scan_u32(hipStream_t st, const uint32_t* in, uint32_t* out, size_t n, DevBuf& tmp) {
-  if (n == 0) return;
-  size_t chunks = (n + SCAN_CHUNK - 1) / SCAN_CHUNK;
-  uint32_t* sums = tmp.as<uint32_t>(chunks + 1);
-  hipLaunchKernelGGL(scan_reduce_kernel, dim3(chunks), dim3(256), 0, st, in, n, sums);
-  hipLaunchKernelGGL(scan_sums_kernel, dim3(1), dim3(1024), 0, st, sums, chunks);
-  hipLaunchKernelGGL(scan_apply_kernel, dim3(chunks), dim3(256), 0, st, in, n, sums, out);
-}
-
 constexpr int SORT_H1_MAX = 13;
 constexpr uint32_t SORT_BIN_TARGET = 16384;
 constexpr int SORT_L_MAX = 13;
@@ -406,6 +328,94 @@
   *total = tmp[NT / 64];
   __syncthreads();
   return res;
+}
+
+constexpr int SCAN_TILE = 2048, SCAN_PER = SCAN_TILE / 256;
+constexpr unsigned long long SCAN_AGG = 1ull << 32, SCAN_INCL = 2ull << 32;
+struct ScanState {
+  uint32_t* hdr;
+  unsigned long long* status;
+};
+struct PlainLoad {
+  const uint32_t* in;
+  size_t n_in;
+  __device__ __forceinline__ void prologue(uint32_t) const {}
+  __device__ __forceinline__ uint32_t operator()(size_t i) const { return i < n_in ? in[i] : 0; }
+};
+template <class Load>
+__global__ __launch_bounds__(256, 8) void scan_chained_kernel(Load load, size_t n, uint32_t* __restrict__ out, ScanState stt,
+                                                           uint32_t ntiles) {
+  ZKP_SORT_PRIO();
+  __shared__ uint32_t s_tile, s_prefix, s_last;
+  __shared__ uint32_t tmp[256 / 64 + 1];
+  const uint32_t t = threadIdx.x, lane = t & 63u;
+  if (t == 0) s_tile = atomicAdd(&stt.hdr[0], 1u);
+  __syncthreads();
+  const uint32_t tile = s_tile;
+  if (tile >= ntiles) return;
+  load.prologue(tile);
+  const size_t base = (size_t)tile * SCAN_TILE + (size_t)t * SCAN_PER;
+  uint32_t v[SCAN_PER];
+  uint32_t acc = 0;
+#pragma unroll
+  for (int k = 0; k < SCAN_PER; k++) {
+    v[k] = base + k < n ? load(base + k) : 0;
+    acc += v[k];
+  }
+  uint32_t total;
+  uint32_t run = block_excl_scan<256>(acc, tmp, &total);
+  if (t < 64) {
+    if (t == 0 && tile > 0)
+      __hip_atomic_store(&stt.status[tile], SCAN_AGG | total, __ATOMIC_RELAXED, __HIP_MEMORY_SCOPE_AGENT);
+    uint32_t prefix = 0;
+    for (int64_t j0 = (int64_t)tile - 1; j0 >= 0; j0 -= 64) {
+      const int64_t j = j0 - (int64_t)lane;
+      unsigned long long w = SCAN_INCL;
+      if (j >= 0) {
+        w = __hip_atomic_load(&stt.status[j], __ATOMIC_RELAXED, __HIP_MEMORY_SCOPE_AGENT);
+        while ((w >> 32) == 0) {
+          __builtin_amdgcn_s_sleep(2);
+          w = __hip_atomic_load(&stt.status[j], __ATOMIC_RELAXED, __HIP_MEMORY_SCOPE_AGENT);
+        }
+      }
+      const uint64_t incl = __ballot((w >> 32) == 2);
+      const uint32_t first = incl ? (uint32_t)__ffsll((unsigned long long)incl) - 1u : 64u;
+      uint32_t part = lane <= first ? (uint32_t)w : 0;
+#pragma unroll
+      for (int d = 32; d > 0; d >>= 1) part += (uint32_t)__shfl_xor((int)part, d, 64);
+      prefix += part;
+      if (incl) break;
+    }
+    if (t == 0) {
+      __hip_atomic_store(&stt.status[tile], SCAN_INCL | (uint32_t)(prefix + total), __ATOMIC_RELAXED, __HIP_MEMORY_SCOPE_AGENT);
+      s_prefix = prefix;
+      __threadfence();
+      s_last = atomicAdd(&stt.hdr[1], 1u) == ntiles - 1;
+    }
+  }
+  __syncthreads();
+  run += s_prefix;
+#pragma unroll
+  for (int k = 0; k < SCAN_PER; k++) {
+    if (base + k < n) out[base + k] = run;
+    run += v[k];
+  }
+  if (s_last) {
+    __threadfence();
+    for (uint32_t i = t; i < ntiles; i += 256) stt.status[i] = 0;
+    if (t == 0) stt.hdr[0] = stt.hdr[1] = 0;
+  }
+}
+template <class Load>
+static void exclusive_scan_u32(hipStream_t st, Load load, uint32_t* out, size_t n, DevBuf& tmp) {
+  if (n == 0) return;
+  const size_t tiles = (n + SCAN_TILE - 1) / SCAN_TILE, bytes = 16 + 8 * tiles;
+  if (tmp.cap < bytes) {
+    tmp.get(bytes);
+    ZKP_HIP(hipMemsetAsync(tmp.p, 0, tmp.cap, st));
+  }
+  ScanState stt{reinterpret_cast<uint32_t*>(tmp.p), reinterpret_cast<unsigned long long*>(reinterpret_cast<char*>(tmp.p) + 16)};
+  hipLaunchKernelGGL(scan_chained_kernel<Load>, dim3((uint32_t)tiles), dim3(256), 0, st, load, n, out, stt, (uint32_t)tiles);
 }
 
 __device__ __forceinline__ uint32_t wave_agg_inc(uint32_t* cnt, uint32_t idx, bool active) {
@@ -581,23 +591,37 @@
 
 constexpr int TM_NLONG = 0, TM_HIST = 1, TM_CUR = 256, TM_WORDS = 512;
 
-__global__ void task_count_kernel(const uint32_t* __restrict__ start, const uint32_t* __restrict__ end, uint32_t nb,
-                                  uint32_t* __restrict__ tcount, uint32_t cap) {
-  ZKP_SORT_PRIO();
-  uint32_t b = blockIdx.x * blockDim.x + threadIdx.x;
-  if (b > nb) return;
-  tcount[b] = b < nb ? (end[b] - start[b] + cap - 1) / cap : 0;
-}
-
+__device__ __forceinline__ void zero_bucket(char* __restrict__ buckets, uint32_t b, uint32_t xb) {
+  uint4* p = reinterpret_cast<uint4*>(buckets + (size_t)b * xb);
+  for (uint32_t k = 0; k < xb / 16; k++) p[k] = make_uint4(0, 0, 0, 0);
+}
 __global__ __launch_bounds__(256) void zero_empty_buckets_kernel(const uint32_t* __restrict__ start,
                                                                  const uint32_t* __restrict__ end, uint32_t nb,
                                                                  char* __restrict__ buckets, uint32_t xb) {
   ZKP_SORT_PRIO();
   const uint32_t b = blockIdx.x * blockDim.x + threadIdx.x;
   if (b >= nb || end[b] != start[b]) return;
-  uint4* p = reinterpret_cast<uint4*>(buckets + (size_t)b * xb);
-  for (uint32_t k = 0; k < xb / 16; k++) p[k] = make_uint4(0, 0, 0, 0);
-}
+  zero_bucket(buckets, b, xb);
+}
+struct TaskCountLoad {
+  const uint32_t* start;
+  const uint32_t* end;
+  uint32_t nb, cap;
+  char* buckets;
+  uint32_t xb;
+  uint32_t* tmeta;
+  __device__ __forceinline__ void prologue(uint32_t tile) const {
+    if (tile == 0)
+      for (uint32_t i = threadIdx.x; i < (uint32_t)TM_WORDS; i += blockDim.x) tmeta[i] = 0;
+  }
+  __device__ __forceinline__ uint32_t operator()(size_t i) const {
+    const uint32_t b = (uint32_t)i;
+    if (b >= nb) return 0;
+    const uint32_t len = end[b] - start[b];
+    if (buckets && len == 0) zero_bucket(buckets, b, xb);
+    return (len + cap - 1) / cap;
+  }
+};
 
 __global__ __launch_bounds__(1024) void task_fill_kernel(const uint32_t* __restrict__ start,
                                                         const uint32_t* __restrict__ end,
@@ -629,16 +653,6 @@
     if (hist[i]) atomicAdd(&tmeta[TM_HIST + i], hist[i]);
 }
 
-__global__ void task_cursor_kernel(uint32_t* tmeta) {
-  ZKP_SORT_PRIO();
-  if (threadIdx.x || blockIdx.x) return;
-  uint32_t acc = 0;
-  for (int l = MSM_TASK_CAP; l >= 0; l--) {
-    tmeta[TM_CUR + l] = acc;
-    acc += tmeta[TM_HIST + l];
-  }
-}
-
 __global__ __launch_bounds__(1024) void task_order_kernel(const uint32_t* __restrict__ task_start,
                                                          const uint32_t* __restrict__ task_len,
                                                          const uint32_t* __restrict__ task_dst,
@@ -647,8 +661,18 @@
   ZKP_SORT_PRIO();
   __shared__ uint32_t cnt[MSM_TASK_CAP + 1];
   __shared__ uint32_t base[MSM_TASK_CAP + 1];
+  __shared__ uint32_t first[256];
+  static_assert(MSM_TASK_CAP + 1 <= 256, "one wave-scan pass over the length histogram");
   for (int i = threadIdx.x; i <= (int)MSM_TASK_CAP; i += blockDim.x) cnt[i] = 0;
-  __syncthreads();
+  if (threadIdx.x < 256) first[threadIdx.x] = threadIdx.x <= MSM_TASK_CAP ? tmeta[TM_HIST + threadIdx.x] : 0;
+  __syncthreads();
+  for (int d = 1; d < 256; d <<= 1) {
+    uint32_t add = 0;
+    if (threadIdx.x < 256 && threadIdx.x + d < 256) add = first[threadIdx.x + d];
+    __syncthreads();
+    if (threadIdx.x < 256) first[threadIdx.x] += add;
+    __syncthreads();
+  }
   uint32_t t = blockIdx.x * blockDim.x + threadIdx.x;
   const bool live = t < *n_tasks_dev;
   uint32_t l = 0, rank = 0;
@@ -658,7 +682,7 @@
   }
   __syncthreads();
   for (int i = threadIdx.x; i <= (int)MSM_TASK_CAP; i += blockDim.x)
-    if (cnt[i]) base[i] = atomicAdd(&tmeta[TM_CUR + i], cnt[i]);
+    if (cnt[i]) base[i] = (i < 255 ? first[i + 1] : 0) + atomicAdd(&tmeta[TM_CUR + i], cnt[i]);
   __syncthreads();
   if (live) desc[base[l] + rank] = make_uint4(task_start[t], l, task_dst[t], t);
 }
@@ -677,6 +701,19 @@
     rep[4] = n_tasks;
     rep[5] = n_tasks > max_tasks;
   }
+}
+
+void debug_exclusive_scan_u32(zkp_ctx* ctx, const uint32_t* in_host, size_t n, uint32_t* out_host) {
+  if (n == 0) return;
+  hipStream_t st = ctx->cur->stream;
+  DevBuf buf;
+  uint32_t* in = buf.as<uint32_t>(2 * n);
+  uint32_t* out = in + n;
+  ZKP_HIP(hipMemcpyAsync(in, in_host, n * 4, hipMemcpyHostToDevice, st));
+  exclusive_scan_u32(st, PlainLoad{in, n}, out, n, ctx->cur->ws[0].scan_tmp);
+  ZKP_HIP(hipGetLastError());
+  ZKP_HIP(hipMemcpyAsync(out_host, out, n * 4, hipMemcpyDeviceToHost, st));
+  ZKP_HIP(hipStreamSynchronize(st));
 }
 
 static void msm_run_entry(zkp_ctx* ctx, const BasesEntry* be, size_t offset, const uint64_t* scalars_dev, size_t n,
@@ -822,8 +859,6 @@
       if (sort_src != ws_idx) ZKP_HIP(hipStreamWaitEvent(st, sw.sorted, 0));
     } else if (l1_reuse) {
       if (l1_src != ws_idx) ZKP_HIP(hipStreamWaitEvent(st, lw.l1_done, 0));
-    } else {
-      ZKP_HIP(hipMemsetAsync(hist + hist_n - 1, 0, 4, st));
     }
     const uint8_t* grp = scan_inf == be->sort_inf ? be->group_flags : nullptr;
     static const bool staged_on = !(getenv("ZKP_SORT_STAGED") && atoi(getenv("ZKP_SORT_STAGED")) == 0);
@@ -850,7 +885,7 @@
         if (nt_hist >= 1024) hist_l(std::integral_constant<int, 1024>{});
         else if (nt_hist >= 512) hist_l(std::integral_constant<int, 512>{});
         else hist_l(std::integral_constant<int, 256>{});
-        exclusive_scan_u32(st, hist, offs, hist_n, ws.scan_tmp);
+        exclusive_scan_u32(st, PlainLoad{hist, hist_n - 1}, offs, hist_n, ws.scan_tmp);
         if (staged_sub) {
           auto scat_l = [&](auto nt) {
             constexpr int NT = decltype(nt)::value;
@@ -880,38 +915,36 @@
                          kv, offs, nblocks, LB, vals, start, end, (l1_reuse || grp) ? be->filter_bit : -1);
     uint32_t* const sorted_vals = vals;
     const uint32_t max_tasks = nb + (uint32_t)(E / be->cap) + 1;
-    uint32_t* sched = sw.sched.as<uint32_t>((size_t)2 * (nb + 2) + (size_t)8 * max_tasks + TM_WORDS + 8);
-    uint32_t* tcount = sched;
-    uint32_t* toff = tcount + (nb + 2);
+    uint32_t* sched = sw.sched.as<uint32_t>((size_t)(nb + 2) + (size_t)8 * max_tasks + TM_WORDS + 8);
+    uint32_t* toff = sched;
     uint32_t* task_start = toff + (nb + 2);
     uint32_t* task_len = task_start + max_tasks;
     uint32_t* task_dst = task_len + max_tasks;
     uint32_t* long_list = task_dst + max_tasks;
     uint32_t* tmeta = long_list + max_tasks;
     uint4* desc = reinterpret_cast<uint4*>((reinterpret_cast<uintptr_t>(tmeta + TM_WORDS) + 15) & ~(uintptr_t)15);
-    if (!reuse) {
-      ZKP_HIP(hipMemsetAsync(tmeta, 0, TM_WORDS * 4, st));
-      hipLaunchKernelGGL(task_count_kernel, dim3((nb + 256) / 256), dim3(256), 0, st, start, end, nb, tcount, be->cap);
-      exclusive_scan_u32(st, tcount, toff, (size_t)nb + 1, ws.scan_tmp2);
-      static const uint32_t tnt = [] { const char* e = getenv("ZKP_TASK_NT"); const int v = e ? atoi(e) : 1024; return (uint32_t)(v >= 1024 ? 1024 : v >= 512 ? 512 : 256); }();
-      hipLaunchKernelGGL(task_fill_kernel, dim3((nb + tnt - 1) / tnt), dim3(tnt), 0, st, start, end, toff, nb, task_start,
-                         task_len, task_dst, long_list, tmeta, be->cap);
-      hipLaunchKernelGGL(task_cursor_kernel, dim3(1), dim3(64), 0, st, tmeta);
-      hipLaunchKernelGGL(task_order_kernel, dim3((max_tasks + tnt - 1) / tnt), dim3(tnt), 0, st, task_start, task_len, task_dst,
-                         toff + nb, tmeta, desc);
-      ZKP_HIP(hipEventRecord(ws.sorted, st));
-      ctx->mark(st, ":sorted");
-    }
     MsmWorkspace& bws = bucket_ws >= 0 ? ctx->cur->ws[bucket_ws] : ws;
     char* buckets = reinterpret_cast<char*>(bws.buckets.get((size_t)2 * nb * XB + XB));
     char* task_partial = reinterpret_cast<char*>(ws.partial.get((size_t)max_tasks * XB));
     static const bool zero_all = getenv("ZKP_MEMSET_BUCKETS") && atoi(getenv("ZKP_MEMSET_BUCKETS")) != 0;
     const uint32_t init = into >= 0 ? 1u : 0u;
+    const bool zero_empty = !init && !zero_all;
+    if (!reuse) {
+      exclusive_scan_u32(st, TaskCountLoad{start, end, nb, be->cap, zero_empty ? buckets : nullptr, (uint32_t)XB, tmeta}, toff,
+                         (size_t)nb + 1, ws.scan_tmp2);
+      static const uint32_t tnt = [] { const char* e = getenv("ZKP_TASK_NT"); const int v = e ? atoi(e) : 1024; return (uint32_t)(v >= 1024 ? 1024 : v >= 512 ? 512 : 256); }();
+      hipLaunchKernelGGL(task_fill_kernel, dim3((nb + tnt - 1) / tnt), dim3(tnt), 0, st, start, end, toff, nb, task_start,
+                         task_len, task_dst, long_list, tmeta, be->cap);
+      hipLaunchKernelGGL(task_order_kernel, dim3((max_tasks + tnt - 1) / tnt), dim3(tnt), 0, st, task_start, task_len, task_dst,
+                         toff + nb, tmeta, desc);
+      ZKP_HIP(hipEventRecord(ws.sorted, st));
+      ctx->mark(st, ":sorted");
+    }
     if (init) {
       ZKP_REQUIRE(bws.chain_nb == nb && bws.chain_xb == XB, ZKP_ERR_BAD_ARG);
       ZKP_HIP(hipStreamWaitEvent(st, bws.acc_done, 0));
     } else if (zero_all) ZKP_HIP(hipMemsetAsync(buckets, 0, (size_t)nb * XB, st));
-    else hipLaunchKernelGGL(zero_empty_buckets_kernel, dim3((nb + 255) / 256), dim3(256), 0, st, start, end, nb, buckets, (uint32_t)XB);
+    else if (reuse) hipLaunchKernelGGL(zero_empty_buckets_kernel, dim3((nb + 255) / 256), dim3(256), 0, st, start, end, nb, buckets, (uint32_t)XB);
     bws.chain_nb = 0;
     const bool timed = ms_accumulate && ctx->profiling;
     if (timed) ZKP_HIP(hipEventRecord(ctx->ev2, st));
@@ -990,84 +1023,115 @@
     if (ctx->dbg_skip_k8) return;
 #endif
     const int L = c - 1;
-    SegPlan plan{};
-    plan.L = L;
     const uint32_t chunk = ctx->batch_mode ? SEG_CHUNK_BATCH : SEG_CHUNK;
-    plan.chunk = chunk;
-    uint32_t lvl_off = 0, cnt = nb, blocks = 0;
     static const bool fuse_seg = !(getenv("ZKP_PAIR_TOP_FUSE_SEG") && atoi(getenv("ZKP_PAIR_TOP_FUSE_SEG")) == 0);
-    int l_top = -1;
-    char* top_base = nullptr;
-    uint32_t top_cnt = 0;
-    for (int l = 0; l < L; l++) {
-      uint32_t next_off = lvl_off + cnt;
-      static const bool top_fused = !(getenv("ZKP_PAIR_TOP") && atoi(getenv("ZKP_PAIR_TOP")) == 0);
-      static const uint32_t top_max = [] {
-        const char* e = getenv("ZKP_PAIR_TOP_MAX");
-        uint32_t v = e ? (uint32_t)atoi(e) : PAIR_TOP_MAX;
-        if (v < 2) v = PAIR_TOP_MAX;
-        while (v & (v - 1)) v &= v - 1;
-        return v;
-      }();
-      if (!top_fused || cnt > top_max) vt->pair(st, buckets + (size_t)lvl_off * XB, buckets + (size_t)next_off * XB, cnt / 2);
-      else if (cnt == top_max || l == 0) {
-        if (fuse_seg && cnt / 2 <= chunk) {
-          l_top = l;
-          top_base = buckets + (size_t)lvl_off * XB;
-          top_cnt = cnt;
+    static const bool top_fused = !(getenv("ZKP_PAIR_TOP") && atoi(getenv("ZKP_PAIR_TOP")) == 0);
+    static const uint32_t top_max = [] {
+      const char* e = getenv("ZKP_PAIR_TOP_MAX");
+      uint32_t v = e ? (uint32_t)atoi(e) : PAIR_TOP_MAX;
+      if (v < 2) v = PAIR_TOP_MAX;
+      while (v & (v - 1)) v &= v - 1;
+      return v;
+    }();
+    const int FK = vt->pair_fused_levels;
+    const uint32_t ftile = 256u << FK;
+    const bool fuse_levels = FK > 0 && top_fused && fuse_seg && top_max / 2 <= chunk;
+    enum { LV_PAIR = 0, LV_FUSED_HEAD, LV_FUSED, LV_TOP };
+    struct Level {
+      uint32_t off, cnt, first, nblk;
+      int kind;
+    } lv[26] = {};
+    int l_top = -1, l_top_plain = -1;
+    {
+      uint32_t off = 0, cnt = nb;
+      for (int l = 0; l <= L; l++, off += cnt, cnt /= 2) lv[l] = Level{off, cnt, 0, 0, LV_PAIR};
+      for (int l = 0; l < L;) {
+        const uint32_t cnt_l = lv[l].cnt;
+        if (top_fused && cnt_l <= top_max) {
+          if (fuse_seg && cnt_l / 2 <= chunk) l_top = l;
+          else l_top_plain = l;
+          for (; l < L; l++) lv[l].kind = LV_TOP;
+        } else if (fuse_levels && cnt_l % ftile == 0 && l + FK <= L) {
+          lv[l].kind = LV_FUSED_HEAD;
+          for (int k = 1; k < FK; k++) lv[l + k].kind = LV_FUSED;
+          l += FK;
         } else {
-          vt->pair_top(st, buckets + (size_t)lvl_off * XB, cnt);
+          l++;
         }
       }
-      plan.first_block[l] = blocks;
-      plan.off[l] = lvl_off + 1;
-      plan.stride[l] = 2;
-      plan.count[l] = cnt / 2;
-      blocks += (cnt / 2 + chunk - 1) / chunk;
-      lvl_off = next_off;
-      cnt /= 2;
-    }
-    plan.first_block[L] = blocks;
-    const char* root = buckets + (size_t)lvl_off * XB;
+    }
+    uint32_t blocks = 0;
+    for (int l = 0; l < L; l++)
+      if (lv[l].kind == LV_PAIR || lv[l].kind == LV_TOP) {
+        lv[l].first = blocks;
+        lv[l].nblk = (lv[l].cnt / 2 + chunk - 1) / chunk;
+        blocks += lv[l].nblk;
+      }
+    const uint32_t blocks_plain = blocks;
+    for (int l = 0; l < L; l++)
+      if (lv[l].kind == LV_FUSED_HEAD)
+        for (int k = 0; k < FK; k++) {
+          lv[l + k].first = blocks;
+          lv[l + k].nblk = lv[l].cnt / ftile;
+          blocks += lv[l + k].nblk;
+        }
+    const char* root = buckets + (size_t)lv[L].off * XB;
     char* partial = reinterpret_cast<char*>(ws.tmp.get(((size_t)blocks + 64) * XB));
     char* Obuf = partial + (size_t)blocks * XB;
-    if (L > 0 && l_top >= 0) {
-      SegPlan low = plan;
-      low.L = l_top;
-      const uint32_t blocks_low = plan.first_block[l_top];
-      vt->pair_top_segsum(st, top_base, top_cnt, buckets, &low, partial, blocks_low);
+    for (int l = 0; l < L; l++) {
+      if (lv[l].kind == LV_PAIR) {
+        vt->pair(st, buckets + (size_t)lv[l].off * XB, buckets + (size_t)lv[l + 1].off * XB, lv[l].cnt / 2);
+      } else if (lv[l].kind == LV_FUSED_HEAD) {
+        PairFusedOut po{};
+        for (int k = 0; k < FK; k++) po.first[k] = lv[l + k].first;
+        vt->pair_fused(st, buckets + (size_t)lv[l].off * XB, buckets + (size_t)lv[l + FK].off * XB, lv[l].cnt / ftile, partial, po);
+      }
+    }
+    if (l_top_plain >= 0) vt->pair_top(st, buckets + (size_t)lv[l_top_plain].off * XB, lv[l_top_plain].cnt);
+    auto first_stage_plan = [&](int upto) {
+      SegPlan p{};
+      p.chunk = chunk;
+      int j = 0;
+      for (int l = 0; l < upto; l++)
+        if (lv[l].kind == LV_PAIR || lv[l].kind == LV_TOP) {
+          p.first_block[j] = lv[l].first;
+          p.off[j] = lv[l].off + 1;
+          p.stride[j] = 2;
+          p.count[j] = lv[l].cnt / 2;
+          j++;
+        }
+      p.L = j;
+      p.first_block[j] = j ? p.first_block[j - 1] + (p.count[j - 1] + chunk - 1) / chunk : 0;
+      return p;
+    };
+    if (L > 0) {
+      if (l_top >= 0) {
+        const SegPlan low = first_stage_plan(l_top);
+        vt->pair_top_segsum(st, buckets + (size_t)lv[l_top].off * XB, lv[l_top].cnt, buckets, &low, partial, low.first_block[low.L]);
+      } else {
+        const SegPlan all = first_stage_plan(L);
+        ZKP_REQUIRE(all.first_block[all.L] == blocks_plain && blocks == blocks_plain, ZKP_ERR_BAD_ARG);
+        vt->segsum(st, buckets, &all, partial, blocks_plain, nullptr, 1 << 30);
+      }
       SegPlan p2{};
       p2.L = L;
       p2.chunk = chunk;
       for (int l = 0; l < L; l++) {
         p2.first_block[l] = l;
-        if (l < l_top) {
-          p2.off[l] = plan.first_block[l];
+        if (l_top < 0 || l < l_top) {
+          p2.off[l] = lv[l].first;
           p2.stride[l] = 1;
-          p2.count[l] = plan.first_block[l + 1] - plan.first_block[l];
+          p2.count[l] = lv[l].nblk;
         } else {
-          p2.off[l] = plan.off[l];
-          p2.stride[l] = plan.stride[l];
-          p2.count[l] = plan.count[l];
+          p2.off[l] = lv[l].off + 1;
+          p2.stride[l] = 2;
+          p2.count[l] = lv[l].cnt / 2;
         }
         ZKP_REQUIRE(p2.count[l] <= chunk, ZKP_ERR_BAD_ARG);
       }
       p2.first_block[L] = L;
-      vt->segsum(st, partial, &p2, Obuf, L, buckets, l_top);
-    } else if (L > 0) {
-      vt->segsum(st, buckets, &plan, partial, blocks, nullptr, 1 << 30);
-      SegPlan p2{};
-      p2.L = L;
-      p2.chunk = chunk;
-      for (int l = 0; l < L; l++) {
-        p2.first_block[l] = l;
-        p2.off[l] = plan.first_block[l];
-        p2.stride[l] = 1;
-        p2.count[l] = plan.first_block[l + 1] - plan.first_block[l];
-        ZKP_REQUIRE(p2.count[l] <= chunk, ZKP_ERR_BAD_ARG);
-      }
-      p2.first_block[L] = L;
-      vt->segsum(st, partial, &p2, Obuf, L, nullptr, 1 << 30);
+      if (l_top >= 0) vt->segsum(st, partial, &p2, Obuf, L, buckets, l_top);
+      else vt->segsum(st, partial, &p2, Obuf, L, nullptr, 1 << 30);
     }
     vt->final(st, Obuf, L, root, (char*)out_dev_xyzz, out_jac);
     ctx->mark(st, ":reduced");
diff --git a/ckb_zkp_amd/csrc/msm_group.hip b/ckb_zkp_amd/csrc/msm_group.hip
--- a/ckb_zkp_amd/csrc/msm_group.hip
+++ b/ckb_zkp_amd/csrc/msm_group.hip
@@ -164,6 +164,46 @@
     return;
   }
   segsum_body<F>(base, plan, partial, blockIdx.x - 1, nullptr, 1 << 30);
+}
+
+template <class F>
+__global__ __launch_bounds__(256) void pair_fused_kernel(char* in, char* __restrict__ out, char* __restrict__ partial, PairFusedOut po) {
+  __builtin_amdgcn_s_setprio(3);
+  using B = BkPoint<F>;
+  constexpr size_t PB = B::BYTES;
+  constexpr int E = 1 << PAIR_FUSED_K;
+  static_assert(PAIR_FUSED_K == 3, "the addition schedule below is written for eight entries per thread");
+  if constexpr (B::MEM_ADD) {
+    const uint32_t t = threadIdx.x;
+    char* blk = in + (size_t)blockIdx.x * 256 * E * PB;
+    char* e = blk + (size_t)t * E * PB;
+    static constexpr unsigned char OPS[11][3] = {{0, 1, 0}, {2, 3, 2}, {1, 3, 1}, {4, 5, 4}, {1, 5, 1}, {6, 7, 6}, {1, 7, 1},
+                                                 {2, 6, 3}, {0, 2, 0}, {4, 6, 4}, {0, 4, 8}};
+    char* mine_out = out + ((size_t)blockIdx.x * 256 + t) * PB;
+#pragma unroll 1
+    for (int k = 0; k < 11; k++) {
+      const int o = OPS[k][2];
+      B::add_mem(e + OPS[k][0] * PB, e + OPS[k][1] * PB, o == E ? mine_out : e + o * PB);
+    }
+    auto slot = [&](uint32_t tree, uint32_t j) { return blk + ((size_t)j * E + (tree == 0 ? 1 : tree == 1 ? 3 : 4)) * PB; };
+    __threadfence_block();
+    __syncthreads();
+    for (uint32_t s = 128; s > 0; s >>= 1) {
+      const uint32_t adds = PAIR_FUSED_K * s;
+      bool coop = false;
+      if constexpr (QuadCoop<F>::ON) {
+        coop = adds <= 128;
+        if (coop)
+          for (uint32_t i = t >> 2; i < adds; i += 64)
+            quad_add_any<F>(slot(i / s, i % s), slot(i / s, i % s + s), slot(i / s, i % s), t & 3);
+      }
+      if (!coop)
+        for (uint32_t i = t; i < adds; i += 256) B::add_mem(slot(i / s, i % s), slot(i / s, i % s + s), slot(i / s, i % s));
+      __threadfence_block();
+      __syncthreads();
+    }
+    if (t < (uint32_t)PAIR_FUSED_K) B::copy_point(partial + ((size_t)po.first[t] + blockIdx.x) * PB, slot(t, 0));
+  }
 }
 
 constexpr uint32_t COMBINE_SMALL = 32;
@@ -883,6 +923,9 @@
   hipLaunchKernelGGL(pair_top_segsum_kernel<F>, dim3(1 + blocks), dim3(PAIR_TOP_THREADS), 256 * BB, s, top_base, top_cnt, base, *plan,
                      partial);
 }
+void l_pair_fused(hipStream_t s, char* in, char* out, uint32_t groups, char* partial, PairFusedOut po) {
+  hipLaunchKernelGGL(pair_fused_kernel<F>, dim3(groups), dim3(256), 0, s, in, out, partial, po);
+}
 void l_final(hipStream_t s, const char* O, int L, const char* root, char* out_xyzz, uint32_t* out_jac) {
   constexpr int threads = (QuadCoop<F>::ON && QuadCoop<F>::GROUP == 1) ? 128 : 64;
   hipLaunchKernelGGL(final_kernel<F>, dim3(1), dim3(threads), 64 * BB, s, O, L, root, out_xyzz, out_jac);
@@ -977,6 +1020,7 @@
       nullptr, nullptr,
 #endif
       l_pair_top_segsum,
+      BkPoint<F>::MEM_ADD ? PAIR_FUSED_K : 0, BkPoint<F>::MEM_ADD ? l_pair_fused : nullptr,
   };
   return &v;
 }
diff --git a/ckb_zkp_amd/csrc/msm_vtbl.hpp b/ckb_zkp_amd/csrc/msm_vtbl.hpp
--- a/ckb_zkp_amd/csrc/msm_vtbl.hpp
+++ b/ckb_zkp_amd/csrc/msm_vtbl.hpp
@@ -19,6 +19,11 @@
 
 struct SegDesc {
   uint32_t off, stride, count, out;
+};
+
+constexpr int PAIR_FUSED_K = 3;
+struct PairFusedOut {
+  uint32_t first[PAIR_FUSED_K];
 };
 
 struct MsmVtbl {
@@ -60,6 +65,8 @@
                 const uint8_t* kind, const uint32_t* coeff, const char* G_xy, const uint8_t* G_inf, char* out_xy, uint8_t* out_inf);
   void (*pair_top_segsum)(hipStream_t, char* top_base, uint32_t top_cnt, const char* base, const SegPlan* plan, char* partial,
                           uint32_t blocks);
+  int pair_fused_levels;
+  void (*pair_fused)(hipStream_t, char* in, char* out, uint32_t groups, char* partial, PairFusedOut po);
 };
 constexpr uint32_t PAIR_TOP_MAX = 2048;
 
diff --git a/include/zkp_accel.h b/include/zkp_accel.h
--- a/include/zkp_accel.h
+++ b/include/zkp_accel.h
@@ -312,6 +312,7 @@
 int32_t zkp_set_profiling(zkp_ctx* ctx, int32_t enable);
 int32_t zkp_bench_mulmod(zkp_ctx* ctx, zkp_curve_t curve, int32_t field, int32_t unsaturated, double* gmulmod_per_s);
 int32_t zkp_bench_hbm_copy(zkp_ctx* ctx, size_t bytes, double* gbytes_per_s);
+int32_t zkp_debug_exclusive_scan_u32(zkp_ctx* ctx, const uint32_t* in_host, size_t n, uint32_t* out_host);
 
 #ifdef __cplusplus
 }
diff --git a/rust/zkp-accel/src/ffi.rs b/rust/zkp-accel/src/ffi.rs
--- a/rust/zkp-accel/src/ffi.rs
+++ b/rust/zkp-accel/src/ffi.rs
@@ -294,4 +294,5 @@
     pub fn zkp_set_profiling(ctx: *mut zkp_ctx, enable: i32) -> i32;
     pub fn zkp_bench_mulmod(ctx: *mut zkp_ctx, curve: c_int, field: i32, unsaturated: i32, gmulmod_per_s: *mut f64) -> i32;
     pub fn zkp_bench_hbm_copy(ctx: *mut zkp_ctx, bytes: usize, gbytes_per_s: *mut f64) -> i32;
-}
+    pub fn zkp_debug_exclusive_scan_u32(ctx: *mut zkp_ctx, in_host: *const u32, n: usize, out_host: *mut u32) -> i32;
+}
```

Result: slower. 122.9 proofs/s (-10.9%).
